# limeorange1102/multimodal-av-model

Measured on AMD Instinct MI355X. Metric: utterances/sec (4 s clip, 25 fps 96x96 lip) at batch 64, full training step, higher is better.
Workload: dtype bf16; 1 GPU; BASELINE metric configuration (= configs[3]'s per-GPU batch): batch 64/GPU x 4 s (T_audio 64000, T_enc 199, 100 lip frames 96x96 x 2 speakers), wav2vec2-large + ResNet-18 + fusion BiLSTM + CTC + contrastive, fwd+bwd+Adam, random-init weights; variant=as_executed, global_batch=64, parallelism=dp1, audio_passes=2, wav2vec2_regularizers=hf-defaults (dropout 0.1, LayerDrop 0.1, SpecAugment 0.05)

## Files before the change

include/av_hip.h:

```cpp
#ifndef AV_HIP_H
#define AV_HIP_H
#ifdef __cplusplus
extern "C" {
#endif

#define AV_OK 0
#define AV_ERR_ARG 1
#define AV_ERR_LAUNCH 2

#define AV_F32 0
#define AV_BF16 1

#define AV_A_ROWMAJOR 0
#define AV_A_TRANS 1
#define AV_A_CONV2D 2
#define AV_A_CONV3D1 3
#define AV_B_NK 0
#define AV_B_KN 1
#define AV_ACT_NONE 0
#define AV_ACT_GELU 1
#define AV_ACT_MUL_GELU_GRAD 2
#define AV_ACT_GELU_GF 3
#define AV_ACT_MUL_AUX 4

const char* av_last_error(void);
int av_version(void);

typedef struct av_gemm_args {
    const void* A;
    const void* B;
    void* C;
    void* C2;
    const float* bias;
    const float* R;
    const void* aux;
    float* stats;
    int M, N, K, batch;
    long long lda, ldb, ldc, ldr;
    long long sA, sB, sC, sR, sBias;
    int a_mode, b_mode, in_dtype, out_dtype, aux_dtype, act;
    float alpha;
    int cT, cH, cW, cCtot, cCin, cCoff;
    int cKt, cKh, cKw, cSh, cSw, cPt, cPh, cPw, cOh, cOw;
    int batch_inner;
    long long oA, oB, oC;
    float drop_p;
    unsigned int drop_stream;
    unsigned long long drop_seed;
    int k_total;
    int cNF, cPM;
} av_gemm_args;
int av_gemm(const av_gemm_args* args, void* stream);
int av_sum_slices(const float* parts, int n_slices, long long n, long long stride, float alpha, float* out, int accumulate,
                  void* stream);
int av_transpose(const void* in, int idt, void* out, int odt, int R, int C, long long ldi, int Rpad, void* stream);

int av_layernorm_fwd(const void* x, int xdt, const float* gamma, const float* beta, void* y, int ydt,
                     float* mean, float* rstd, long long rows, int cols, float eps, int act, void* stream);
int av_layernorm_bwd(const void* x, int xdt, const void* dy, int dydt, const float* gamma, const float* mean,
                     const float* rstd, const float* dres, float* dx, float* dgb_partial, int nblk,
                     long long rows, int cols, void* dx_bf16, void* stream);
int av_layernorm_bwd_drop(const void* x, int xdt, const void* dy, int dydt, const float* gamma, const float* mean,
                          const float* rstd, const float* dres, float* dx, float* dgb_partial, int nblk,
                          long long rows, int cols, void* dx_bf16, float drop_p, unsigned long long drop_seed,
                          unsigned int drop_stream, void* stream);
int av_log_softmax_fwd(const void* x, int xdt, float* y, long long rows, int cols, void* stream);
int av_log_softmax_bwd(const float* y, const float* dy, void* dx, int dxdt, long long rows, int cols, void* stream);
int av_log_softmax_bwd_ld(const float* y, const float* dy, void* dx, int dxdt, long long rows, int cols, int ldx, void* stream);
int av_colsum(const void* x, int xdt, float* out, long long rows, int cols, long long ld, int accumulate,
              void* stream);
int av_cast(const void* x, int xdt, void* y, int ydt, long long n, void* stream);
int av_cast_dropout(const void* x, int xdt, void* y, int ydt, long long n, float p, unsigned long long seed, unsigned int stream_id,
                    void* stream);
int av_dropout_uniform(float* u, long long n, unsigned long long seed, unsigned int stream_id, void* stream);
int av_fusion_xattn_fwd(const void* a, const void* v, const void* w_in, const float* b_in, void* q_out, void* kv_out, void* o,
                        float* lse, int B, int T, int E, int H, float scale, void* stream);
int av_fusion_xattn_bwd(const void* q, const void* kv, const void* o, const void* dout, const float* lse, void* dq, void* dkv, int B, int T,
                        int E, int H, float scale, void* stream);
int av_zero_feature_cols(void* x, int xdt, const unsigned char* mask, int B, int T, int H, void* stream);
int av_overwrite_rows(void* x, int xdt, const unsigned char* mask, const float* embed, long long rows, int cols, void* stream);
int av_axpby(float a, const void* x, int xdt, float b, float* y, long long n, void* stream);
int av_mask_rows(void* x, int xdt, const unsigned char* keep, long long rows, int cols, void* stream);
int av_mul_scalar_dev(const float* x, const float* scalar, float* y, long long n, void* stream);

int av_attention_fwd(const void* q, const void* k, const void* v, void* o, float* lse, int dtype, int B, int H, int Tq,
                     int Tk, int D, long long q_bs, long long q_rs, long long k_bs, long long k_rs, long long v_bs,
                     long long v_rs, long long o_bs, long long o_rs, const int* klen, float scale, float drop_p,
                     unsigned long long drop_seed, unsigned int drop_stream, void* stream);
int av_attention_bwd(const void* q, const void* k, const void* v, const void* o, const void* dout, const float* lse,
                     float* delta_ws, void* dq, void* dk, void* dv, int B, int H, int Tq, int Tk, int D,
                     const long long* strides, const int* klen, float scale, float drop_p, unsigned long long drop_seed,
                     unsigned int drop_stream, void* stream);
int av_attention_dropmask(void* mask, int B, int H, int Tq, int Tk, float drop_p, unsigned long long drop_seed, unsigned int drop_stream,
                          void* stream);
int av_attention_fwd_mask(const void* q, const void* k, const void* v, void* o, float* lse, int dtype, int B, int H, int Tq,
                          int Tk, int D, long long q_bs, long long q_rs, long long k_bs, long long k_rs, long long v_bs,
                          long long v_rs, long long o_bs, long long o_rs, const int* klen, float scale, float drop_p,
                          unsigned long long drop_seed, unsigned int drop_stream, const void* drop_mask, void* stream);
int av_attention_bwd_mask(const void* q, const void* k, const void* v, const void* o, const void* dout, const float* lse,
                          float* delta_ws, void* dq, void* dk, void* dv, int B, int H, int Tq, int Tk, int D,
                          const long long* strides, const int* klen, float scale, float drop_p, unsigned long long drop_seed,
                          unsigned int drop_stream, const void* drop_mask, void* stream);
int av_softmax_rows(const float* s, void* p, int pdt, long long rows, int cols, float scale, const int* klen,
                    int rows_per_batch, int ld, void* stream);
int av_softmax_bwd_rows(const void* p, int pdt, const float* dp, void* ds, int dsdt, long long rows, int cols,
                        float scale, int ld, void* stream);

int av_conv0_ln_gelu(const float* wav, const float* w, const float* bias, const float* gamma, const float* beta, void* out,
                     int out_dtype, int B, int T_in, int L_out, int C, int k, int stride, float eps, void* stream);

int av_lstm_fwd_step(const float* gx, const void* whh, void* hseq, float* cseq, void* gates, void* out_bt, int dtype,
                     int T, int B, int H, int s, void* stream);
int av_lstm_bwd_step(const void* dout, int dout_dtype, long long do_bs, long long do_ts, void* dgates, const void* whhT,
                     const void* gates, const float* cseq, float* dc, int dtype, int T, int B, int H, int s, void* stream);

#define AV_LSTM_COUNTER_INTS 1024
int av_lstm_fwd_layer(const float* gx, const void* whh, void* hseq, float* cseq, void* gates, void* out_bt, int* counters,
                      int T, int B, int H, void* stream);
int av_lstm_bwd_layer(const void* dout, int dout_dtype, long long do_bs, long long do_ts, void* dgates, const void* whhT,
                      const void* gates, const float* cseq, float* dc, int* counters, int T, int B, int H, void* stream);

int av_mask_downsample(const long long* mask, long long* out, int B, int Tin, int Tout, void* stream);
int av_fusion_gather_lerp_fwd(const float* feat, const long long* mask, int* ws_i32, float* out, long long* mask_out,
                              long long* lens, int B, int Ta, int Tv, int D, int groups, void* stream);
int av_fusion_gather_lerp_bwd(const float* dout, const int* ws_i32, float* dfeat, int B, int Ta, int Tv, int D, int groups,
                              void* stream);
int av_permute_bt(const void* in, int idt, void* out, int odt, int B, int T, int D, void* stream);
int av_gather_rows(const void* src, int sdt, const long long* idx, void* out, int odt, long long n, int D, void* stream);
int av_scatter_rows(const float* src, const long long* idx, float* out, long long n, int D, float alpha, int accumulate,
                    void* stream);
int av_class_order(const long long* mask, long long n, long long* order, void* stream);

int av_conv3d_front(const float* x, const void* w, void* y, float* stats, int B, int T, int H, int W, void* stream);
int av_conv3d_front_pool(const float* x, const void* w, void* ymax, void* ymin, float* stats, int B, int T, int H, int W, void* stream);
int av_bn_prelu_minmax(const void* ymax, const void* ymin, const float* scale, const float* shift, const float* slope, void* out, long long n,
                       void* stream);
int av_conv3x3_c64(const void* x, const void* w, void* y, float* stats, int n_img, int H, int W, const float* in_scale,
                   const float* in_shift, const float* in_slope, void* stream);
int av_bn_finalize(const float* partial, int nblk, long long count, const float* gamma, const float* beta,
                   float* running_mean, float* running_var, float momentum, float eps, int training, float* scale,
                   float* shift, int C, double* ws, int ws_zeroed, void* stream);
int av_bn_act(const void* x, const float* scale, const float* shift, const void* res, const float* rscale,
              const float* rshift, const float* slope, void* out, int dtype, long long n, int C, void* stream);
int av_bn_prelu_maxpool(const void* x, const float* scale, const float* shift, const float* slope, void* out, int dtype,
                        long long N, int H, int W, int C, void* stream);
int av_avgpool(const void* x, int dtype, float* out, long long N, int HW, int C, int pm_block, void* stream);

int av_l2norm_fwd(const float* x, float* y, float* nrm, long long rows, int cols, float eps, void* stream);
int av_l2norm_bwd(const float* y, const float* dy, const float* nrm, float* dx, long long rows, int cols, float eps,
                  void* stream);
int av_lse_rows(const float* s, float* lse, float* rowsum, long long rows, int cols, int ld, void* stream);
int av_contrastive_dsim(const float* s, const float* lse, void* out, int odt, long long rows, int cols, int ld, float coef,
                        void* stream);
int av_lse_rows_chunk(const float* s, float* lse, float* rowsum, long long rows, int cols, int ld, int accumulate, void* stream);
int av_contrastive_dsim_chunk(const float* s, const float* lse, void* out, int odt, long long rows, int cols, int ld, float coef,
                              int total_cols, void* stream);
int av_reduce_sum(const float* x, long long n, float* out, float scale, int accumulate, void* stream);
int av_loss_combine(const float* nll, const float* w, const float* c1, const float* c2, float half_lambda, int n, float* out3,
                    void* stream);
int av_ctc_greedy(const float* log_probs, const long long* lengths, int* out_ids, int* out_len, int B, int T, int V, int blank,
                  void* stream);
int av_ctc_beam_workspace_bytes(int B, int T, int V, int beam_width, long long* bytes);
int av_ctc_beam_frame_pass(const float* log_probs, long long stride_b, long long stride_t, const long long* lengths, void* workspace,
                           long long workspace_bytes, int B, int T, int V, int blank, int beam_width, void* stream);
int av_ctc_beam_search(const float* log_probs, long long stride_b, long long stride_t, const long long* lengths, int* out_ids,
                       int* out_len, float* out_score, void* workspace, long long workspace_bytes, int B, int T, int V, int blank,
                       int beam_width, int nbest, void* stream);
int av_ngram_score(const int* ids, const long long* lens, float* out, int B, int Lmax, const float* lm_unigrams, const void* lm_table,
                   long long lm_slots, int lm_order, int lm_vocab, int lm_bos, int lm_probe_bound, void* stream);
int av_ctc_beam_lm_workspace_bytes(int B, int T, int V, int beam_width, int tokens, long long* bytes);
int av_ctc_beam_search_lm(const float* log_probs, long long stride_b, long long stride_t, const long long* lengths, int* out_ids,
                          int* out_len, float* out_score, float* out_lm_score, void* workspace, long long workspace_bytes, int B, int T,
                          int V, int blank, int beam_width, int nbest, int tokens, const float* lm_unigrams, const void* lm_table,
                          long long lm_slots, int lm_order, int lm_vocab, int lm_bos, int lm_probe_bound, float lm_weight,
                          float token_bonus, void* stream);
int av_ctc_loss_fwd(const float* log_probs, long long stride_b, long long stride_t, const long long* targets, long long target_ld,
                    const long long* input_lengths, const long long* target_lengths, int B, int T, int V, int S_max, int blank,
                    int zero_infinity, float* nll, float* log_alpha, float* log_beta, void* stream);
int av_ctc_loss_bwd(const float* log_probs, long long stride_b, long long stride_t, const long long* targets, long long target_ld,
                    const long long* input_lengths, const long long* target_lengths, int B, int T, int V, int S_max, int blank,
                    const float* nll, const float* log_alpha, const float* log_beta, const float* grad_nll, float* grad, void* stream);
int av_ctc_align_workspace_bytes(int B, int T, int S_max, long long* bytes);
int av_ctc_align(const float* log_probs, long long stride_b, long long stride_t, const long long* targets, long long target_ld,
                 const long long* input_lengths, const long long* target_lengths, int B, int T, int V, int S_max, int blank,
                 int* out_state, int* out_span, float* out_token_score, float* out_score, void* workspace, long long workspace_bytes,
                 void* stream);
int av_lip_gray_resize(const void* src, int src_is_u8, float* dst, int T, int Hs, int Ws, int C, int Hd, int Wd, float divisor,
                       void* stream);
int av_mix_pair(const float* a1, long long len1, const float* a2, long long len2, float* mixed, long long* mask1, long long* mask2,
                unsigned* peak_ws, void* stream);
int av_adam_step(float* p, const float* g, float* m, float* v, long long n, float lr, float beta1, float beta2, float eps,
                 int step, float grad_scale, void* stream);
int av_adam_multi(const void* ptrs, const long long* sizes, const float* hyper, const int* chunk_tensor, const long long* chunk_start,
                  int n_chunks, int chunk_elems, int* steps, const int* step_slot, int n_tensors, float grad_scale,
                  float* scaler_state, float growth, float backoff, int growth_interval, void* stream);

int av_nchw_to_nhwc(const float* in, void* out, int out_dtype, long long N, int C, int H, int W, int Cp, void* stream);
int av_relu_maxpool2_fwd(const void* x, void* y, int dtype, long long N, int H, int W, int C, int nchw_out, void* stream);
int av_relu_maxpool2_bwd(const void* x, const void* dy, void* dx, int dtype, long long N, int H, int W, int C, int nchw_dy, void* stream);
int av_im2col3(const void* x, void* cols, int dtype, long long N, int H, int W, int C, void* stream);
int av_gru_fwd_step(const float* gx, const void* whh, const float* bhh, void* hseq, float* hf, float* gates, void* out_bt, int dtype,
                    int T, int B, int H, int s, void* stream);
int av_gru_bwd_step(const void* dout, int dout_dtype, long long do_bs, long long do_ts, void* dgi, void* dgh, const void* whhT,
// ... 45 lines not shown
```

multimodal-av-model_amd/_lib.py:

```python
from __future__ import annotations

import ctypes as C
import os

from . import precision as _precision

_HERE = os.path.dirname(os.path.abspath(__file__))
LIB_PATH = os.environ.get("AVAMD_LIB") or os.path.join(_HERE, "libavhip.so")

AV_F32, AV_BF16 = 0, 1
A_ROWMAJOR, A_TRANS, A_CONV2D, A_CONV3D1 = 0, 1, 2, 3
B_NK, B_KN = 0, 1
ACT_NONE, ACT_GELU, ACT_MUL_GELU_GRAD, ACT_GELU_GF, ACT_MUL_AUX = 0, 1, 2, 3, 4
LSTM_COUNTER_INTS = 1024

vp, ll, i32, f32 = C.c_void_p, C.c_longlong, C.c_int, C.c_float


class GemmArgs(C.Structure):
    _fields_ = [
        ("A", vp), ("B", vp), ("C", vp), ("C2", vp), ("bias", vp), ("R", vp), ("aux", vp), ("stats", vp),
        ("M", i32), ("N", i32), ("K", i32), ("batch", i32),
        ("lda", ll), ("ldb", ll), ("ldc", ll), ("ldr", ll),
        ("sA", ll), ("sB", ll), ("sC", ll), ("sR", ll), ("sBias", ll),
        ("a_mode", i32), ("b_mode", i32), ("in_dtype", i32), ("out_dtype", i32), ("aux_dtype", i32), ("act", i32),
        ("alpha", f32),
        ("cT", i32), ("cH", i32), ("cW", i32), ("cCtot", i32), ("cCin", i32), ("cCoff", i32),
        ("cKt", i32), ("cKh", i32), ("cKw", i32), ("cSh", i32), ("cSw", i32), ("cPt", i32), ("cPh", i32), ("cPw", i32),
        ("cOh", i32), ("cOw", i32),
        ("batch_inner", i32), ("oA", ll), ("oB", ll), ("oC", ll),
        ("drop_p", f32), ("drop_stream", C.c_uint), ("drop_seed", C.c_ulonglong),
        ("k_total", i32), ("cNF", i32), ("cPM", i32),
    ]


class W2v2LayerArgs(C.Structure):
    _fields_ = [
        ("B", i32), ("T", i32), ("hidden", i32), ("heads", i32), ("inter", i32), ("lp", i32), ("gf", i32), ("stream_base", i32),
        ("eps", f32), ("scale", f32), ("hd_p", f32), ("at_p", f32), ("ac_p", f32),
        ("seed", C.c_ulonglong),
        ("ln1_g", vp), ("ln1_b", vp), ("ln2_g", vp), ("ln2_b", vp), ("b_qkv", vp), ("b_o", vp), ("b_1", vp), ("b_2", vp),
        ("w_qkv", vp), ("w_o", vp), ("w_1", vp), ("w_2", vp),
        ("h", vp), ("klen", vp), ("amask", vp),
        ("x1", vp), ("qkv", vp), ("ao", vp), ("x2", vp), ("u", vp), ("g", vp),
        ("mu1", vp), ("rs1", vp), ("lse", vp), ("h2", vp), ("mu2", vp), ("rs2", vp), ("h3", vp),
    ]


class W2v2LayerBwdArgs(C.Structure):
    _fields_ = [
        ("B", i32), ("T", i32), ("hidden", i32), ("heads", i32), ("inter", i32), ("lp", i32), ("gf", i32), ("stream_base", i32), ("lower_stream", i32),
        ("scale", f32), ("hd_p", f32), ("at_p", f32), ("ac_p", f32),
        ("seed", C.c_ulonglong),
        ("ln1_g", vp), ("ln2_g", vp),
        ("w_2t", vp), ("w_1t", vp), ("w_ot", vp), ("w_qkvt", vp),
        ("dh", vp), ("h", vp), ("mu1", vp), ("rs1", vp), ("lse", vp), ("h2", vp), ("mu2", vp), ("rs2", vp),
        ("dh_lp", vp), ("qkv", vp), ("ao", vp), ("amask", vp), ("u", vp),
        ("klen", vp),
        ("dh3_t", vp), ("du", vp), ("dx2", vp), ("dh2_lp", vp), ("dao", vp), ("dqkv", vp), ("dx1", vp), ("dh_out_lp", vp),
        ("dh2", vp), ("delta", vp), ("dh_out", vp),
    ]


SIGNATURES = {
    "av_last_error": [],
    "av_version": [],
    "av_gemm": [C.POINTER(GemmArgs), vp],
    "av_w2v2_layer_fwd": [C.POINTER(W2v2LayerArgs), vp],
    "av_w2v2_layer_bwd_dx": [C.POINTER(W2v2LayerBwdArgs), vp],
    "av_transpose": [vp, i32, vp, i32, i32, i32, ll, i32, vp],
    "av_sum_slices": [vp, i32, ll, ll, f32, vp, i32, vp],
    "av_layernorm_fwd": [vp, i32, vp, vp, vp, i32, vp, vp, ll, i32, f32, i32, vp],
    "av_layernorm_bwd_drop": [vp, i32, vp, i32, vp, vp, vp, vp, vp, vp, i32, ll, i32, vp, f32, C.c_ulonglong, C.c_uint, vp],
    "av_layernorm_bwd": [vp, i32, vp, i32, vp, vp, vp, vp, vp, vp, i32, ll, i32, vp, vp],
    "av_log_softmax_fwd": [vp, i32, vp, ll, i32, vp],
    "av_log_softmax_bwd": [vp, vp, vp, i32, ll, i32, vp],
    "av_log_softmax_bwd_ld": [vp, vp, vp, i32, ll, i32, i32, vp],
    "av_colsum": [vp, i32, vp, ll, i32, ll, i32, vp],
    "av_cast": [vp, i32, vp, i32, ll, vp],
    "av_cast_dropout": [vp, i32, vp, i32, ll, f32, C.c_ulonglong, C.c_uint, vp],
    "av_dropout_uniform": [vp, ll, C.c_ulonglong, C.c_uint, vp],
    "av_fusion_xattn_fwd": [vp, vp, vp, vp, vp, vp, vp, vp, i32, i32, i32, i32, f32, vp],
    "av_fusion_xattn_bwd": [vp, vp, vp, vp, vp, vp, vp, i32, i32, i32, i32, f32, vp],
    "av_zero_feature_cols": [vp, i32, vp, i32, i32, i32, vp],
    "av_overwrite_rows": [vp, i32, vp, vp, ll, i32, vp],
    "av_axpby": [f32, vp, i32, f32, vp, ll, vp],
    "av_mask_rows": [vp, i32, vp, ll, i32, vp],
    "av_mul_scalar_dev": [vp, vp, vp, ll, vp],
    "av_attention_fwd": [vp, vp, vp, vp, vp, i32, i32, i32, i32, i32, i32, ll, ll, ll, ll, ll, ll, ll, ll, vp, f32, f32, C.c_ulonglong, C.c_uint, vp],
    "av_attention_dropmask": [vp, i32, i32, i32, i32, f32, C.c_ulonglong, C.c_uint, vp],
    "av_attention_fwd_mask": [vp, vp, vp, vp, vp, i32, i32, i32, i32, i32, i32, ll, ll, ll, ll, ll, ll, ll, ll, vp, f32, f32, C.c_ulonglong, C.c_uint, vp, vp],
    "av_attention_bwd_mask": [vp, vp, vp, vp, vp, vp, vp, vp, vp, vp, i32, i32, i32, i32, i32, vp, vp, f32, f32, C.c_ulonglong, C.c_uint, vp, vp],
    "av_attention_bwd": [vp, vp, vp, vp, vp, vp, vp, vp, vp, vp, i32, i32, i32, i32, i32, vp, vp, f32, f32, C.c_ulonglong, C.c_uint, vp],
    "av_softmax_rows": [vp, vp, i32, ll, i32, f32, vp, i32, i32, vp],
    "av_conv0_ln_gelu": [vp, vp, vp, vp, vp, vp, i32, i32, i32, i32, i32, i32, i32, f32, vp],
    "av_lstm_fwd_step": [vp, vp, vp, vp, vp, vp, i32, i32, i32, i32, i32, vp],
    "av_lstm_bwd_step": [vp, i32, ll, ll, vp, vp, vp, vp, vp, i32, i32, i32, i32, i32, vp],
    "av_lstm_fwd_layer": [vp, vp, vp, vp, vp, vp, vp, i32, i32, i32, vp],
    "av_lstm_bwd_layer": [vp, i32, ll, ll, vp, vp, vp, vp, vp, vp, i32, i32, i32, vp],
    "av_mask_downsample": [vp, vp, i32, i32, i32, vp],
    "av_fusion_gather_lerp_fwd": [vp, vp, vp, vp, vp, vp, i32, i32, i32, i32, i32, vp],
    "av_fusion_gather_lerp_bwd": [vp, vp, vp, i32, i32, i32, i32, i32, vp],
    "av_permute_bt": [vp, i32, vp, i32, i32, i32, i32, vp],
    "av_gather_rows": [vp, i32, vp, vp, i32, ll, i32, vp],
    "av_scatter_rows": [vp, vp, vp, ll, i32, f32, i32, vp],
    "av_class_order": [vp, ll, vp, vp],
    "av_conv3d_front": [vp, vp, vp, vp, i32, i32, i32, i32, vp],
    "av_conv3d_front_pool": [vp, vp, vp, vp, vp, i32, i32, i32, i32, vp],
    "av_bn_prelu_minmax": [vp, vp, vp, vp, vp, vp, ll, vp],
    "av_conv3x3_c64": [vp, vp, vp, vp, i32, i32, i32, vp, vp, vp, vp],
    "av_bn_finalize": [vp, i32, ll, vp, vp, vp, vp, f32, f32, i32, vp, vp, i32, vp, i32, vp],
    "av_bn_act": [vp, vp, vp, vp, vp, vp, vp, vp, i32, ll, i32, vp],
    "av_bn_prelu_maxpool": [vp, vp, vp, vp, vp, i32, ll, i32, i32, i32, vp],
    "av_avgpool": [vp, i32, vp, ll, i32, i32, i32, vp],
    "av_l2norm_fwd": [vp, vp, vp, ll, i32, f32, vp],
    "av_l2norm_bwd": [vp, vp, vp, vp, ll, i32, f32, vp],
    "av_lse_rows": [vp, vp, vp, ll, i32, i32, vp],
    "av_lse_rows_chunk": [vp, vp, vp, ll, i32, i32, i32, vp],
    "av_contrastive_dsim_chunk": [vp, vp, vp, i32, ll, i32, i32, f32, i32, vp],
    "av_contrastive_dsim": [vp, vp, vp, i32, ll, i32, i32, f32, vp],
    "av_reduce_sum": [vp, ll, vp, f32, i32, vp],
    "av_loss_combine": [vp, vp, vp, vp, f32, i32, vp, vp],
    "av_ctc_greedy": [vp, vp, vp, vp, i32, i32, i32, i32, vp],
    "av_ctc_beam_workspace_bytes": [i32, i32, i32, i32, C.POINTER(ll)],
    "av_ctc_beam_frame_pass": [vp, ll, ll, vp, vp, ll, i32, i32, i32, i32, i32, vp],
    "av_ctc_beam_search": [vp, ll, ll, vp, vp, vp, vp, vp, ll, i32, i32, i32, i32, i32, i32, vp],
    "av_ngram_score": [vp, vp, vp, i32, i32, vp, vp, ll, i32, i32, i32, i32, vp],
    "av_ctc_beam_lm_workspace_bytes": [i32, i32, i32, i32, i32, C.POINTER(ll)],
    "av_ctc_beam_search_lm": [vp, ll, ll, vp, vp, vp, vp, vp, vp, ll, i32, i32, i32, i32, i32, i32, i32, vp, vp, ll, i32, i32, i32, i32, f32, f32, vp],
    "av_ctc_loss_fwd": [vp, ll, ll, vp, ll, vp, vp, i32, i32, i32, i32, i32, i32, vp, vp, vp, vp],
    "av_ctc_loss_bwd": [vp, ll, ll, vp, ll, vp, vp, i32, i32, i32, i32, i32, vp, vp, vp, vp, vp, vp],
    "av_ctc_align_workspace_bytes": [i32, i32, i32, C.POINTER(ll)],
    "av_ctc_align": [vp, ll, ll, vp, ll, vp, vp, i32, i32, i32, i32, i32, vp, vp, vp, vp, vp, ll, vp],
    "av_lip_gray_resize": [vp, i32, vp, i32, i32, i32, i32, i32, i32, f32, vp],
    "av_mix_pair": [vp, ll, vp, ll, vp, vp, vp, vp, vp],
    "av_adam_multi": [vp, vp, vp, vp, vp, i32, i32, vp, vp, i32, f32, vp, f32, f32, i32, vp],
    "av_adam_step": [vp, vp, vp, vp, ll, f32, f32, f32, f32, i32, f32, vp],
    "av_softmax_bwd_rows": [vp, i32, vp, vp, i32, ll, i32, f32, i32, vp],
    "av_nchw_to_nhwc": [vp, vp, i32, ll, i32, i32, i32, i32, vp],
    "av_relu_maxpool2_fwd": [vp, vp, i32, ll, i32, i32, i32, i32, vp],
    "av_relu_maxpool2_bwd": [vp, vp, vp, i32, ll, i32, i32, i32, i32, vp],
    "av_im2col3": [vp, vp, i32, ll, i32, i32, i32, vp],
    "av_gru_fwd_step": [vp, vp, vp, vp, vp, vp, vp, i32, i32, i32, i32, i32, vp],
    "av_gru_bwd_step": [vp, i32, ll, ll, vp, vp, vp, vp, vp, vp, i32, i32, i32, i32, i32, vp],
    "av_wav_info": [C.c_char_p, C.POINTER(i32), C.POINTER(i32), C.POINTER(ll), C.POINTER(i32), C.POINTER(i32)],
    "av_wav_read_mono_f32": [C.c_char_p, ll, ll, vp],
    "av_resample_sinc": [vp, ll, vp, ll, vp, vp, i32, i32, i32, i32, vp],
}
_RESTYPES = {"av_last_error": C.c_char_p}

_libs = {}
_by_mode = {}


def _path() -> str:
    if _precision.get_precision() == "fp16":
        return os.environ.get("AVAMD_LIB_F16") or os.path.join(_HERE, "libavhip_f16.so")
    return LIB_PATH


def lib() -> C.CDLL:
    l = _by_mode.get(_precision._mode)
    if l is not None:
        return l
    path = _path()
    l = _libs.get(path)
    if l is None:
        if not os.path.exists(path):
            raise RuntimeError(
                f"{path} is missing: build it with `python {os.path.join(_HERE, 'build.py')}` "
                "(hipcc --offload-arch=gfx950). The MI355X path has no CPU/PyTorch fallback.")
        import torch
        l = C.CDLL(path)
        for name, argtypes in SIGNATURES.items():
            fn = getattr(l, name)
            fn.argtypes = argtypes
            fn.restype = _RESTYPES.get(name, C.c_int)
        _libs[path] = l
    _by_mode[_precision._mode] = l
    return l


def check(status: int, what: str = "") -> None:
    if status != 0:
        msg = lib().av_last_error().decode("utf-8", "replace")
# ... 2 lines not shown
```

multimodal-av-model_amd/csrc/gemm.hip:

```cpp
#include "av_common.h"

namespace {

constexpr int BM = 128;
constexpr int BK = 32;
constexpr int NT = 256;

template <typename T> struct Cfg;
template <> struct Cfg<float> { static constexpr int LD = 36, VEC = 4; };
template <> struct Cfg<bf16_t> { static constexpr int LD = 40, VEC = 8; };

template <typename T> struct Vec16 { uint4 v; };

template <typename T> __device__ __forceinline__ T elem_of(const uint4& v, int i);
template <> __device__ __forceinline__ float elem_of<float>(const uint4& v, int i) {
    const unsigned u = i == 0 ? v.x : i == 1 ? v.y : i == 2 ? v.z : v.w;
    return __uint_as_float(u);
}
template <> __device__ __forceinline__ bf16_t elem_of<bf16_t>(const uint4& v, int i) {
    const unsigned u = (i >> 1) == 0 ? v.x : (i >> 1) == 1 ? v.y : (i >> 1) == 2 ? v.z : v.w;
    const unsigned short s = (i & 1) ? (unsigned short)(u >> 16) : (unsigned short)(u & 0xffff);
    return __builtin_bit_cast(bf16_t, s);
}
template <typename T> __device__ __forceinline__ void set_elem(uint4& v, int i, T x);
// ... 215 lines not shown
    stage_load<T, BM, AMODE>(ra, A, p.lda, m0, p.M, 0, p.K, a_vec, p, ri, tid);
    stage_load<T, BN, BMODE == AV_B_NK ? AV_A_ROWMAJOR : AV_A_TRANS>(rb, B, p.ldb, n0, p.N, 0, p.K, b_vec, p, rib, tid);
    stage_store<T, BM, AMODE>(sA, ra, tid);
    stage_store<T, BN, BMODE == AV_B_NK ? AV_A_ROWMAJOR : AV_A_TRANS>(sB, rb, tid);
    __syncthreads();

    for (int kt = 0; kt < nk; ++kt) {
        const int cur = kt & 1;
        if (kt + 1 < nk) {
            stage_load<T, BM, AMODE>(ra, A, p.lda, m0, p.M, (kt + 1) * BK, p.K, a_vec, p, ri, tid);
            stage_load<T, BN, BMODE == AV_B_NK ? AV_A_ROWMAJOR : AV_A_TRANS>(rb, B, p.ldb, n0, p.N, (kt + 1) * BK, p.K, b_vec, p, rib, tid);
        }
        mma_step<T, WN_T>(sA + cur * BM * LD + wm * 64 * LD, sB + cur * BN * LD + wn * (BN / 2) * LD, acc, lane);
        if (kt + 1 < nk) {
            stage_store<T, BM, AMODE>(sA + (cur ^ 1) * BM * LD, ra, tid);
            stage_store<T, BN, BMODE == AV_B_NK ? AV_A_ROWMAJOR : AV_A_TRANS>(sB + (cur ^ 1) * BN * LD, rb, tid);
        }
        __syncthreads();
    }

    const int r = lane & 15, g = lane >> 4;
    const long long cbase = (long long)zo * p.oC + (long long)zi * p.sC;
    const float* R = p.R ? p.R + (long long)zi * p.sR : nullptr;
    float csum[WN_T], csq[WN_T];
#pragma unroll
    for (int j = 0; j < WN_T; ++j) { csum[j] = 0.f; csq[j] = 0.f; }
#pragma unroll
    for (int j = 0; j < WN_T; ++j) {
        const int n = n0 + wn * (BN / 2) + j * 16 + r;
        const bool nok = n < p.N;
        const float bias = (p.bias && nok) ? p.bias[(long long)zi * p.sBias + n] : 0.f;
#pragma unroll
        for (int i = 0; i < 4; ++i) {
#pragma unroll
            for (int e = 0; e < 4; ++e) {
                const int m = m0 + wm * 64 + i * 16 + 4 * g + e;
                if (nok && m < p.M) {
                    float v = acc[i][j][e] * p.alpha + bias;
                    const long long off = cbase + (long long)m * p.ldc + n;
                    if (p.act == AV_ACT_GELU_GF) {
                        const float mlt = p.drop_p > 0.f ? drop_mult_call(p.drop_seed, p.drop_stream, (unsigned long long)off, p.drop_p, drop_inv_keep(p.drop_p)) : 1.f;
                        if (p.C2) st_any(p.C2, off, p.out_dtype, gelu_grad_f(v) * mlt);
                        v = gelu_f(v) * mlt;
                    } else {
                        if (p.C2) st_any(p.C2, off, p.out_dtype, v);
                        if (p.act == AV_ACT_GELU) v = gelu_f(v);
                        else if (p.act == AV_ACT_MUL_GELU_GRAD) v *= gelu_grad_f(ld_any(p.aux, off, p.aux_dtype));
                        else if (p.act == AV_ACT_MUL_AUX) v *= ld_any(p.aux, off, p.aux_dtype);
                        if (p.drop_p > 0.f) v *= drop_mult_call(p.drop_seed, p.drop_stream, (unsigned long long)off, p.drop_p, drop_inv_keep(p.drop_p));
                    }
                    if (R) v += R[(long long)m * p.ldr + n];
                    st_any(p.C, off, p.out_dtype, v);
                    csum[j] += v; csq[j] += v * v;
                }
            }
        }
    }
    if (p.stats) {
        __syncthreads();
        float* red = (float*)smem;
#pragma unroll
        for (int j = 0; j < WN_T; ++j) {
            float s = csum[j], q = csq[j];
            s += __shfl_xor(s, 16, 64); s += __shfl_xor(s, 32, 64);
            q += __shfl_xor(q, 16, 64); q += __shfl_xor(q, 32, 64);
            if (g == 0) {
                const int col = wn * (BN / 2) + j * 16 + r;
                red[(wm * 2 + 0) * BN + col] = s;
                red[(wm * 2 + 1) * BN + col] = q;
            }
        }
        __syncthreads();
        if (tid < BN && n0 + tid < p.N) {
            float* out = p.stats + (long long)mb * 2 * p.N;
            out[n0 + tid] = red[0 * BN + tid] + red[2 * BN + tid];
            out[p.N + n0 + tid] = red[1 * BN + tid] + red[3 * BN + tid];
        }
    }
}

template <typename T, int BN, int AMODE, int BMODE>
int launch(const av_gemm_args& p, hipStream_t st, bool a_vec, bool b_vec) {
    const size_t lds = (size_t)(2 * BM + 2 * BN) * Cfg<T>::LD * sizeof(T);
    static bool attr_done = false;
    auto kern = gemm_kernel<T, BN, AMODE, BMODE>;
    if (!attr_done && lds > 48 * 1024) {
        if (hipFuncSetAttribute((const void*)kern, hipFuncAttributeMaxDynamicSharedMemorySize, (int)lds) != hipSuccess) {
            av_set_error("av_gemm: cannot raise dynamic LDS to %zu", lds);
            return AV_ERR_LAUNCH;
        }
        attr_done = true;
    }
    const int nbM = av_cdiv(p.M, BM), nbN = av_cdiv(p.N, BN);
    dim3 grid((unsigned)(nbM * (long long)nbN), 1, (unsigned)p.batch);
    hipLaunchKernelGGL(kern, grid, dim3(NT), lds, st, p, nbN, a_vec, b_vec);
    AV_LAUNCH_CHECK();
    return AV_OK;
}

template <typename T, int BN>
int dispatch_modes(const av_gemm_args& p, hipStream_t st, bool a_vec, bool b_vec) {
    if (p.a_mode == AV_A_ROWMAJOR && p.b_mode == AV_B_NK) return launch<T, BN, AV_A_ROWMAJOR, AV_B_NK>(p, st, a_vec, b_vec);
    if (p.a_mode == AV_A_ROWMAJOR && p.b_mode == AV_B_KN) return launch<T, BN, AV_A_ROWMAJOR, AV_B_KN>(p, st, a_vec, b_vec);
    if (p.a_mode == AV_A_TRANS && p.b_mode == AV_B_KN) return launch<T, BN, AV_A_TRANS, AV_B_KN>(p, st, a_vec, b_vec);
    if (p.a_mode == AV_A_CONV2D && p.b_mode == AV_B_NK) return launch<T, BN, AV_A_CONV2D, AV_B_NK>(p, st, a_vec, b_vec);
    if (p.a_mode == AV_A_CONV3D1 && p.b_mode == AV_B_NK) return launch<T, BN, AV_A_CONV3D1, AV_B_NK>(p, st, a_vec, b_vec);
    av_set_error("av_gemm: unsupported operand mode pair a_mode=%d b_mode=%d", p.a_mode, p.b_mode);
    return AV_ERR_ARG;
}

template <typename T>
bool vec_ok(const void* base, long long ld, long long stride) {
    const long long es = sizeof(T);
    return ((uintptr_t)base % 16 == 0) && ((ld * es) % 16 == 0) && ((stride * es) % 16 == 0);
}
template <typename T> bool vec_ok2(const void* base, long long ld, long long s1, long long s2) {
    return vec_ok<T>(base, ld, s1) && ((s2 * (long long)sizeof(T)) % 16 == 0);
}

}

int av_gemm_fast_try(const av_gemm_args& p, hipStream_t st);

extern "C" int av_gemm(const av_gemm_args* a, void* stream) {
    AV_CHECK(a != nullptr, "av_gemm: null args");
    const av_gemm_args& p = *a;
    AV_CHECK(p.A && p.B && p.C, "av_gemm: null operand pointer");
    AV_CHECK(p.M >= 0 && p.N >= 0 && p.K > 0 && p.batch >= 1, "av_gemm: bad shape M=%d N=%d K=%d batch=%d", p.M, p.N, p.K, p.batch);
    AV_CHECK(p.in_dtype == AV_F32 || p.in_dtype == AV_BF16, "av_gemm: bad in_dtype %d", p.in_dtype);
    AV_CHECK(p.out_dtype == AV_F32 || p.out_dtype == AV_BF16, "av_gemm: bad out_dtype %d", p.out_dtype);
    AV_CHECK(!(p.stats && p.batch != 1), "av_gemm: stats need batch == 1");
    AV_CHECK(!((p.act == AV_ACT_MUL_GELU_GRAD || p.act == AV_ACT_MUL_AUX) && !p.aux), "av_gemm: MUL_GELU_GRAD / MUL_AUX need aux");
    AV_CHECK(p.act >= AV_ACT_NONE && p.act <= AV_ACT_MUL_AUX, "av_gemm: unknown activation %d", p.act);
    AV_CHECK(p.drop_p >= 0.f && p.drop_p < 1.f, "av_gemm: drop_p=%f out of [0,1)", p.drop_p);
    if (p.M == 0 || p.N == 0) return AV_OK;
    const long long es = p.in_dtype == AV_F32 ? 4 : 2;
    const int vec = (int)(16 / es);
    if (p.a_mode == AV_A_CONV2D) {
        AV_CHECK(p.cCin % vec == 0 && p.cCoff % vec == 0 && p.cCtot % vec == 0 && (uintptr_t)p.A % 16 == 0 && (p.sA * es) % 16 == 0,
                 "av_gemm conv2d: channels (Cin=%d, Coff=%d, Ctot=%d) must be multiples of %d and the base 16-byte aligned", p.cCin, p.cCoff, p.cCtot, vec);
        AV_CHECK(p.K == p.cKh * p.cKw * p.cCin, "av_gemm conv2d: K=%d != Kh*Kw*Cin", p.K);
        AV_CHECK(p.cOh > 0 && p.cOw > 0 && p.M % (p.cOh * p.cOw) == 0, "av_gemm conv2d: M=%d not a multiple of Oh*Ow", p.M);
    }
    if (p.a_mode == AV_A_CONV3D1) {
        AV_CHECK(p.K == p.cKt * p.cKh * p.cKw, "av_gemm conv3d: K=%d != Kt*Kh*Kw", p.K);
        AV_CHECK(p.cOh > 0 && p.cOw > 0 && p.cT > 0 && p.M % (p.cOh * p.cOw * p.cT) == 0, "av_gemm conv3d: bad M=%d", p.M);
    }
    hipStream_t st = (hipStream_t)stream;
    {
        const int fr = av_gemm_fast_try(p, st);
        if (fr >= 0) return fr;
    }
    AV_CHECK(p.cPM == 0, "av_gemm: position-major pixel order (cPM) needs the bf16 fast path (2-D convolution, Cin a multiple of 64, one batch)");
    AV_CHECK(p.k_total == 0, "av_gemm: split-K (k_total) needs the bf16 fast path with both operands k-major (a_mode 1, b_mode 1, M, N multiples of 8 and > 64)");
    const bool wide = p.N > 64;
    if (p.in_dtype == AV_F32) {
        const bool av = vec_ok2<float>(p.A, p.lda, p.sA, p.oA), bv = vec_ok2<float>(p.B, p.ldb, p.sB, p.oB);
        return wide ? dispatch_modes<float, 128>(p, st, av, bv) : dispatch_modes<float, 64>(p, st, av, bv);
    } else {
        const bool av = vec_ok2<bf16_t>(p.A, p.lda, p.sA, p.oA), bv = vec_ok2<bf16_t>(p.B, p.ldb, p.sB, p.oB);
        return wide ? dispatch_modes<bf16_t, 128>(p, st, av, bv) : dispatch_modes<bf16_t, 64>(p, st, av, bv);
    }
}
```

multimodal-av-model_amd/csrc/gemm_fast.hip:

```cpp
#include <cstdlib>

#include "av_common.h"

namespace {

constexpr int BM = 128, BK = 64, NT = 256;
constexpr int TILE_A = BM * BK * 2;

typedef const __attribute__((address_space(1))) void* gptr_t;
typedef __attribute__((address_space(3))) void* lptr_t;

__device__ __attribute__((aligned(256))) unsigned char g_zero_line[256];

#ifdef AV_GEMM_STAMPS
__device__ unsigned long long g_gemm_stamps[8192 * 4];
#define AV_STAMP(SLOT) do { if (threadIdx.x == 0 && blockIdx.x < 8192) g_gemm_stamps[blockIdx.x * 4 + (SLOT)] = __builtin_amdgcn_s_memrealtime(); } while (0)
__device__ unsigned long long g_v7_stamps[256 * 16 * 4];
#define AV_STAMP7(SEQ, SLOT) do { if (threadIdx.x == 0 && blockIdx.x < 256 && (SEQ) < 16) g_v7_stamps[(blockIdx.x * 16 + (SEQ)) * 4 + (SLOT)] = __builtin_amdgcn_s_memrealtime(); } while (0)
#else
#define AV_STAMP(SLOT) do { } while (0)
#define AV_STAMP7(SEQ, SLOT) do { } while (0)
#endif

template <int NWI>
// ... 239 lines not shown
                bf16x8 o;
#pragma unroll
                for (int e = 0; e < 8; ++e) o[e] = (bf16_t)gf[e];
                {
#if AV_EPI_NT
                    __builtin_nontemporal_store(o, (bf16x8*)((bf16_t*)p.C2 + off));
#else
                    *(bf16x8*)((bf16_t*)p.C2 + off) = o;
#endif
                }
            } else {
#pragma unroll
                for (int e = 0; e < 8; ++e) if (gn + e < p.N) st_any(p.C2, off + e, p.out_dtype, gf[e]);
            }
        }
    } else
    if (p.C2) {
        if (full && fl.c_vec) {
            if (p.out_dtype == AV_BF16) {
                bf16x8 o;
#pragma unroll
                for (int e = 0; e < 8; ++e) o[e] = (bf16_t)v[e];
                *(bf16x8*)((bf16_t*)p.C2 + off) = o;
            } else {
                *(f32x4*)((float*)p.C2 + off) = f32x4{v[0], v[1], v[2], v[3]};
                *(f32x4*)((float*)p.C2 + off + 4) = f32x4{v[4], v[5], v[6], v[7]};
            }
        } else {
#pragma unroll
            for (int e = 0; e < 8; ++e) if (gn + e < p.N) st_any(p.C2, off + e, p.out_dtype, v[e]);
        }
    }
    if (p.act == AV_ACT_GELU) {
        av_f32x2 x4[4], g4[4];
#pragma unroll
        for (int k = 0; k < 4; ++k) x4[k] = av_f32x2{v[2 * k], v[2 * k + 1]};
        gelu_fast2x4(x4, g4);
#pragma unroll
        for (int k = 0; k < 4; ++k) { v[2 * k] = g4[k].x; v[2 * k + 1] = g4[k].y; }
    } else if (p.act == AV_ACT_MUL_AUX) {
        if (full && fl.aux_vec && p.aux_dtype == AV_BF16) {
            const bf16x8 u = *(const bf16x8*)((const bf16_t*)p.aux + off);
#pragma unroll
            for (int e = 0; e < 8; ++e) v[e] *= (float)u[e];
        } else {
#pragma unroll
            for (int e = 0; e < 8; ++e) if (gn + e < p.N) v[e] *= ld_any(p.aux, off + e, p.aux_dtype);
        }
    } else if (p.act == AV_ACT_MUL_GELU_GRAD) {
        if (full && fl.aux_vec && p.aux_dtype == AV_BF16) {
            const bf16x8 u = *(const bf16x8*)((const bf16_t*)p.aux + off);
#pragma unroll
            for (int e = 0; e < 8; e += 2) { const av_f32x2 g = gelu_grad_fast2(av_f32x2{(float)u[e], (float)u[e + 1]}); v[e] *= g.x; v[e + 1] *= g.y; }
        } else {
#pragma unroll
            for (int e = 0; e < 8; ++e) if (gn + e < p.N) v[e] *= gelu_grad_fast(ld_any(p.aux, off + e, p.aux_dtype));
        }
    }
    if (p.drop_p > 0.f && p.act != AV_ACT_GELU_GF) {
        const float ik = drop_inv_keep(p.drop_p);
        if (VO || (off & 3) == 0) {
            float m4[4];
            drop_mult4(p.drop_seed, p.drop_stream, (unsigned long long)off, p.drop_p, ik, m4);
#pragma unroll
            for (int e = 0; e < 4; e += 2) { const av_f32x2 t = av_f32x2{v[e], v[e + 1]} * av_f32x2{m4[e], m4[e + 1]}; v[e] = t.x; v[e + 1] = t.y; }
            drop_mult4(p.drop_seed, p.drop_stream, (unsigned long long)off + 4, p.drop_p, ik, m4);
#pragma unroll
            for (int e = 0; e < 4; e += 2) { const av_f32x2 t = av_f32x2{v[4 + e], v[5 + e]} * av_f32x2{m4[e], m4[e + 1]}; v[4 + e] = t.x; v[5 + e] = t.y; }
        } else {
#pragma unroll
            for (int e = 0; e < 8; ++e) v[e] *= drop_mult(p.drop_seed, p.drop_stream, (unsigned long long)(off + e), p.drop_p, ik);
        }
    }
    if (R) {
        const long long roff = (long long)gm * p.ldr + gn;
        if (full && fl.r_vec) {
            const f32x4 r0 = *(const f32x4*)(R + roff), r1 = *(const f32x4*)(R + roff + 4);
#pragma unroll
            for (int e = 0; e < 4; e += 2) {
                const av_f32x2 a = av_f32x2{v[e], v[e + 1]} + av_f32x2{r0[e], r0[e + 1]}, b = av_f32x2{v[4 + e], v[5 + e]} + av_f32x2{r1[e], r1[e + 1]};
                v[e] = a.x; v[e + 1] = a.y; v[4 + e] = b.x; v[5 + e] = b.y;
            }
        } else {
#pragma unroll
            for (int e = 0; e < 8; ++e) if (gn + e < p.N) v[e] += R[roff + e];
        }
    }
    if (full && fl.c_vec) {
        if (p.out_dtype == AV_BF16) {
            bf16x8 o;
#pragma unroll
            for (int e = 0; e < 8; ++e) o[e] = (bf16_t)v[e];
            *(bf16x8*)((bf16_t*)p.C + off) = o;
        } else {
            *(f32x4*)((float*)p.C + off) = f32x4{v[0], v[1], v[2], v[3]};
            *(f32x4*)((float*)p.C + off + 4) = f32x4{v[4], v[5], v[6], v[7]};
        }
    } else {
#pragma unroll
        for (int e = 0; e < 8; ++e) if (gn + e < p.N) st_any(p.C, off + e, p.out_dtype, v[e]);
    }
}

__device__ __forceinline__ void epilogue_store(const av_gemm_args& p, const FastFlags& fl, float (&v)[8], long long off, int gm, int gn, bool full,
                                               const float* R) {
    epilogue_store_t<false>(p, fl, v, off, gm, gn, full, R);
}


template <int BNT, bool CONV, bool AKM = false, bool BKM = false>
__global__ __launch_bounds__(NT, 2) void gemm_nt_bf16_kernel(const av_gemm_args p, const int nbM, const int nbN, const FastFlags fl) {
    constexpr int WM_T = BNT == 128 ? 4 : 2;
    constexpr int TILE_BB = BNT * BK * 2;
    constexpr int STAGE = TILE_A + TILE_BB;
    constexpr int CLD = BNT + 4;
    constexpr int EPI_BYTES = BM * CLD * 4;
    extern __shared__ __attribute__((aligned(16))) char smem[];
    const int tid = threadIdx.x, lane = tid & 63, w = tid >> 6;
    const int wrow = BNT == 128 ? (w >> 1) * 64 : w * 32;
    const int wcol = BNT == 128 ? (w & 1) * 64 : 0;
    const int r = lane & 15, g = lane >> 4;

    const int nwg = nbM * nbN;
    int bid = blockIdx.x;
    {
        const int q = nwg >> 3, rem = nwg & 7, xcd = bid & 7, slot = bid >> 3;
        bid = (xcd < rem ? xcd * (q + 1) : rem * (q + 1) + (xcd - rem) * q) + slot;
    }
    constexpr int GM = 8;
    const int per_group = GM * nbN;
    const int grp = bid / per_group, in_grp = bid - grp * per_group;
    const int first_m = grp * GM;
    const int gsz = nbM - first_m < GM ? nbM - first_m : GM;
    const int mb = first_m + in_grp % gsz, nb = in_grp / gsz;
    const int m0 = mb * BM, n0 = nb * BNT;
    const int z = blockIdx.z;
    const int zo = p.batch_inner > 0 ? z / p.batch_inner : 0;
    const int zi = p.batch_inner > 0 ? z % p.batch_inner : z;
    const bf16_t* A = (const bf16_t*)p.A + (long long)zo * p.oA + (long long)zi * p.sA;
    const bf16_t* B = (const bf16_t*)p.B + (long long)zo * p.oB + (long long)zi * p.sB;

    ConvRows cr;
    if constexpr (CONV) conv_rows_init(cr, A, p, m0, w, lane);
    int Kz = p.K;
    if constexpr (AKM && BKM) {
        if (p.k_total > 0 && p.k_total - z * p.K < Kz) Kz = p.k_total - z * p.K;
    }

    f32x4 acc[WM_T][4];
#pragma unroll
    for (int i = 0; i < WM_T; ++i)
#pragma unroll
        for (int j = 0; j < 4; ++j) acc[i][j] = f32x4{0.f, 0.f, 0.f, 0.f};

    TapSeq ts;
    ts.seq = 0ull; ts.ntap = -1; ts.sh = 0;
    if constexpr (CONV) { if (p.cPM) ts = tap_seq(p, m0, BM); }
    auto stage = [&](int kt, char* buf) {
        int k0 = kt * BK;
        if constexpr (CONV) { k0 = tap_k0(p, ts, kt); stage_conv(p, cr, k0, buf, w, lane); }
        else if constexpr (AKM) stage_kmajor(A, p.lda, m0, p.M, kt * BK, Kz, buf, w, lane);
        else stage_rows<4>(A, p.lda, m0, p.M, kt * BK, buf, w, lane);
        if constexpr (BKM) stage_kmajor(B, p.ldb, n0, p.N, kt * BK, Kz, buf + TILE_A, w, lane);
        else stage_rows<BNT / 32>(B, p.ldb, n0, p.N, k0, buf + TILE_A, w, lane);
    };

    int nk = (Kz + BK - 1) / BK;
    if constexpr (CONV) { if (ts.ntap >= 0) nk = ts.ntap << ts.sh; }
    KmOff ao[WM_T], bo[4];
    if constexpr (AKM) {
#pragma unroll
        for (int i = 0; i < WM_T; ++i) ao[i] = kmajor_off(wrow / 16 + i, lane);
    }
    if constexpr (BKM) {
#pragma unroll
        for (int j = 0; j < 4; ++j) bo[j] = kmajor_off(wcol / 16 + j, lane);
    }
    stage(0, smem);
    __syncthreads();

    const int sw = r & 7;
    const char* a_base = smem + (wrow + r) * 128;
    const char* b_base = smem + TILE_A + (wcol + r) * 128;
    for (int kt = 0; kt < nk; ++kt) {
        const int cur = kt & 1;
        if (kt + 1 < nk) stage(kt + 1, smem + (cur ^ 1) * STAGE);
        const char* ab = a_base + cur * STAGE;
        const char* bb = b_base + cur * STAGE;
#pragma unroll
        for (int ks = 0; ks < 2; ++ks) {
            const int choff = ((ks * 4 + g) ^ sw) << 4;
            bf16x8 a[WM_T], b[4];
            bf16x4 ah[4][2], bh[4][2];
#pragma unroll
            for (int i = 0; i < WM_T; ++i) {
                if constexpr (AKM) kmajor_read(smem + cur * STAGE, ao[i], ks, ah[i]);
                else a[i] = *(const bf16x8*)(ab + i * 16 * 128 + choff);
            }
#pragma unroll
            for (int j = 0; j < 4; ++j) {
                if constexpr (BKM) kmajor_read(smem + cur * STAGE + TILE_A, bo[j], ks, bh[j]);
                else b[j] = *(const bf16x8*)(bb + j * 16 * 128 + choff);
            }
            if constexpr (AKM || BKM) {
                asm volatile("s_waitcnt lgkmcnt(0)" ::: "memory");
                if constexpr (AKM) {
                    static_assert(WM_T == 4, "k-major A: 128-wide tiles");
                    kmajor_tie4(ah);
#pragma unroll
                    for (int i = 0; i < WM_T; ++i) a[i] = __builtin_shufflevector(ah[i][0], ah[i][1], 0, 1, 2, 3, 4, 5, 6, 7);
                }
                if constexpr (BKM) {
                    kmajor_tie4(bh);
#pragma unroll
                    for (int j = 0; j < 4; ++j) b[j] = __builtin_shufflevector(bh[j][0], bh[j][1], 0, 1, 2, 3, 4, 5, 6, 7);
                }
            }
#pragma unroll
            for (int i = 0; i < WM_T; ++i)
#pragma unroll
                for (int j = 0; j < 4; ++j)
                    acc[i][j] = AV_MFMA_F32_16X16X32_LP(a[i], b[j], acc[i][j], 0, 0, 0);
        }
        __syncthreads();
    }

    float* cs = (float*)smem;
#pragma unroll
    for (int i = 0; i < WM_T; ++i)
#pragma unroll
        for (int j = 0; j < 4; ++j)
#pragma unroll
            for (int e = 0; e < 4; ++e)
                cs[(wrow + i * 16 + 4 * g + e) * CLD + wcol + j * 16 + r] = acc[i][j][e] * p.alpha;
    if (p.stats) {
        float* red = (float*)(smem + EPI_BYTES);
        const int wslot = BNT == 128 ? (w >> 1) : w;
#pragma unroll
        for (int j = 0; j < 4; ++j) {
            float s1 = 0.f, s2 = 0.f;
#pragma unroll
            for (int i = 0; i < WM_T; ++i)
#pragma unroll
                for (int e = 0; e < 4; ++e) { const float v = acc[i][j][e] * p.alpha; s1 += v; s2 += v * v; }
            s1 += __shfl_xor(s1, 16, 64); s1 += __shfl_xor(s1, 32, 64);
            s2 += __shfl_xor(s2, 16, 64); s2 += __shfl_xor(s2, 32, 64);
            if (g == 0) {
                red[(wslot * 2) * BNT + wcol + j * 16 + r] = s1;
                red[(wslot * 2 + 1) * BNT + wcol + j * 16 + r] = s2;
            }
        }
    }
    __syncthreads();

    const long long cbase = (long long)zo * p.oC + (long long)zi * p.sC;
    const float* R = p.R ? p.R + (long long)zi * p.sR : nullptr;
    const float* bias = p.bias ? p.bias + (long long)zi * p.sBias : nullptr;
    constexpr int CPR = BNT / 8;
    float bv[8];
    {
        const int gnt = n0 + (tid % CPR) * 8;
#pragma unroll
        for (int e = 0; e < 8; ++e) bv[e] = (bias && gnt + e < p.N) ? bias[gnt + e] : 0.f;
    }
    const bool fast_tail = n0 + BNT <= p.N && fl.c_vec && !p.C2 && p.act == AV_ACT_NONE && p.drop_p <= 0.f && !R && p.out_dtype == AV_BF16;
    if (fast_tail) {
        constexpr int NIT = BM * CPR / NT;
        uint4 ov[NIT];
        const int cc = (tid % CPR) * 8;
#pragma unroll
        for (int it = 0; it < NIT; ++it) {
            const int row = (it * NT + tid) / CPR;
            const f32x4 v0 = *(const f32x4*)(cs + row * CLD + cc), v1 = *(const f32x4*)(cs + row * CLD + cc + 4);
            bf16x8 o;
#pragma unroll
            for (int e = 0; e < 4; ++e) { o[e] = (bf16_t)(v0[e] + bv[e]); o[4 + e] = (bf16_t)(v1[e] + bv[4 + e]); }
            ov[it] = __builtin_bit_cast(uint4, o);
        }
#pragma unroll
        for (int it = 0; it < NIT; ++it) asm volatile("" :: "v"(ov[it].x), "v"(ov[it].y), "v"(ov[it].z), "v"(ov[it].w));
#pragma unroll
        for (int it = 0; it < NIT; ++it) {
            const int row = (it * NT + tid) / CPR;
            if (m0 + row < p.M) *(uint4*)((bf16_t*)p.C + cbase + (long long)(m0 + row) * p.ldc + n0 + cc) = ov[it];
        }
    }
    if (!fast_tail)
#pragma unroll
    for (int it = 0; it < BM * CPR / NT; ++it) {
        const int id = it * NT + tid;
        const int row = id / CPR, cc = (id % CPR) * 8;
        const int gm = m0 + row, gn = n0 + cc;
        if (gm >= p.M || gn >= p.N) continue;
        float v[8];
        const f32x4 v0 = *(const f32x4*)(cs + row * CLD + cc), v1 = *(const f32x4*)(cs + row * CLD + cc + 4);
#pragma unroll
        for (int e = 0; e < 4; ++e) { v[e] = v0[e]; v[4 + e] = v1[e]; }
        const bool full = gn + 8 <= p.N;
        const long long off = cbase + (long long)gm * p.ldc + gn;
#pragma unroll
        for (int e = 0; e < 8; ++e) v[e] += bv[e];
        if (p.act == AV_ACT_GELU_GF) {
            float m[8], gf[8];
#pragma unroll
            for (int e = 0; e < 8; ++e) m[e] = 1.f;
            if (p.drop_p > 0.f) {
                const float ik = drop_inv_keep(p.drop_p);
                if ((off & 3) == 0) {
                    float m4[4];
                    drop_mult4(p.drop_seed, p.drop_stream, (unsigned long long)off, p.drop_p, ik, m4);
#pragma unroll
                    for (int e = 0; e < 4; ++e) m[e] = m4[e];
                    drop_mult4(p.drop_seed, p.drop_stream, (unsigned long long)off + 4, p.drop_p, ik, m4);
#pragma unroll
                    for (int e = 0; e < 4; ++e) m[4 + e] = m4[e];
                } else {
#pragma unroll
                    for (int e = 0; e < 8; ++e) m[e] = drop_mult(p.drop_seed, p.drop_stream, (unsigned long long)(off + e), p.drop_p, ik);
                }
            }
#pragma unroll
            for (int e = 0; e < 8; e += 2) {
                av_f32x2 gl, gp;
                const av_f32x2 mm = av_f32x2{m[e], m[e + 1]};
                gelu_both_fast2(av_f32x2{v[e], v[e + 1]}, gl, gp);
                gl = gl * mm; gp = gp * mm;
                v[e] = gl.x; v[e + 1] = gl.y; gf[e] = gp.x; gf[e + 1] = gp.y;
            }
            if (p.C2) {
                if (full && fl.c_vec && p.out_dtype == AV_BF16) {
                    bf16x8 o;
#pragma unroll
                    for (int e = 0; e < 8; ++e) o[e] = (bf16_t)gf[e];
                    *(bf16x8*)((bf16_t*)p.C2 + off) = o;
                } else {
#pragma unroll
                    for (int e = 0; e < 8; ++e) if (gn + e < p.N) st_any(p.C2, off + e, p.out_dtype, gf[e]);
                }
            }
        } else
        if (p.C2) {
            if (full && fl.c_vec) {
                if (p.out_dtype == AV_BF16) {
                    bf16x8 o;
#pragma unroll
                    for (int e = 0; e < 8; ++e) o[e] = (bf16_t)v[e];
                    *(bf16x8*)((bf16_t*)p.C2 + off) = o;
                } else {
                    *(f32x4*)((float*)p.C2 + off) = f32x4{v[0], v[1], v[2], v[3]};
                    *(f32x4*)((float*)p.C2 + off + 4) = f32x4{v[4], v[5], v[6], v[7]};
                }
            } else {
#pragma unroll
                for (int e = 0; e < 8; ++e) if (gn + e < p.N) st_any(p.C2, off + e, p.out_dtype, v[e]);
            }
        }
        if (p.act == AV_ACT_GELU) {
#pragma unroll
            for (int e = 0; e < 8; e += 2) { const av_f32x2 g = gelu_fast2(av_f32x2{v[e], v[e + 1]}); v[e] = g.x; v[e + 1] = g.y; }
        } else if (p.act == AV_ACT_MUL_AUX) {
            if (full && fl.aux_vec && p.aux_dtype == AV_BF16) {
                const bf16x8 u = *(const bf16x8*)((const bf16_t*)p.aux + off);
#pragma unroll
                for (int e = 0; e < 8; ++e) v[e] *= (float)u[e];
            } else {
#pragma unroll
                for (int e = 0; e < 8; ++e) if (gn + e < p.N) v[e] *= ld_any(p.aux, off + e, p.aux_dtype);
            }
        } else if (p.act == AV_ACT_MUL_GELU_GRAD) {
            if (full && fl.aux_vec && p.aux_dtype == AV_BF16) {
                const bf16x8 u = *(const bf16x8*)((const bf16_t*)p.aux + off);
#pragma unroll
                for (int e = 0; e < 8; e += 2) { const av_f32x2 g = gelu_grad_fast2(av_f32x2{(float)u[e], (float)u[e + 1]}); v[e] *= g.x; v[e + 1] *= g.y; }
            } else {
#pragma unroll
                for (int e = 0; e < 8; ++e) if (gn + e < p.N) v[e] *= gelu_grad_fast(ld_any(p.aux, off + e, p.aux_dtype));
            }
// ... 255 lines not shown
        if (t + 2 < nk) { issue(t + 2); asm volatile("s_waitcnt vmcnt(4)" ::: "memory"); }
        else asm volatile("s_waitcnt vmcnt(0)" ::: "memory");
        __builtin_amdgcn_s_barrier();
        __builtin_amdgcn_s_waitcnt(0xC07F);
        __builtin_amdgcn_sched_barrier(0);
        __builtin_amdgcn_s_setprio(1);
#pragma unroll
        for (int ks = 0; ks < 2; ++ks)
#pragma unroll
            for (int i = 0; i < 4; ++i)
#pragma unroll
                for (int j = 0; j < 2; ++j)
                    acc[i][j] = AV_MFMA_F32_16X16X32_LP(fa[i][ks], fb[j][ks], acc[i][j], 0, 0, 0);
        __builtin_amdgcn_s_setprio(0);
        __builtin_amdgcn_sched_barrier(0);
        __builtin_amdgcn_s_barrier();
        asm volatile("" ::: "memory");
    }
    if (wr == 0) __builtin_amdgcn_s_barrier();

    constexpr int QLD = 128 + 4;
    float* cs = (float*)smem;
    __syncthreads();
#pragma unroll
    for (int i = 0; i < 4; ++i)
#pragma unroll
        for (int j = 0; j < 2; ++j)
#pragma unroll
            for (int e = 0; e < 4; ++e)
                cs[(wr * 64 + i * 16 + 4 * g + e) * QLD + wc * 32 + j * 16 + r] = acc[i][j][e] * p.alpha;
    __syncthreads();
    constexpr int CPR = 128 / 8;
    float bv[8];
    {
        const int gnt = n0 + (tid % CPR) * 8;
#pragma unroll
        for (int e = 0; e < 8; ++e) bv[e] = (bias && gnt + e < p.N) ? bias[gnt + e] : 0.f;
    }
    for (int it = 0; it < 128 * CPR / V4_NT; ++it) {
        const int id = it * V4_NT + tid;
        const int row = id / CPR, cc = (id % CPR) * 8;
        const int gm = m0 + row, gn = n0 + cc;
        if (gm >= m_end || gn >= p.N) continue;
        float v[8];
        const f32x4 v0 = *(const f32x4*)(cs + row * QLD + cc), v1 = *(const f32x4*)(cs + row * QLD + cc + 4);
#pragma unroll
        for (int e = 0; e < 4; ++e) { v[e] = v0[e] + bv[e]; v[4 + e] = v1[e] + bv[4 + e]; }
        const bool full = gn + 8 <= p.N;
        const long long off = cbase + (long long)gm * p.ldc + gn;
        epilogue_store(p, fl, v, off, gm, gn, full, R);
    }
}

struct ConvRows2 { const bf16_t* rowp[2]; unsigned valid[2]; };
__device__ __forceinline__ void conv_rows2_init(ConvRows2& cr, const bf16_t* __restrict__ base, const av_gemm_args& p, int mbase, int w, int lane) {
    const int sub = lane >> 3, choff = ((lane & 7) ^ sub) << 3;
#pragma unroll
    for (int i = 0; i < 2; ++i) {
        const int m = mbase + (w * 2 + i) * 8 + sub;
        cr.rowp[i] = base;
        cr.valid[i] = 0u;
        if (m < p.M) {
            int q, oy, ox;
            conv_decode(p, m, q, oy, ox);
            const int iy0 = oy * p.cSh - p.cPh, ix0 = ox * p.cSw - p.cPw;
            cr.rowp[i] = base + conv_pixel(p, q, iy0, ix0) * p.cCtot + p.cCoff + choff;
            unsigned v = 0u;
            for (int ky = 0; ky < p.cKh; ++ky)
                for (int kx = 0; kx < p.cKw; ++kx)
                    if (iy0 + ky >= 0 && iy0 + ky < p.cH && ix0 + kx >= 0 && ix0 + kx < p.cW) v |= 1u << (ky * p.cKw + kx);
            cr.valid[i] = v;
        }
    }
}
__device__ __forceinline__ void stage_conv2(const av_gemm_args& p, const ConvRows2& cr, int k0, char* tile, int w, int lane, bool all_in) {
    const int sub = lane >> 3, pch = lane & 7;
    const int tap = k0 / p.cCin, c0 = k0 - tap * p.cCin;
    const int ky = tap / p.cKw, kx = tap - ky * p.cKw;
    const long long toff = ((long long)ky * p.cW + kx) * ((p.cPM & 1) ? p.cNF : 1) * p.cCtot + c0;
    if (all_in) {
#pragma unroll
        for (int i = 0; i < 2; ++i) {
            const unsigned off = __builtin_amdgcn_readfirstlane((unsigned)((w * 2 + i) * 1024));
            __builtin_amdgcn_global_load_lds((gptr_t)(cr.rowp[i] + toff), (lptr_t)(tile + off), 16, 0, 0);
        }
        return;
    }
    const bf16_t* zl = (const bf16_t*)g_zero_line + ((pch ^ sub) << 3);
#pragma unroll
    for (int i = 0; i < 2; ++i) {
        const bf16_t* src = ((cr.valid[i] >> tap) & 1u) ? cr.rowp[i] + toff : zl;
        const unsigned off = __builtin_amdgcn_readfirstlane((unsigned)((w * 2 + i) * 1024));
        __builtin_amdgcn_global_load_lds((gptr_t)src, (lptr_t)(tile + off), 16, 0, 0);
    }
}

template <bool CONV, bool KM = false>
__global__ __launch_bounds__(V4_NT, 2) void gemm_nt_bf16_v4_kernel(const av_gemm_args p, const int nbM, const int nbN, const FastFlags fl, const int nfull, const int bm_eff) {
    static_assert(!(CONV && KM), "k-major operands: plain products only");
    extern __shared__ __attribute__((aligned(16))) char smem[];
    AV_STAMP(0);
    const int tid = threadIdx.x, lane = tid & 63, w = tid >> 6;
    const int wr = __builtin_amdgcn_readfirstlane(w >> 2), wc = w & 3;
    const int r = lane & 15, g = lane >> 4;
    const int ntile = nbM * nbN;
    int bid = blockIdx.x, quad = -1;
    if (bid < nfull) {
        const int q = nfull >> 3, rem = nfull & 7, xcd = bid & 7, slot = bid >> 3;
        bid = (xcd < rem ? xcd * (q + 1) : rem * (q + 1) + (xcd - rem) * q) + slot;
    } else {
        const int nq = 4 * (ntile - nfull);
        int j = bid - nfull;
        const int q = nq >> 3, rem = nq & 7, xcd = j & 7, slot = j >> 3;
        j = (xcd < rem ? xcd * (q + 1) : rem * (q + 1) + (xcd - rem) * q) + slot;
        bid = nfull + (j >> 2);
        quad = j & 3;
    }
    int z = blockIdx.z;
    if constexpr (KM) {
        z = bid / ntile;
        bid -= z * ntile;
    }
    constexpr int GM = 4;
    const int per_group = GM * nbN;
    const int grp = bid / per_group, in_grp = bid - grp * per_group;
    const int first_m = grp * GM;
    const int gsz = nbM - first_m < GM ? nbM - first_m : GM;
    const int mb = first_m + in_grp % gsz, nb = in_grp / gsz;
    const int m0 = mb * bm_eff, n0 = nb * V4_BN;
    const int rows_here = p.M - m0 < bm_eff ? p.M - m0 : bm_eff;
    const int zo = p.batch_inner > 0 ? z / p.batch_inner : 0;
    const int zi = p.batch_inner > 0 ? z % p.batch_inner : z;
    const bf16_t* A = (const bf16_t*)p.A + (long long)zo * p.oA + (long long)zi * p.sA;
    const bf16_t* B = (const bf16_t*)p.B + (long long)zo * p.oB + (long long)zi * p.sB;
    if (quad >= 0) {
        const int qm = m0 + (quad >> 1) * 128, qn = n0 + (quad & 1) * 128;
        if (qm < m0 + rows_here && qn < p.N)
            v4_quadrant_job(p, fl, smem, A, B, qm, qn, m0 + rows_here, (long long)zo * p.oC + (long long)zi * p.sC,
                            p.R ? p.R + (long long)zi * p.sR : nullptr, p.bias ? p.bias + (long long)zi * p.sBias : nullptr);
        return;
    }
    auto ntiles = [&](int start) { int n = (rows_here - start + 15) >> 4; return n < 0 ? 0 : (n > 4 ? 4 : n); };
    const int nmt0 = __builtin_amdgcn_readfirstlane(ntiles(wr * 64)), nmt1 = __builtin_amdgcn_readfirstlane(ntiles(128 + wr * 64));

    f32x4 acc[2][2][4][2];
#pragma unroll
    for (int a = 0; a < 2; ++a)
#pragma unroll
        for (int b = 0; b < 2; ++b)
#pragma unroll
            for (int i = 0; i < 4; ++i)
#pragma unroll
                for (int j = 0; j < 2; ++j) acc[a][b][i][j] = f32x4{0.f, 0.f, 0.f, 0.f};

    int nk = p.K / BK;
    int Kz = p.K;
    if constexpr (KM) {
        if (p.k_total > 0 && p.k_total - z * p.K < Kz) Kz = p.k_total - z * p.K;
        nk = (Kz + BK - 1) / BK;
    }
    ConvRows2 cr0, cr1;
    TapSeq ts;
    ts.seq = 0ull; ts.ntap = -1; ts.sh = 0;
    if constexpr (CONV) {
        conv_rows2_init(cr0, A, p, m0, w, lane); conv_rows2_init(cr1, A, p, m0 + 128, w, lane);
        if (p.cPM) { ts = tap_seq(p, m0, V4_BM); if (ts.ntap >= 0) nk = ts.ntap << ts.sh; }
    }
    const bool conv_all_in = CONV && (p.cPM & 2) && ts.ntap >= 0 && m0 + V4_BM <= p.M && m0 / p.cNF == (m0 + V4_BM - 1) / p.cNF;
    KmLane kl[4];
    if constexpr (KM) {
        km_lane_init(kl[0], p.lda, m0, p.M, w, lane); km_lane_init(kl[2], p.lda, m0 + 128, p.M, w, lane);
        km_lane_init(kl[3], p.ldb, n0, p.N, w, lane); km_lane_init(kl[1], p.ldb, n0 + 128, p.N, w, lane);
    }
    const int nh = 4 * nk;
    auto issue = [&](int t, int j, int sidx) {
#ifdef AV_ABL_NODMA
        return;
#endif
        char* slot = smem + sidx * V4_HALF;
        int k0 = t * BK;
#ifdef AV_ABL_KSCRAMBLE
        k0 = (int)(((long long)t * 37) % nk) * BK;
#endif
        if constexpr (CONV) k0 = tap_k0(p, ts, t);
        if constexpr (KM) {
            if (j == 0) stage_kmajor8(A, p.lda, kl[0], k0, Kz, slot, w, lane);
            else if (j == 2) stage_kmajor8(A, p.lda, kl[2], k0, Kz, slot, w, lane);
            else if (j == 3) stage_kmajor8(B, p.ldb, kl[3], k0, Kz, slot, w, lane);
            else stage_kmajor8(B, p.ldb, kl[1], k0, Kz, slot, w, lane);
            return;
        }
        if (j == 0) { if constexpr (CONV) stage_conv2(p, cr0, k0, slot, w, lane, conv_all_in); else stage_rows<2>(A, p.lda, m0, p.M, k0, slot, w, lane); }
        else if (j == 2) { if constexpr (CONV) stage_conv2(p, cr1, k0, slot, w, lane, conv_all_in); else stage_rows<2>(A, p.lda, m0 + 128, p.M, k0, slot, w, lane); }
        else if (j == 3) stage_rows<2>(B, p.ldb, n0, p.N, k0, slot, w, lane);
        else stage_rows<2>(B, p.ldb, n0 + 128, p.N, k0, slot, w, lane);
    };
    issue(0, 0, 0); issue(0, 1, 1); issue(0, 2, 2); issue(0, 3, 3);
    if (nk > 1) {
        issue(1, 0, 4); issue(1, 1, 5);
        if constexpr (V4_LEAD == 8) { issue(1, 2, 6); issue(1, 3, 7); asm volatile("s_waitcnt vmcnt(8)" ::: "memory"); }
        else asm volatile("s_waitcnt vmcnt(4)" ::: "memory");
    } else asm volatile("s_waitcnt vmcnt(0)" ::: "memory");
    __builtin_amdgcn_s_barrier();
    asm volatile("" ::: "memory");
    if (wr == 1) __builtin_amdgcn_s_barrier();
    AV_STAMP(1);

    const int sw = r & 7;
    const int ch0 = (g ^ sw) << 4, ch1 = ((4 + g) ^ sw) << 4;
    const int a_row = (wr * 64 + r) * 128, b_row = (wc * 32 + r) * 128;
    bf16x8 fa[4][2], fb[2][2];
#ifdef AV_ABL_NOREAD
#pragma unroll
    for (int i = 0; i < 4; ++i)
#pragma unroll
        for (int ks = 0; ks < 2; ++ks) { fa[i][ks] = bf16x8{0, 0, 0, 0, 0, 0, 0, 0}; fb[i >> 1][ks] = bf16x8{0, 0, 0, 0, 0, 0, 0, 0}; asm volatile("" : "+v"(fa[i][ks]), "+v"(fb[i >> 1][ks])); }
#endif
    bf16x8 fb0[2][2];
    bf16x4 kfa[2][2][2][2], kfb[2][2][2];
    Km8Base kab, kbb;
    const unsigned lds0 = (unsigned)(unsigned long long)(lds_b4_t)smem;
    if constexpr (KM) { km8_base_init(kab, 1024 * wr, lane); km8_base_init(kbb, 512 * wc, lane); }

#ifdef AV_ABL_NOMFMA
#define V4_MFMA_OP(ACC, A, B) asm volatile("" :: "v"(A), "v"(B))
#else
#define V4_MFMA_OP(ACC, A, B) ACC = AV_MFMA_F32_16X16X32_LP(A, B, ACC, 0, 0, 0)
#endif
#ifdef AV_ABL_NOREAD
#define V4_ABL_NR 0
#else
#define V4_ABL_NR 4
#endif
#define V4_READ_A(SLOT, NMT)                                                                                       \
    if constexpr (KM) {                                                                                            \
        if (V4_ABL_NR) {                                                                                           \
            const unsigned sb_ = lds0 + sl[SLOT] * V4_HALF;                                                        \
            const unsigned a00_ = sb_ + kab.b[0][0], a01_ = sb_ + kab.b[0][1], a10_ = sb_ + kab.b[1][0], a11_ = sb_ + kab.b[1][1];    \
            km8_read<0>(a00_, a01_, kfa[0][0][0]);       km8_read<8192>(a00_, a01_, kfa[0][0][1]);                 \
            km8_read<0>(a10_, a11_, kfa[0][1][0]);       km8_read<8192>(a10_, a11_, kfa[0][1][1]);                 \
            km8_read<512>(a00_, a01_, kfa[1][0][0]);     km8_read<8192 + 512>(a00_, a01_, kfa[1][0][1]);           \
            km8_read<512>(a10_, a11_, kfa[1][1][0]);     km8_read<8192 + 512>(a10_, a11_, kfa[1][1][1]);           \
        }                                                                                                          \
    } else {                                                                                                       \
    _Pragma("unroll") for (int i = 0; i < V4_ABL_NR; ++i) {                                                        \
            fa[i][0] = *(const bf16x8*)(smem + sl[SLOT] * V4_HALF + a_row + i * 2048 + ch0);                       \
            fa[i][1] = *(const bf16x8*)(smem + sl[SLOT] * V4_HALF + a_row + i * 2048 + ch1); } }
#define V4_READ_B(SLOT, FB, KFB)                                                                                   \
    if constexpr (KM) {                                                                                            \
        if (V4_ABL_NR) {                                                                                           \
            const unsigned sb_ = lds0 + sl[SLOT] * V4_HALF;                                                        \
            const unsigned b00_ = sb_ + kbb.b[0][0], b01_ = sb_ + kbb.b[0][1], b10_ = sb_ + kbb.b[1][0], b11_ = sb_ + kbb.b[1][1];    \
            km8_read<0>(b00_, b01_, KFB[0][0]);          km8_read<8192>(b00_, b01_, KFB[0][1]);                    \
            km8_read<0>(b10_, b11_, KFB[1][0]);          km8_read<8192>(b10_, b11_, KFB[1][1]);                    \
        }                                                                                                          \
    } else {                                                                                                       \
    _Pragma("unroll") for (int j = 0; j < V4_ABL_NR / 2; ++j) {                                                    \
            FB[j][0] = *(const bf16x8*)(smem + sl[SLOT] * V4_HALF + b_row + j * 2048 + ch0);                       \
            FB[j][1] = *(const bf16x8*)(smem + sl[SLOT] * V4_HALF + b_row + j * 2048 + ch1); } }
#define V4_JOIN_A                                                                                                  \
    if constexpr (KM) { if (V4_ABL_NR) {                                                                           \
        km8_tie8(kfa[0]); km8_tie8(kfa[1]);                                                                        \
        _Pragma("unroll") for (int i = 0; i < 4; ++i) { fa[i][0] = km8_join(kfa[i >> 1][i & 1][0]); fa[i][1] = km8_join(kfa[i >> 1][i & 1][1]); } } }
#define V4_JOIN_B(FB, KFB)                                                                                         \
    if constexpr (KM) { if (V4_ABL_NR) {                                                                           \
        km8_tie8(KFB);                                                                                             \
        _Pragma("unroll") for (int j = 0; j < 2; ++j) { FB[j][0] = km8_join(KFB[j][0]); FB[j][1] = km8_join(KFB[j][1]); } } }
#define V4_JOIN_NONE
#define V4_MMA(QA, QB, FB, JOIN)                                                                                   \
    __builtin_amdgcn_s_barrier();                                                                                  \
    __builtin_amdgcn_s_waitcnt(0xC07F);                                                                            \
    JOIN                                                                                                           \
    __builtin_amdgcn_sched_barrier(0);                                                                             \
    __builtin_amdgcn_s_setprio(1);                                                                                 \
    _Pragma("unroll") for (int ks = 0; ks < 2; ++ks)                                                               \
        _Pragma("unroll") for (int i = 0; i < 4; ++i)                                                              \
            _Pragma("unroll") for (int j = 0; j < 2; ++j)                                                          \
                V4_MFMA_OP(acc[QA][QB][i][j], fa[i][ks], FB[j][ks]);                                               \
    __builtin_amdgcn_s_setprio(0);                                                                                 \
    __builtin_amdgcn_sched_barrier(0);                                                                             \
    __builtin_amdgcn_s_barrier();                                                                                  \
    asm volatile("" ::: "memory");

    int b4 = 0;
    for (int t = 0; t < nk; ++t) {
        int sl[4], si[4];
#pragma unroll
        for (int j = 0; j < 4; ++j) {
            int x = b4 + j; x = x >= V4_NS ? x - V4_NS : x; sl[j] = x;
            int y = b4 + j - 2; y = y < 0 ? y + V4_NS : y; si[j] = y;
        }
        b4 += 4; b4 = b4 >= V4_NS ? b4 - V4_NS : b4;
        if constexpr (KM) { V4_READ_B(3, fb0, kfb) } else { V4_READ_B(3, fb, kfb) }
        __builtin_amdgcn_sched_barrier(0);
        V4_READ_A(0, nmt0)
        if (4 * t + V4_LEAD + 0 < nh) issue(t + (V4_LEAD + 0) / 4, (V4_LEAD + 0) % 4, si[0]);
        if constexpr (KM) { V4_MMA(0, 0, fb0, V4_JOIN_A V4_JOIN_B(fb0, kfb)) } else { V4_MMA(0, 0, fb, V4_JOIN_NONE) }
        V4_READ_B(1, fb, kfb)
        if (4 * t + V4_LEAD + 1 < nh) issue(t + (V4_LEAD + 1) / 4, (V4_LEAD + 1) % 4, si[1]);
        V4_MMA(0, 1, fb, V4_JOIN_B(fb, kfb))
        V4_READ_A(2, nmt1)
        if (4 * t + V4_LEAD + 2 < nh) issue(t + (V4_LEAD + 2) / 4, (V4_LEAD + 2) % 4, si[2]);
        V4_MMA(1, 1, fb, V4_JOIN_A)
        if constexpr (!KM) { V4_READ_B(3, fb, kfb) }
        if (4 * t + V4_LEAD + 3 < nh) {
            issue(t + (V4_LEAD + 3) / 4, (V4_LEAD + 3) % 4, si[3]);
            if constexpr (V4_LEAD == 8) asm volatile("s_waitcnt vmcnt(8)" ::: "memory"); else asm volatile("s_waitcnt vmcnt(4)" ::: "memory");
        } else asm volatile("s_waitcnt vmcnt(0)" ::: "memory");
        if constexpr (KM) { V4_MMA(1, 0, fb0, V4_JOIN_NONE) } else { V4_MMA(1, 0, fb, V4_JOIN_B(fb, kfb)) }
    }
#undef V4_READ_A
#undef V4_READ_B
#undef V4_MMA
#undef V4_JOIN_A
#undef V4_JOIN_B
#undef V4_JOIN_NONE
#undef V4_MFMA_OP
    if (wr == 0) __builtin_amdgcn_s_barrier();
    AV_STAMP(2);

    float* cs = (float*)smem;
    const long long cbase = (long long)zo * p.oC + (long long)zi * p.sC;
    const float* R = p.R ? p.R + (long long)zi * p.sR : nullptr;
    const float* bias = p.bias ? p.bias + (long long)zi * p.sBias : nullptr;
    constexpr int CPR = V4_BN / 8;
    float bv[8];
    {
        const int gnt = n0 + (tid % CPR) * 8;
#pragma unroll
        for (int e = 0; e < 8; ++e) bv[e] = (bias && gnt + e < p.N) ? bias[gnt + e] : 0.f;
    }
#pragma unroll
    for (int half = 0; half < 2; ++half) {
        __syncthreads();
#pragma unroll
        for (int b = 0; b < 2; ++b)
#pragma unroll
            for (int i = 0; i < 4; ++i)
#pragma unroll
                for (int j = 0; j < 2; ++j)
#pragma unroll
                    for (int e = 0; e < 4; ++e)
                        cs[(wr * 64 + i * 16 + 4 * g + e) * V4_CLD + b * 128 + wc * 32 + j * 16 + r] = acc[half][b][i][j][e] * p.alpha;
        if (CONV && p.stats) {
            float* red = (float*)(smem + V4_EPI);
#pragma unroll
            for (int b = 0; b < 2; ++b)
#pragma unroll
                for (int j = 0; j < 2; ++j) {
                    float s1 = 0.f, s2 = 0.f;
#pragma unroll
                    for (int i = 0; i < 4; ++i)
#pragma unroll
                        for (int e = 0; e < 4; ++e) { const float v = acc[half][b][i][j][e] * p.alpha; s1 += v; s2 += v * v; }
                    s1 += __shfl_xor(s1, 16, 64); s1 += __shfl_xor(s1, 32, 64);
                    s2 += __shfl_xor(s2, 16, 64); s2 += __shfl_xor(s2, 32, 64);
                    if (g == 0) {
                        const int col = b * 128 + wc * 32 + j * 16 + r;
                        red[(wr * 2) * 256 + col] = s1;
                        red[(wr * 2 + 1) * 256 + col] = s2;
                    }
                }
        }
        __syncthreads();
        for (int it = 0; it < 128 * CPR / V4_NT; ++it) {
            const int id = it * V4_NT + tid;
            const int row = id / CPR, cc = (id % CPR) * 8;
            const int gm = m0 + half * 128 + row, gn = n0 + cc;
            if (half * 128 + row >= rows_here || gn >= p.N) continue;
            float v[8];
            const f32x4 v0 = *(const f32x4*)(cs + row * V4_CLD + cc), v1 = *(const f32x4*)(cs + row * V4_CLD + cc + 4);
#pragma unroll
            for (int e = 0; e < 4; ++e) { v[e] = v0[e] + bv[e]; v[4 + e] = v1[e] + bv[4 + e]; }
            const bool full = gn + 8 <= p.N;
            const long long off = cbase + (long long)gm * p.ldc + gn;
            epilogue_store(p, fl, v, off, gm, gn, full, R);
        }
        if (CONV && p.stats && tid < 256 && n0 + tid < p.N && m0 + half * 128 < p.M) {
            const float* red = (const float*)(smem + V4_EPI);
            float* o = p.stats + (long long)(2 * mb + half) * 2 * p.N;
            o[n0 + tid] = red[tid] + red[512 + tid];
            o[p.N + n0 + tid] = red[256 + tid] + red[768 + tid];
        }
    }
#ifdef AV_GEMM_STAMPS
    asm volatile("s_waitcnt vmcnt(0)" ::: "memory");
#endif
    AV_STAMP(3);
}


__device__ __forceinline__ int v7_bcol(int rho, int b) {
    return ((rho >> 5) << 6) | (b << 5) | (((rho >> 2) & 3) << 3) | (((rho >> 4) & 1) << 2) | (rho & 3);
}
__device__ __forceinline__ void v7_stage_b(const bf16_t* __restrict__ base, long long ld, int n0, int nrows, int k0, char* tile, int w, int lane, int b) {
    const int sub = lane >> 3, pch = lane & 7;
#pragma unroll
    for (int i = 0; i < 2; ++i) {
        const int rho = (w * 2 + i) * 8 + sub;
        int gr = n0 + v7_bcol(rho, b);
        if (gr > nrows - 1) gr = nrows - 1;
        const bf16_t* src = base + (long long)gr * ld + k0 + ((pch ^ sub) << 3);
        const unsigned off = __builtin_amdgcn_readfirstlane((unsigned)((w * 2 + i) * 1024));
        __builtin_amdgcn_global_load_lds((gptr_t)src, (lptr_t)(tile + off), 16, 0, 0);
    }
}

__device__ __forceinline__ void v7_wait_dma8_plus(int S) {
#define V7_WCASE(H) case H: asm volatile("s_waitcnt vmcnt(%0)" :: "n"(8 + 2 * (H)) : "memory"); break;
    switch (S >> 1) {
        V7_WCASE(16) V7_WCASE(15) V7_WCASE(14) V7_WCASE(13) V7_WCASE(12) V7_WCASE(11) V7_WCASE(10) V7_WCASE(9) V7_WCASE(8) V7_WCASE(7) V7_WCASE(6)
        V7_WCASE(5) V7_WCASE(4) V7_WCASE(3) V7_WCASE(2) V7_WCASE(1)
        default: asm volatile("s_waitcnt vmcnt(8)" ::: "memory"); break;
    }
#undef V7_WCASE
}

template <bool VO>
__device__ __forceinline__ void v7_chunk(const av_gemm_args& p, const FastFlags& fl, const f32x4& c0, const f32x4& c1, const float (&bv)[8],
                                         int gm, int gn, int m_end, long long cbase, const float* R) {
    if (gm >= m_end || gn >= p.N) return;
    float v[8];
#pragma unroll
    for (int e = 0; e < 4; ++e) { v[e] = c0[e] * p.alpha + bv[e]; v[4 + e] = c1[e] * p.alpha + bv[4 + e]; }
    epilogue_store_t<VO>(p, fl, v, cbase + (long long)gm * p.ldc + gn, gm, gn, gn + 8 <= p.N, R);
}

template <int ACT, int ODT, bool VO, int NM1>
__global__ __launch_bounds__(V4_NT, 2) void gemm_nt_bf16_v7_kernel(const av_gemm_args pa, const int nbM, const int nbN, const FastFlags fl, const int nfull, const int bm_eff) {
    extern __shared__ __attribute__((aligned(16))) char smem[];
    static_assert(V4_LEAD == 8, "v7 assumes the 10-slot ring");
    av_gemm_args p = pa;
    if constexpr (ACT >= 0) p.act = ACT;
    if constexpr (ODT >= 0) p.out_dtype = ODT;
    const int tid = threadIdx.x, lane = tid & 63, w = tid >> 6;
    const int wr = __builtin_amdgcn_readfirstlane(w >> 2), wc = w & 3;
    const int r = lane & 15, g = lane >> 4;
    const int ntile = nbM * nbN;
    const int G = (int)gridDim.x;
    const int xcd = blockIdx.x & 7, slot = blockIdx.x >> 3;
    const int S = (G - xcd + 7) >> 3;
    int cs, cn;
    { const int q = nfull >> 3, rem = nfull & 7; cn = q + (xcd < rem ? 1 : 0); cs = xcd < rem ? xcd * (q + 1) : rem * (q + 1) + (xcd - rem) * q; }
    auto coords = [&](int id, int& m0, int& n0, int& mb) {
        constexpr int GM = 4;
        const int per_group = GM * nbN;
        const int grp = id / per_group, in_grp = id - grp * per_group;
        const int first_m = grp * GM;
        const int gsz = nbM - first_m < GM ? nbM - first_m : GM;
        mb = first_m + in_grp % gsz;
        m0 = mb * bm_eff; n0 = (in_grp / gsz) * V4_BN;
    };
    const int z = blockIdx.z;
    const int zo = p.batch_inner > 0 ? z / p.batch_inner : 0;
    const int zi = p.batch_inner > 0 ? z % p.batch_inner : z;
    const bf16_t* A = (const bf16_t*)p.A + (long long)zo * p.oA + (long long)zi * p.sA;
    const bf16_t* B = (const bf16_t*)p.B + (long long)zo * p.oB + (long long)zi * p.sB;
    const long long cbase = (long long)zo * p.oC + (long long)zi * p.sC;
    const float* R = p.R ? p.R + (long long)zi * p.sR : nullptr;
    const float* bias = p.bias ? p.bias + (long long)zi * p.sBias : nullptr;
    const int nk = p.K / BK, nh = 4 * nk;

    auto issue = [&](int tm0, int tn0, int t, int j, int sidx) {
        char* sl_ = smem + sidx * V4_HALF;
        const int k0 = t * BK;
        const int a_end = p.M - tm0 < bm_eff ? p.M : tm0 + bm_eff;
        if (j == 0) stage_rows<2>(A, p.lda, tm0, a_end, k0, sl_, w, lane);
        else if (j == 2) stage_rows<2>(A, p.lda, tm0 + 128, a_end, k0, sl_, w, lane);
        else if (j == 3) v7_stage_b(B, p.ldb, tn0, p.N, k0, sl_, w, lane, 0);
        else v7_stage_b(B, p.ldb, tn0, p.N, k0, sl_, w, lane, 1);
    };
    auto prefetch = [&](int tm0, int tn0) {
// ... 251 lines not shown
        asm volatile("s_waitcnt vmcnt(8)" ::: "memory");
    } else {
        asm volatile("s_waitcnt vmcnt(0)" ::: "memory");
    }
    __builtin_amdgcn_s_barrier();
    asm volatile("" ::: "memory");
    AV_STAMP(1);

    const int sw = r & 7;
    const int ch0 = (g ^ sw) << 4, ch1 = ((4 + g) ^ sw) << 4;
    const int a_off = (wr * 128 + r) * 128, b_off = 32768 + (wc * 128 + r) * 128;
#define V6_A(ST, I, CH) (*(const bf16x8*)((ST) + a_off + (I) * 2048 + (CH)))
#define V6_B(ST, J, CH) (*(const bf16x8*)((ST) + b_off + (J) * 2048 + (CH)))
#define V6_MMA8(I, FA, FB)                                                                                         \
    _Pragma("unroll") for (int j = 0; j < 8; ++j) acc[I][j] = AV_MFMA_F32_16X16X32_LP(FA, FB[j], acc[I][j], 0, 0, 0);

    bf16x8 fb[8], fbn[8], fa0, fa1, fa2;
    {
        const char* st = smem;
#pragma unroll
        for (int j = 0; j < 8; ++j) fb[j] = V6_B(st, j, ch0);
        fa0 = V6_A(st, 0, ch0);
    }
    for (int t = 0; t < nk; ++t) {
        const char* st = smem + (t & 1) * V6_STAGE;
        const char* stn = smem + ((t + 1) & 1) * V6_STAGE;
        const bool more1 = t + 1 < nk, more2 = t + 2 < nk;
#pragma unroll
        for (int i = 0; i < 8; ++i) {
            __builtin_amdgcn_sched_barrier(0);
            fa1 = i < 7 ? V6_A(st, i + 1, ch0) : V6_A(st, 0, ch1);
            fbn[i] = V6_B(st, i, ch1);
            if (more1) V6_DMA(t + 1, 8 + i);
            __builtin_amdgcn_sched_barrier(0);
            V6_MMA8(i, fa0, fb)
            fa0 = fa1;
        }
#pragma unroll
        for (int i = 0; i < 6; ++i) {
            __builtin_amdgcn_sched_barrier(0);
            fa1 = V6_A(st, i + 1, ch1);
            if (i == 5) fa2 = V6_A(st, 7, ch1);
            __builtin_amdgcn_sched_barrier(0);
            V6_MMA8(i, fa0, fbn)
            fa0 = fa1;
        }
        __builtin_amdgcn_sched_barrier(0);
        asm volatile("s_waitcnt vmcnt(0) lgkmcnt(0)" ::: "memory");
        __builtin_amdgcn_s_barrier();
        asm volatile("" ::: "memory");
        __builtin_amdgcn_sched_barrier(0);
        if (more1) {
#pragma unroll
            for (int j = 0; j < 4; ++j) fb[j] = V6_B(stn, j, ch0);
        }
        if (more2) {
#pragma unroll
            for (int q = 0; q < 4; ++q) V6_DMA(t + 2, q);
        }
        __builtin_amdgcn_sched_barrier(0);
        V6_MMA8(6, fa0, fbn)
        __builtin_amdgcn_sched_barrier(0);
        if (more1) {
#pragma unroll
            for (int j = 4; j < 8; ++j) fb[j] = V6_B(stn, j, ch0);
            fa0 = V6_A(stn, 0, ch0);
        }
        if (more2) {
#pragma unroll
            for (int q = 4; q < 8; ++q) V6_DMA(t + 2, q);
        }
        __builtin_amdgcn_sched_barrier(0);
        V6_MMA8(7, fa2, fbn)
    }
#undef V6_A
#undef V6_B
#undef V6_MMA8
#undef V6_DMA
    AV_STAMP(2);

    float* cs = (float*)smem;
    const long long cbase = (long long)zo * p.oC + (long long)zi * p.sC;
    const float* R = p.R ? p.R + (long long)zi * p.sR : nullptr;
    const float* bias = p.bias ? p.bias + (long long)zi * p.sBias : nullptr;
    constexpr int CPR = 32;
    float bv[8];
    {
        const int gnt = n0 + (tid % CPR) * 8;
#pragma unroll
        for (int e = 0; e < 8; ++e) bv[e] = (bias && gnt + e < p.N) ? bias[gnt + e] : 0.f;
    }
#pragma unroll
    for (int h = 0; h < 2; ++h) {
        __syncthreads();
#pragma unroll
        for (int i = 0; i < 4; ++i)
#pragma unroll
            for (int j = 0; j < 8; ++j)
#pragma unroll
                for (int e = 0; e < 4; ++e)
                    cs[(wr * 64 + i * 16 + 4 * g + e) * V6_CLD + wc * 128 + j * 16 + r] = acc[4 * h + i][j][e] * p.alpha;
        __syncthreads();
        const int cc = (tid % CPR) * 8, gn = n0 + cc, row0 = tid / CPR;
        const bool full = gn + 8 <= p.N;
        f32x4 n0v = *(const f32x4*)(cs + row0 * V6_CLD + cc), n1v = *(const f32x4*)(cs + row0 * V6_CLD + cc + 4);
        for (int it = 0; it < 128 * CPR / V6_NT; ++it) {
            const int row = row0 + it * (V6_NT / CPR);
            const f32x4 v0 = n0v, v1 = n1v;
            if (it + 1 < 128 * CPR / V6_NT) {
                n0v = *(const f32x4*)(cs + (row + V6_NT / CPR) * V6_CLD + cc);
                n1v = *(const f32x4*)(cs + (row + V6_NT / CPR) * V6_CLD + cc + 4);
            }
            const int gm = m0 + (row >> 6) * 128 + h * 64 + (row & 63);
            if (gm >= p.M || gn >= p.N) continue;
            float v[8];
#pragma unroll
            for (int e = 0; e < 4; ++e) { v[e] = v0[e] + bv[e]; v[4 + e] = v1[e] + bv[4 + e]; }
            const long long off = cbase + (long long)gm * p.ldc + gn;
            epilogue_store(p, fl, v, off, gm, gn, full, R);
        }
    }
#ifdef AV_GEMM_STAMPS
    asm volatile("s_waitcnt vmcnt(0)" ::: "memory");
#endif
    AV_STAMP(3);
}

template <int BNT, bool CONV, bool AKM = false, bool BKM = false>
int launch_fast(const av_gemm_args& p, hipStream_t st, const FastFlags& fl) {
    constexpr int STAGE = TILE_A + BNT * BK * 2;
    constexpr int EPI = BM * (BNT + 4) * 4 + 2048;
    constexpr int LDS = 2 * STAGE > EPI ? 2 * STAGE : EPI;
    auto kern = gemm_nt_bf16_kernel<BNT, CONV, AKM, BKM>;
    static bool attr_done = false;
    if (!attr_done) {
        if (hipFuncSetAttribute((const void*)kern, hipFuncAttributeMaxDynamicSharedMemorySize, LDS) != hipSuccess) {
            av_set_error("av_gemm(fast): cannot raise dynamic LDS to %d", LDS);
            return AV_ERR_LAUNCH;
        }
        attr_done = true;
    }
    const int nbM = av_cdiv(p.M, BM), nbN = av_cdiv(p.N, BNT);
    dim3 grid((unsigned)(nbM * (long long)nbN), 1, (unsigned)p.batch);
    hipLaunchKernelGGL(kern, grid, dim3(NT), LDS, st, p, nbM, nbN, fl);
    AV_LAUNCH_CHECK();
    return AV_OK;
}

int av_gemm_fast_try(const av_gemm_args& p, hipStream_t st) {
    if (p.in_dtype != AV_BF16) return -1;
    if (p.k_total > 0 && !(p.a_mode == AV_A_TRANS && p.b_mode == AV_B_KN && p.batch_inner == 0 && (long long)(p.batch - 1) * p.K < p.k_total)) return -1;
    const bool conv = p.a_mode == AV_A_CONV2D;
    const bool akm = p.a_mode == AV_A_TRANS, bkm = p.b_mode == AV_B_KN;
    if (!conv && !akm && p.a_mode != AV_A_ROWMAJOR) return -1;
    if (!bkm && p.b_mode != AV_B_NK) return -1;
    if (p.K < BK || p.ldb % 8 || p.sA % 8 || p.sB % 8 || p.oA % 8 || p.oB % 8) return -1;
    if (p.K % BK && !(akm && bkm)) return -1;
    if (conv && bkm) return -1;
    if ((akm && (p.M % 8 || p.M <= 64)) || (bkm && (p.N % 8 || p.N <= 64))) return -1;
    if (!al16(p.A) || !al16(p.B) || p.M < 1 || p.N < 1) return -1;
    if (conv) {
        if (p.cCin % 64 || p.cCtot % 8 || p.cCoff % 8 || (p.cKh * p.cKw > 32 && (p.cKw != 1 || p.cKh > 65535))) return -1;
        if (p.cPM && (p.cNF < 1 || p.cT != 1 || p.cKt != 1 || p.batch != 1 || p.cKh * p.cKw > 32 || p.M % (p.cOh * p.cOw * p.cNF))) return -1;
    } else {
        if (p.lda % 8 || p.stats) return -1;
    }
    const long long oes = p.out_dtype == AV_F32 ? 4 : 2;
    FastFlags fl;
    fl.c_vec = al16(p.C) && (!p.C2 || al16(p.C2)) && (p.ldc * oes) % 16 == 0 && (p.sC * oes) % 16 == 0 && (p.oC * oes) % 16 == 0;
    fl.r_vec = p.R && al16(p.R) && (p.ldr % 4 == 0) && (p.sR % 4 == 0);
    const long long aes = p.aux_dtype == AV_F32 ? 4 : 2;
    fl.aux_vec = p.aux && al16(p.aux) && (p.ldc * aes) % 16 == 0 && (p.sC * aes) % 16 == 0 && (p.oC * aes) % 16 == 0;
    const bool narrow = p.N <= 64;
    if (akm || bkm) {
        if (p.stats || p.lda % 8) return -1;
        static const int km8 = [] { const char* e = getenv("AVAMD_GEMM_KM8"); return e ? atoi(e) : 1; }();
        if (akm && bkm && km8 && p.M >= 256 && p.N >= 256 && (km8 >= 2 || av_cdiv(p.M, V4_BM) * av_cdiv(p.N, V4_BN) >= 32) && p.batch_inner == 0 && p.lda < (1 << 24) && p.ldb < (1 << 24)) {
            static bool km_attr = false;
            if (!km_attr) {
                if (hipFuncSetAttribute((const void*)gemm_nt_bf16_v4_kernel<false, true>, hipFuncAttributeMaxDynamicSharedMemorySize, V4_LDS) != hipSuccess) {
                    av_set_error("av_gemm(fast v4 k-major): cannot raise dynamic LDS to %d", V4_LDS);
                    return AV_ERR_LAUNCH;
                }
                km_attr = true;
            }
            const int nbM = av_cdiv(p.M, V4_BM), nbN = av_cdiv(p.N, V4_BN);
            hipLaunchKernelGGL((gemm_nt_bf16_v4_kernel<false, true>), dim3((unsigned)(nbM * nbN * p.batch), 1, 1), dim3(V4_NT), V4_LDS, st, p, nbM, nbN, fl,
                               nbM * nbN * p.batch, V4_BM);
            AV_LAUNCH_CHECK();
            return AV_OK;
        }
        if (akm && bkm) return launch_fast<128, false, true, true>(p, st, fl);
        if (akm) return launch_fast<128, false, true, false>(p, st, fl);
        return launch_fast<128, false, false, true>(p, st, fl);
    }
    static const int v4_mode = [] { const char* e = getenv("AVAMD_GEMM_V4"); return e ? atoi(e) : 1; }();
    static const int v2_mode = [] { const char* e = getenv("AVAMD_GEMM_V2"); return e ? atoi(e) : 2; }();
    const bool v2_ok = !conv && !narrow && p.M >= 512 && (v2_mode == 1 || (v2_mode == 2 && p.K >= 2048));
    static const int v4_conv = [] { const char* e = getenv("AVAMD_GEMM_V4_CONV"); return e ? atoi(e) : 1; }();
    if (conv && v4_conv && v4_mode > 0 && p.N >= 256 && p.M >= 4096 && p.K >= 512 && p.batch == 1 && p.cKh * p.cKw <= 32 && p.alpha == 1.0f) {
        static bool v4c_attr = false;
        if (!v4c_attr) {
            if (hipFuncSetAttribute((const void*)gemm_nt_bf16_v4_kernel<true>, hipFuncAttributeMaxDynamicSharedMemorySize, V4_LDS) != hipSuccess) {
                av_set_error("av_gemm(fast v4 conv): cannot raise dynamic LDS to %d", V4_LDS);
                return AV_ERR_LAUNCH;
            }
            v4c_attr = true;
        }
        const int nbM = av_cdiv(p.M, V4_BM), nbN = av_cdiv(p.N, V4_BN);
        hipLaunchKernelGGL(gemm_nt_bf16_v4_kernel<true>, dim3((unsigned)(nbM * nbN), 1, 1), dim3(V4_NT), V4_LDS, st, p, nbM, nbN, fl, nbM * nbN, V4_BM);
        AV_LAUNCH_CHECK();
        return AV_OK;
    }
    static const int v6_mode = [] { const char* e = getenv("AVAMD_GEMM_V6"); return e ? atoi(e) : 0; }();
    if (v6_mode > 0 && !conv && !narrow && p.M >= 256 && p.N >= 256 && !p.stats) {
        static bool v6_attr = false;
        if (!v6_attr) {
            if (hipFuncSetAttribute((const void*)gemm_nt_bf16_v6_kernel, hipFuncAttributeMaxDynamicSharedMemorySize, V6_LDS) != hipSuccess) {
                av_set_error("av_gemm(fast v6): cannot raise dynamic LDS to %d", V6_LDS);
                return AV_ERR_LAUNCH;
            }
            v6_attr = true;
        }
        const int nbM = av_cdiv(p.M, 256), nbN = av_cdiv(p.N, 256);
        hipLaunchKernelGGL(gemm_nt_bf16_v6_kernel, dim3((unsigned)(nbM * nbN), 1, (unsigned)p.batch), dim3(V6_NT), V6_LDS, st, p, nbM, nbN, fl);
        AV_LAUNCH_CHECK();
        return AV_OK;
    }
    if (!conv && !narrow && v4_mode > 0 && p.M >= 256 && p.N >= 256) {
        const double nk = p.K / 64.0;
        const int nbN4 = av_cdiv(p.N, V4_BN);
        static const int v4_tail = [] { const char* e = getenv("AVAMD_GEMM_V4_TAIL"); return e ? atoi(e) : 1; }();
        static const int v4_bm = [] { const char* e = getenv("AVAMD_GEMM_V4_BM"); return e ? atoi(e) : 0; }();
        static const int v7_mode = [] { const char* e = getenv("AVAMD_GEMM_V7"); return e ? atoi(e) : 1; }();
        const bool v7_vo = p.N % 8 == 0 && fl.c_vec && (!p.R || fl.r_vec) && (!p.aux || fl.aux_vec);
        const bool v7_cls = (p.out_dtype == AV_BF16 && (p.act == AV_ACT_NONE || p.act == AV_ACT_GELU || p.act == AV_ACT_GELU_GF || p.act == AV_ACT_MUL_AUX)) ||
                            (p.out_dtype == AV_F32 && p.act == AV_ACT_NONE);
        const bool v7_ok = v7_mode > 0 && v7_vo && v7_cls;
        int best_bm = V4_BM; double e4 = 1e30; int best_full = 0;
        for (int bm = V4_BM; bm >= 160; bm -= 16) {
            if (v4_bm && bm != v4_bm) continue;
            const long long t4 = (long long)av_cdiv(p.M, bm) * nbN4 * p.batch;
            const double per_tile = nk * 1.55 * ((v7_ok && bm <= 224) ? 0.9 : 1.0) + 4.0;
            const long long r4 = t4 % 256;
            const bool tail = p.batch == 1 && v4_tail && t4 > 256 && r4 > 0 && r4 <= 128;
            const double e = tail ? (double)(t4 / 256) * per_tile + (double)((4 * r4 + 255) / 256) * (nk * 0.8 + 4.0) : (double)((t4 + 255) / 256) * per_tile;
            if (e < e4 * 0.98) { e4 = e; best_bm = bm; best_full = tail ? (int)(t4 - r4) : (int)t4; }
        }
        const long long t2 = (long long)av_cdiv(p.M, V2_BM) * av_cdiv(p.N, V2_BN) * p.batch;
        const long long t1 = (long long)av_cdiv(p.M, BM) * av_cdiv(p.N, 128) * p.batch;
        const double e2 = (double)((t2 + 255) / 256) * (nk * 0.85 + 2.0);
        const double e1 = (double)((t1 + 511) / 512) * (nk * 1.0 + 2.5);
        if (v7_ok && (v7_mode >= 2 || v4_mode >= 2 || e4 < (v2_ok ? (e2 < e1 ? e2 : e1) : e1))) {
            static int ncu = 0;
            if (!ncu) {
                int dev = 0;
                if (hipGetDevice(&dev) != hipSuccess || hipDeviceGetAttribute(&ncu, hipDeviceAttributeMultiprocessorCount, dev) != hipSuccess || ncu <= 0) ncu = 256;
            }
            static const int v7_g = [] { const char* e = getenv("AVAMD_GEMM_V7_G"); return e ? atoi(e) : 0; }();
            const int ng = v7_g > 0 && v7_g < ncu ? v7_g : ncu;
            const int nbM = av_cdiv(p.M, best_bm);
            const int ntile = nbM * nbN4;
            int nfull = ntile;
            if (p.batch == 1 && v4_tail && ntile > ng) { const int r = ntile % ng; if (r > 0 && r <= ng / 2) nfull = ntile - r; }
            const int G = ntile < ng ? ntile : ng;
            int rc = AV_OK;
            auto go = [&](auto kern) {
                static bool attr = false;
                if (!attr) {
                    if (hipFuncSetAttribute((const void*)kern, hipFuncAttributeMaxDynamicSharedMemorySize, V4_LDS) != hipSuccess) {
                        av_set_error("av_gemm(fast v7): cannot raise dynamic LDS to %d", V4_LDS);
                        rc = AV_ERR_LAUNCH;
                        return;
                    }
                    attr = true;
                }
                hipLaunchKernelGGL(kern, dim3((unsigned)G, 1, (unsigned)p.batch), dim3(V4_NT), V4_LDS, st, p, nbM, nbN4, fl, nfull, best_bm);
            };
            const bool nm3 = best_bm <= 224;
            if (p.out_dtype == AV_F32) { if (nm3) go(gemm_nt_bf16_v7_kernel<AV_ACT_NONE, AV_F32, true, 3>); else go(gemm_nt_bf16_v7_kernel<AV_ACT_NONE, AV_F32, true, 4>); }
            else if (p.act == AV_ACT_NONE) { if (nm3) go(gemm_nt_bf16_v7_kernel<AV_ACT_NONE, AV_BF16, true, 3>); else go(gemm_nt_bf16_v7_kernel<AV_ACT_NONE, AV_BF16, true, 4>); }
            else if (p.act == AV_ACT_GELU) { if (nm3) go(gemm_nt_bf16_v7_kernel<AV_ACT_GELU, AV_BF16, true, 3>); else go(gemm_nt_bf16_v7_kernel<AV_ACT_GELU, AV_BF16, true, 4>); }
            else if (p.act == AV_ACT_GELU_GF) { if (nm3) go(gemm_nt_bf16_v7_kernel<AV_ACT_GELU_GF, AV_BF16, true, 3>); else go(gemm_nt_bf16_v7_kernel<AV_ACT_GELU_GF, AV_BF16, true, 4>); }
            else { if (nm3) go(gemm_nt_bf16_v7_kernel<AV_ACT_MUL_AUX, AV_BF16, true, 3>); else go(gemm_nt_bf16_v7_kernel<AV_ACT_MUL_AUX, AV_BF16, true, 4>); }
            if (rc != AV_OK) return rc;
            AV_LAUNCH_CHECK();
            return AV_OK;
        }
        if (v4_mode >= 2 || e4 < (v2_ok ? (e2 < e1 ? e2 : e1) : e1)) {
            static bool v4_attr = false;
            if (!v4_attr) {
                if (hipFuncSetAttribute((const void*)gemm_nt_bf16_v4_kernel<false>, hipFuncAttributeMaxDynamicSharedMemorySize, V4_LDS) != hipSuccess) {
                    av_set_error("av_gemm(fast v4): cannot raise dynamic LDS to %d", V4_LDS);
                    return AV_ERR_LAUNCH;
                }
                v4_attr = true;
            }
            const int nbM = av_cdiv(p.M, best_bm);
            const int ntile = nbM * nbN4;
            const int nfull = p.batch == 1 ? best_full : ntile;
            const unsigned nblocks = (unsigned)(nfull + 4 * (ntile - nfull));
            hipLaunchKernelGGL(gemm_nt_bf16_v4_kernel<false>, dim3(nblocks, 1, (unsigned)p.batch), dim3(V4_NT), V4_LDS, st, p, nbM, nbN4, fl, nfull, best_bm);
            AV_LAUNCH_CHECK();
            return AV_OK;
        }
    }
// ... 42 lines not shown
```

multimodal-av-model_amd/model/decoder.py:

```python
from __future__ import annotations

import torch
import torch.nn as nn
import torch.nn.functional as F

from .. import ops
from ..precision import compute_dtype
from ..utils.shadow import ParamCache


class _HeadFn(torch.autograd.Function):
    @staticmethod
    def forward(fctx, x, w, b, wt, arena, wpad):
        dtype = compute_dtype()
        xt = ops.cast(x.contiguous().float(), dtype)
        logits = ops.linear(xt, wt, b.data, out_dtype=torch.float32)
        lp = ops.log_softmax_fwd(logits)
        fctx.save_for_backward(xt, wt, lp)
        fctx.dtype = dtype
        fctx.arena = arena
        fctx.wpad = wpad
        return lp

    @staticmethod
    def backward(fctx, dlp):
        xt, wt, lp = fctx.saved_tensors
        V, D = wt.shape
        wpad = fctx.wpad
        if wpad is not None:
            Vp = wpad.shape[0]
            dpad = ops.log_softmax_bwd(lp, dlp.contiguous().float(), fctx.dtype, pad_to=64).view(-1, Vp)
            d2 = dpad[:, :V]
            dx = ops.matmul_nn(dpad, wpad, out_dtype=torch.float32).view(xt.shape) if fctx.needs_input_grad[0] else None
        else:
            dlogits = ops.log_softmax_bwd(lp, dlp.contiguous().float(), fctx.dtype)
            d2 = dlogits.view(-1, V)
            dx = ops.matmul_nn(d2, wt, out_dtype=torch.float32).view(xt.shape) if fctx.needs_input_grad[0] else None
        ar, dev = fctx.arena, d2.device
        A = (lambda n, shp, vec=False: ar.out("decoder." + n, shp, dev, vec)) if ar is not None else (lambda n, shp, vec=False: None)
        dw = ops.matmul_tn(d2, xt.view(-1, D), out=A("weight", (V, D))) if fctx.needs_input_grad[1] else None
        db = ops.colsum_into(d2, A("bias", (V,), True)) if fctx.needs_input_grad[2] else None
        return dx, dw, db, None, None, None


class CTCDecoder(nn.Module):
    def __init__(self, input_dim, vocab_size, blank_id=0, native_ctc=None):
        super().__init__()
        self.net = nn.Sequential(nn.Linear(input_dim, vocab_size))
        self.ctc_loss = nn.CTCLoss(blank=blank_id, zero_infinity=True)
        self.blank_id = blank_id
        self.native_ctc = ops.native_ctc_default() if native_ctc is None else bool(native_ctc)
        self._cache = ParamCache()
        self.grad_arena = None
        self._wpad = None

    def forward(self, x, target=None, input_lengths=None, target_lengths=None):
        if not x.is_cuda:
            raise RuntimeError("CTCDecoder (HIP): input must be on the GPU; there is no CPU fallback")
        lin = self.net[0]
        dtype = compute_dtype()
        wpad = None
        if dtype == torch.float32:
            wt = lin.weight.data
        else:
            V, D = lin.weight.shape
            Vp = (V + 63) // 64 * 64
            if Vp != V and D % 8 == 0:
                def build():
                    self._wpad = torch.zeros((Vp, D), dtype=dtype, device=lin.weight.device)
                    self._wpad[:V].copy_(ops.cast(lin.weight.data.contiguous(), dtype))
                    return self._wpad[:V]
                wt = self._cache.get("w", [lin.weight], dtype, build, flat=True)
                wpad = self._wpad
            else:
                wt = self._cache.get("w", [lin.weight], dtype, lambda: ops.cast(lin.weight.data.contiguous(), dtype), flat=True)
        log_probs = _HeadFn.apply(x, lin.weight, lin.bias, wt, self.grad_arena, wpad)
        if target is not None:
            if self.native_ctc:
                return ops.ctc_loss(log_probs, target, input_lengths, target_lengths, blank=self.blank_id, reduction="mean",
                                    zero_infinity=True, batch_first=True)
            return self.ctc_loss(log_probs.transpose(0, 1), target, input_lengths, target_lengths)
        return log_probs
```

multimodal-av-model_amd/model/fusion_module.py:

```python
from __future__ import annotations

from typing import Dict, Optional

import torch
import torch.nn as nn

from .. import _lib as L
from .. import ops
from ..precision import compute_dtype, is_lp
from ..utils.shadow import ParamCache

Tensor = torch.Tensor
import os as _os
PERSISTENT_LSTM = _os.environ.get("AVAMD_LSTM_PERSISTENT", "1") != "0"
FUSED_XATTN = _os.environ.get("AVAMD_FUSED_XATTN", "1") != "0"


def lstm_forward(mod: "CrossAttentionFusion", x_tm: Tensor, save: bool):
    lstm = mod.temporal_model
    dtype = x_tm.dtype
    T, B, _ = x_tm.shape
    H = lstm.hidden_size
    dev = x_tm.device
    layers = []
    inp = x_tm
    out_bt = None
    for layer in range(lstm.num_layers):
        names = [f"weight_ih_l{layer}", f"weight_ih_l{layer}_reverse", f"weight_hh_l{layer}", f"weight_hh_l{layer}_reverse",
                 f"bias_ih_l{layer}", f"bias_ih_l{layer}_reverse", f"bias_hh_l{layer}", f"bias_hh_l{layer}_reverse"]
        P = [getattr(lstm, n) for n in names]
        wih = mod._cache.get(("wih", layer), P[0:2], dtype, lambda: ops.cast(torch.cat([P[0].data, P[1].data], 0).contiguous(), dtype), flat=True)
        whh = mod._cache.get(("whh", layer), P[2:4], dtype, lambda: ops.cast(torch.stack([P[2].data, P[3].data], 0).contiguous(), dtype), flat=True)
        bias = mod._cache.get(("b", layer), P[4:8], torch.float32,
                              lambda: torch.cat([P[4].data + P[6].data, P[5].data + P[7].data], 0).contiguous())
        gx = ops.linear(inp, wih, bias, out_dtype=torch.float32)
        hseq = torch.empty((T, B, 2 * H), dtype=dtype, device=dev)
        cseq = torch.empty((T, B, 2, H), dtype=torch.float32, device=dev)
        gates = torch.empty((T, B, 2, 4 * H), dtype=dtype, device=dev) if save else None
        last = layer == lstm.num_layers - 1
        if last:
            out_bt = torch.empty((B, T, 2 * H), dtype=dtype, device=dev)
        st = ops.stream()
        if PERSISTENT_LSTM and is_lp(dtype) and H == 512:
            cnt = torch.empty(L.LSTM_COUNTER_INTS, dtype=torch.int32, device=dev)
            L.check(L.lib().av_lstm_fwd_layer(ops.ptr(gx), ops.ptr(whh), ops.ptr(hseq), ops.ptr(cseq), ops.ptr(gates),
                                              ops.ptr(out_bt) if last else None, ops.ptr(cnt), T, B, H, st), "av_lstm_fwd_layer")
            mod._lstm_flags.append(cnt)
        else:
            fn = L.lib().av_lstm_fwd_step
            for s in range(T):
                L.check(fn(ops.ptr(gx), ops.ptr(whh), ops.ptr(hseq), ops.ptr(cseq), ops.ptr(gates), ops.ptr(out_bt) if last else None,
                           ops.dt(hseq), T, B, H, s, st), "av_lstm_fwd_step")
        if save:
            layers.append(dict(inp=inp, hseq=hseq, cseq=cseq, gates=gates, wih=wih, whh=whh, names=names))
        inp = hseq
    return out_bt, (layers if save else None)


def lstm_backward(mod: "CrossAttentionFusion", layers, dout_bt: Tensor, grads: Dict[str, Tensor]) -> Tensor:
    lstm = mod.temporal_model
    A = mod._grad_out
    H = lstm.hidden_size
    dout, do_bs, do_ts = dout_bt, dout_bt.shape[1] * 2 * H, 2 * H
    dx = None
    for layer in range(lstm.num_layers - 1, -1, -1):
        c = layers[layer]
        hseq, gates, cseq, inp = c["hseq"], c["gates"], c["cseq"], c["inp"]
        T, B, _ = hseq.shape
        dtype = hseq.dtype
        dev = hseq.device
        whhT = ops.cast(c["whh"].transpose(1, 2).contiguous(), dtype)
        dgates = torch.empty((T, B, 2, 4 * H), dtype=dtype, device=dev)
        dc = torch.empty((2, B, H), dtype=torch.float32, device=dev)
        st = ops.stream()
        if PERSISTENT_LSTM and is_lp(dtype) and H == 512:
            cnt = torch.empty(L.LSTM_COUNTER_INTS, dtype=torch.int32, device=dev)
            L.check(L.lib().av_lstm_bwd_layer(ops.ptr(dout), ops.dt(dout), do_bs, do_ts, ops.ptr(dgates), ops.ptr(whhT), ops.ptr(gates),
                                              ops.ptr(cseq), ops.ptr(dc), ops.ptr(cnt), T, B, H, st), "av_lstm_bwd_layer")
            mod._lstm_flags.append(cnt)
        else:
            fn = L.lib().av_lstm_bwd_step
            for s in range(T):
                L.check(fn(ops.ptr(dout), ops.dt(dout), do_bs, do_ts, ops.ptr(dgates), ops.ptr(whhT), ops.ptr(gates), ops.ptr(cseq),
                           ops.ptr(dc), ops.dt(dgates), T, B, H, s, st), "av_lstm_bwd_step")
        M = T * B
        dg2 = dgates.view(M, 8 * H)
        in_f = inp.shape[-1]
        dwih = ops.matmul_tn(dg2, inp.view(M, in_f), out=A(f"lstm.dwih{layer}", (8 * H, in_f), dev))
        db = ops.colsum_into(dg2, A(f"lstm.db{layer}", (8 * H,), dev, True))
        n = c["names"]
        grads["temporal_model." + n[0]] = dwih[:4 * H]
        grads["temporal_model." + n[1]] = dwih[4 * H:]
        grads["temporal_model." + n[4]] = db[:4 * H]; grads["temporal_model." + n[6]] = db[:4 * H]
        grads["temporal_model." + n[5]] = db[4 * H:]; grads["temporal_model." + n[7]] = db[4 * H:]
        dwhh = A(f"lstm.dwhh{layer}", (2, 4 * H, H), dev)
        if dwhh is None:
            dwhh = torch.zeros((2, 4 * H, H), dtype=torch.float32, device=dev)
        elif T <= 1:
            dwhh.zero_()
        if T > 1:
            h2 = hseq.view(M, 2 * H)
            ops.matmul_tn(dg2[B:, :4 * H], h2[:M - B, :H], out=dwhh[0])
            ops.matmul_tn(dg2[:M - B, 4 * H:], h2[B:, H:], out=dwhh[1])
        grads["temporal_model." + n[2]] = dwhh[0]
        grads["temporal_model." + n[3]] = dwhh[1]
        dx = ops.matmul_nn(dg2, c["wih"], out_dtype=dtype).view(T, B, in_f)
        dout, do_bs, do_ts = dx, in_f, B * in_f
    return dx


class _FusionFn(torch.autograd.Function):
    @staticmethod
    def forward(fctx, mod: "CrossAttentionFusion", save: bool, names, groups: int, visual_feat, audio_feat, mask, *params):
        dtype = compute_dtype()
        dev = audio_feat.device
        E, nh = mod.fused_dim, mod.num_heads
        hd = E // nh
        B, Tv, Dv = visual_feat.shape
        _, Ta, Da = audio_feat.shape
        af = audio_feat.contiguous().float()
        mask = mask.contiguous().long()
        ws = torch.empty(B * Ta + B + groups, dtype=torch.int32, device=dev)
        a_in = torch.empty((B, Tv, Da), dtype=torch.float32, device=dev)
        m_out = torch.empty((B, Tv), dtype=torch.long, device=dev)
        lens = torch.empty((B,), dtype=torch.long, device=dev)
        L.check(L.lib().av_fusion_gather_lerp_fwd(ops.ptr(af), ops.ptr(mask), ops.ptr(ws), ops.ptr(a_in), ops.ptr(m_out), ops.ptr(lens),
                                                  B, Ta, Tv, Da, groups, ops.stream()), "av_fusion_gather_lerp_fwd")
        c = lambda p: mod.cparam(p, dtype)
        vis_t = ops.cast(visual_feat.contiguous().float(), dtype)
        a_in_t = ops.cast(a_in, dtype)
        v = ops.linear(vis_t, c(mod.visual_proj.weight), mod.visual_proj.bias.data)
        a = ops.linear(a_in_t, c(mod.audio_proj.weight), mod.audio_proj.bias.data)
        mha = mod.cross_attn_audio
        Win = c(mha.in_proj_weight)
        bin_ = mha.in_proj_bias.data
        scale = hd ** -0.5
        if FUSED_XATTN and is_lp(dtype) and E == 512 and nh == 4 and Tv <= 112:
            o, q, kv, lse = ops.fusion_xattn_fwd(a, v, Win, bin_, nh, scale, save)
        else:
            q = ops.linear(a, Win[:E], bin_[:E].contiguous()).view(B, Tv, nh, hd)
            kv = ops.linear(v, Win[E:], bin_[E:].contiguous()).view(B, Tv, 2, nh, hd)
            o, lse = ops.attention_fwd(q, kv[:, :, 0], kv[:, :, 1], None, scale, need_lse=save)
        a2v = ops.linear(o.view(B, Tv, E), c(mha.out_proj.weight), mha.out_proj.bias.data)
        fused = ops.linear(a2v, c(mod.fusion_proj.weight), mod.fusion_proj.bias.data)
        x_tm = torch.empty((Tv, B, E), dtype=dtype, device=dev)
        L.check(L.lib().av_permute_bt(ops.ptr(fused), ops.dt(fused), ops.ptr(x_tm), ops.dt(x_tm), B, Tv, E, ops.stream()), "av_permute_bt")
        out_bt, lctx = lstm_forward(mod, x_tm, save)
        out = ops.cast(out_bt, torch.float32)
        if save:
            fctx.saved = dict(ws=ws, vis_t=vis_t, a_in_t=a_in_t, v=v, a=a, q=q, kv=kv, o=o, lse=lse, a2v=a2v, fused=fused, lstm=lctx,
                              shape=(B, Tv, Ta, Da, Dv), dtype=dtype, groups=groups)
        else:
            fctx.saved = None
        fctx.mod, fctx.names = mod, names
        fctx.need_audio = audio_feat.requires_grad
        fctx.need_visual = visual_feat.requires_grad
        fctx.mark_non_differentiable(lens, m_out)
        return out, lens, m_out

    @staticmethod
    def backward(fctx, dout, _dl, _dm):
        mod, s = fctx.mod, fctx.saved
        n_extra = 7
        if s is None:
            return (None,) * (n_extra + len(fctx.names))
        B, Tv, Ta, Da, Dv = s["shape"]
        dtype = s["dtype"]
        E, nh = mod.fused_dim, mod.num_heads
        hd = E // nh
        M = B * Tv
        c = lambda p: mod.cparam(p, dtype)
        g: Dict[str, Tensor] = {}
        dx_tm = lstm_backward(mod, s["lstm"], dout.contiguous().float(), g)
        dfused = torch.empty((B, Tv, E), dtype=dtype, device=dout.device)
        L.check(L.lib().av_permute_bt(ops.ptr(dx_tm), ops.dt(dx_tm), ops.ptr(dfused), ops.dt(dfused), Tv, B, E, ops.stream()), "av_permute_bt")
        df2 = dfused.view(M, E)
        dev = dout.device
        A = mod._grad_out
        g["fusion_proj.weight"] = ops.matmul_tn(df2, s["a2v"].view(M, E), out=A("fusion_proj.weight", (E, E), dev))
        g["fusion_proj.bias"] = ops.colsum_into(df2, A("fusion_proj.bias", (E,), dev, True))
        da2v = ops.matmul_nn(df2, c(mod.fusion_proj.weight))
        mha = mod.cross_attn_audio
        g["cross_attn_audio.out_proj.weight"] = ops.matmul_tn(da2v, s["o"].view(M, E), out=A("xa.out_proj.weight", (E, E), dev))
        g["cross_attn_audio.out_proj.bias"] = ops.colsum_into(da2v, A("xa.out_proj.bias", (E,), dev, True))
        do = ops.matmul_nn(da2v, c(mha.out_proj.weight)).view(B, Tv, nh, hd)
        q, kv = s["q"], s["kv"]
        if FUSED_XATTN and is_lp(dtype) and E == 512 and nh == 4 and Tv <= 112:
            dq, dkv = ops.fusion_xattn_bwd(q, kv, s["o"], do.contiguous(), s["lse"], hd ** -0.5)
        else:
            dq = torch.empty_like(q); dkv = torch.empty_like(kv)
            ops.attention_bwd(q, kv[:, :, 0], kv[:, :, 1], do, dq, dkv[:, :, 0], dkv[:, :, 1], None, hd ** -0.5, o=s["o"], lse=s["lse"])
        Win = c(mha.in_proj_weight)
        dq2, dkv2 = dq.view(M, E), dkv.view(M, 2 * E)
        dWin = A("xa.in_proj_weight", (3 * E, E), dev)
        if dWin is None:
            dWin = torch.empty((3 * E, E), dtype=torch.float32, device=dev)
        ops.matmul_tn(dq2, s["a"].view(M, E), out=dWin[:E])
        ops.matmul_tn(dkv2, s["v"].view(M, E), out=dWin[E:])
        g["cross_attn_audio.in_proj_weight"] = dWin
        dbin = A("xa.in_proj_bias", (3 * E,), dev, True)
        zeroed = dbin is not None
        if dbin is None:
            dbin = torch.empty(3 * E, dtype=torch.float32, device=dev)
        ops.colsum(dq2, out=dbin[:E], accumulate=zeroed); ops.colsum(dkv2, out=dbin[E:], accumulate=zeroed)
        g["cross_attn_audio.in_proj_bias"] = dbin
        da = ops.matmul_nn(dq2, Win[:E])
        dv = ops.matmul_nn(dkv2, Win[E:])
        g["audio_proj.weight"] = ops.matmul_tn(da, s["a_in_t"].view(M, Da), out=A("audio_proj.weight", (E, Da), dev))
        g["audio_proj.bias"] = ops.colsum_into(da, A("audio_proj.bias", (E,), dev, True))
        g["visual_proj.weight"] = ops.matmul_tn(dv, s["vis_t"].view(M, Dv), out=A("visual_proj.weight", (E, Dv), dev))
        g["visual_proj.bias"] = ops.colsum_into(dv, A("visual_proj.bias", (E,), dev, True))
        d_audio = d_visual = None
        if fctx.need_audio:
            da_in = ops.matmul_nn(da, c(mod.audio_proj.weight), out_dtype=torch.float32)
            d_audio = torch.empty((B, Ta, Da), dtype=torch.float32, device=dout.device)
            L.check(L.lib().av_fusion_gather_lerp_bwd(ops.ptr(da_in), ops.ptr(s["ws"]), ops.ptr(d_audio), B, Ta, Tv, Da, s["groups"], ops.stream()),
                    "av_fusion_gather_lerp_bwd")
        if fctx.need_visual:
            d_visual = ops.matmul_nn(dv, c(mod.visual_proj.weight), out_dtype=torch.float32).view(B, Tv, Dv)
        fctx.saved = None
        return (None, None, None, None, d_visual, d_audio, None) + tuple(g.get(n) for n in fctx.names)


class CrossAttentionFusion(nn.Module):
    def __init__(self, visual_dim, audio_dim, fused_dim, num_heads=4):
        super().__init__()
        self.visual_proj = nn.Linear(visual_dim, fused_dim)
        self.audio_proj = nn.Linear(audio_dim, fused_dim)
        self.cross_attn_visual = nn.MultiheadAttention(embed_dim=fused_dim, num_heads=num_heads, batch_first=True)
        self.cross_attn_audio = nn.MultiheadAttention(embed_dim=fused_dim, num_heads=num_heads, batch_first=True)
        self.fusion_proj = nn.Linear(fused_dim, fused_dim)
        self.temporal_model = nn.LSTM(input_size=fused_dim, hidden_size=fused_dim, num_layers=2, batch_first=True, bidirectional=True)
        self.fused_dim, self.num_heads = fused_dim, num_heads
        self._cache = ParamCache()
        self.grad_arena = None
        self._lstm_flags = []
        self._flag_host, self._flag_evt, self._flag_n = None, None, 0
        if fused_dim % 32 or (fused_dim // num_heads) not in (16, 32, 64, 128):
            raise ValueError("fused_dim must be a multiple of 32 with head_dim in {16,32,64,128} for the HIP kernels")

    def stage_flag_check(self):
        if not self._lstm_flags or self._flag_evt is not None:
            return
        n = min(len(self._lstm_flags), 16)
        if self._flag_host is None:
            self._flag_host = torch.zeros(16, dtype=torch.int32).pin_memory()
        words = torch.stack([c[2] for c in self._lstm_flags[:n]])
        self._flag_host[:n].copy_(words, non_blocking=True)
        self._flag_evt = torch.cuda.Event(); self._flag_evt.record()
        self._flag_n = n
        del self._lstm_flags[:n]

    def finish_flag_check(self, wait: bool = False):
        if self._flag_evt is None:
            return
        if not self._flag_evt.query():
            if not wait:
                return
            self._flag_evt.synchronize()
        bad = int(self._flag_host[: self._flag_n].max()) != 0
        self._flag_evt = None
        if bad:
            raise RuntimeError("persistent LSTM kernel: inter-workgroup wait timed out (the step that launched it is invalid); "
                               "AVAMD_LSTM_PERSISTENT=0 selects the per-step kernels (e.g. on a GPU shared with other processes)")

    def drain_flag_check(self):
        while self._flag_evt is not None or self._lstm_flags:
            self.stage_flag_check()
            self.finish_flag_check(wait=True)

    def _grad_out(self, name: str, shape, device, vec: bool = False):
        return self.grad_arena.out("fusion." + name, shape, device, vec) if self.grad_arena is not None else None

    def cparam(self, p: Tensor, dtype) -> Tensor:
        if dtype == torch.float32:
            return p.data
        return self._cache.get(("c", id(p)), [p], dtype, lambda: ops.cast(p.data.contiguous(), dtype), flat=True)

    def forward(self, visual_feat, audio_feat, mask=None, groups: int = 1):
        if mask is None:
            raise ValueError("CrossAttentionFusion: mask is required (the reference dereferences it unconditionally, :66)")
        if not audio_feat.is_cuda:
            raise RuntimeError("CrossAttentionFusion (HIP): inputs must be on the GPU; there is no CPU fallback")
        if getattr(self, "_np", None) is None:
            self._np = [(n, p) for n, p in self.named_parameters() if not n.startswith("cross_attn_visual.")]
        names = [n for n, p in self._np if p.requires_grad]
        params = [p for n, p in self._np if p.requires_grad]
        save = torch.is_grad_enabled() and (bool(names) or audio_feat.requires_grad or visual_feat.requires_grad)
        self.finish_flag_check()
        if len(self._lstm_flags) > 64:
            old, self._lstm_flags = self._lstm_flags[:32], self._lstm_flags[32:]
            if int(torch.stack(old)[:, 2].max()) != 0:
                raise RuntimeError("persistent LSTM kernel: inter-workgroup wait timed out (results of that step are invalid)")
        out, lens, m_out = _FusionFn.apply(self, save, names, groups, visual_feat, audio_feat, mask, *params)
        self.last_mask = m_out
        return out, lens
```

multimodal-av-model_amd/model/w2v2.py:

```python
from __future__ import annotations

import ctypes
import json
import os
from types import SimpleNamespace
from typing import Dict, List, Optional

import torch
import torch.nn as nn

from .. import _lib as L
from .. import ops
from ..precision import compute_dtype, is_lp
from ..utils import init as _init
from ..utils.shadow import ParamCache

Tensor = torch.Tensor
DROP_BITS = os.environ.get("AVAMD_ATTN_DROPBITS", "1") != "0"
FFN_GF = os.environ.get("AVAMD_FFN_GF", "1") != "0"
NATIVE_LAYER = int(os.environ.get("AVAMD_W2V2_NATIVE", "1"))
NATIVE_MAX_ROWS = 4096
PASS_STREAMS = os.environ.get("AVAMD_PASS_STREAMS", "1") != "0"


# ... 429 lines not shown
        ctx = None
        if save and first < nl:
            ctx = dict(saved=saved, hL=h, muf=muf, rsf=rsf, klen=klen, first=first, train=train, B=B, T=T, dtype=dtype,
                       seed=r.seed, hd_p=r.hd_p, at_p=r.at_p, ac_p=r.ac_p)
        return last, mid, ctx

    def backward(self, ctx: dict, dlast: Optional[Tensor], dmid: Optional[Tensor]) -> Dict[str, Tensor]:
        return self.backward_multi([ctx], [dlast], [dmid])

    def backward_multi(self, ctxs: List[dict], dlasts: List[Optional[Tensor]], dmids: List[Optional[Tensor]]) -> Dict[str, Tensor]:
        cfg = self.cfg
        nl = cfg["num_hidden_layers"]
        Hd = cfg["hidden_size"]
        grads: Dict[str, Tensor] = {}
        states = []
        for ctx, dlast, dmid in zip(ctxs, dlasts, dmids):
            B, T = ctx["B"], ctx["T"]
            dev = ctx["hL"].device
            if dlast is not None:
                dh = ops.layernorm_bwd(ctx["hL"], dlast.contiguous().float(), self.P("encoder.layer_norm.weight").data, ctx["muf"], ctx["rsf"])
            else:
                dh = torch.zeros((B, T, Hd), dtype=torch.float32, device=dev)
            states.append(dict(dh=dh, dh_lp=None, dmid=dmid.contiguous().float() if dmid is not None else None))
        first = min(c["first"] for c in ctxs)
        dev = ctxs[0]["hL"].device
        two_streams = PASS_STREAMS and len(ctxs) == 2 and dev.type == "cuda"
        if two_streams:
            main = torch.cuda.current_stream(dev)
            side = self._side_stream(dev)
            side.wait_stream(main)
            for t in _tensors_of(states[1]):
                t.record_stream(side)
        for li in range(nl - 1, first - 1, -1):
            p = f"encoder.layers.{li}."
            for i, (ctx, st) in enumerate(zip(ctxs, states)):
                if li < ctx["first"]:
                    continue
                if two_streams and i == 1:
                    done0 = torch.cuda.Event(); done0.record(main)
                    side.wait_event(done0)
                    with torch.cuda.stream(side):
                        before = set(grads)
                        self._layer_backward(ctx, st, li, grads)
                    for k in grads:
                        if k.startswith(p):
                            grads[k].record_stream(side if k in before else main)
                else:
                    self._layer_backward(ctx, st, li, grads)
            if self.grad_ready is not None:
                keys = [k for k in grads if k.startswith(p)]
                ar = self._arenas.get(li)
                if keys and ar is not None and self.grad_flat_ready is not None and all(ar.owns(grads[k]) for k in keys):
                    self.grad_flat_ready(ar, (side,) if two_streams else ())
                elif keys:
                    if two_streams:
                        main.wait_stream(side)
                    for k, v in zip(keys, self.grad_ready([grads[k] for k in keys])):
                        grads[k] = v
        if two_streams:
            main.wait_stream(side)
            for t in _tensors_of(states[1]):
                t.record_stream(main)
        for ar in self._arenas.values():
            ar.finalize()
        if self.grad_wait is not None:
            self.grad_wait()
        return grads

    def _side_stream(self, dev) -> "torch.cuda.Stream":
        if getattr(self, "_pass_stream", None) is None:
            self._pass_stream = torch.cuda.Stream(device=dev)
        return self._pass_stream

    def begin_grad_step(self) -> None:
        for ar in self._arenas.values():
            ar.begin_step()

    @staticmethod
    def _lower_copy_ok(ctx: dict, li: int, dmid_c: Optional[Tensor]) -> bool:
        lower = li - 1
        return ctx["hd_p"] == 0 or (lower >= ctx["first"] and not isinstance(ctx["saved"][lower], str)
                                    and not (dmid_c is not None and 6 <= lower + 1 <= 9))

    def _layer_backward_native(self, ctx: dict, st: dict, li: int, dh: Tensor, dh_lp: Optional[Tensor]) -> bool:
        cfg = self.cfg
        dtype, B, T, s = ctx["dtype"], ctx["B"], ctx["T"], ctx["saved"][li]
        Hd, nh, I = cfg["hidden_size"], cfg["num_attention_heads"], cfg["intermediate_size"]
        hd, M, dev, w = Hd // nh, B * T, ctx["hL"].device, s["w"]
        wt = [ops.transpose_cached(x) for x in (w.w_2, w.w_1, w.w_o, w.w_qkv)]
        if any(x is None for x in wt):
            return False
        lp_ok = self._lower_copy_ok(ctx, li, st["dmid"])
        e16 = lambda *shape: torch.empty(shape, dtype=dtype, device=dev)
        dh3_t = None if dh_lp is not None else e16(M, Hd)
        du, dx2, dh2_lp, dao, dqkv, dx1 = e16(M, I), e16(M, Hd), e16(M, Hd), e16(M, Hd), e16(B, T, 3, nh, hd), e16(M, Hd)
        dh2 = torch.empty((B, T, Hd), dtype=torch.float32, device=dev); dh_new = torch.empty((B, T, Hd), dtype=torch.float32, device=dev)
        delta = torch.empty((B, nh, T), dtype=torch.float32, device=dev)
        dh_new_lp = e16(B, T, Hd) if lp_ok else None
        a = getattr(self, "_lbargs", None)
        if a is None:
            a = self._lbargs = L.W2v2LayerBwdArgs()
        a.B, a.T, a.hidden, a.heads, a.inter, a.lp, a.gf, a.stream_base, a.lower_stream = B, T, Hd, nh, I, L.AV_BF16, int(bool(s.get("gf"))), li * 8, (li - 1) * 8 + 2
        a.scale, a.hd_p, a.at_p, a.ac_p, a.seed = hd ** -0.5, ctx["hd_p"], ctx["at_p"], ctx["ac_p"], ctx["seed"]
        a.ln1_g, a.ln2_g = w.ln1_g.data_ptr(), w.ln2_g.data_ptr()
        a.w_2t, a.w_1t, a.w_ot, a.w_qkvt = (x.data_ptr() for x in wt)
        a.dh, a.h, a.mu1, a.rs1, a.lse = dh.data_ptr(), s["h"].data_ptr(), s["mu1"].data_ptr(), s["rs1"].data_ptr(), s["lse"].data_ptr()
        a.h2, a.mu2, a.rs2 = s["h2"].data_ptr(), s["mu2"].data_ptr(), s["rs2"].data_ptr()
        a.dh_lp, a.qkv, a.ao, a.amask, a.u = ops.ptr(dh_lp), s["qkv"].data_ptr(), s["ao"].data_ptr(), ops.ptr(s["amask"]), s["u"].data_ptr()
        a.klen = ops.ptr(ctx["klen"])
        a.dh3_t, a.du, a.dx2, a.dh2_lp, a.dao, a.dqkv, a.dx1, a.dh_out_lp = (ops.ptr(dh3_t), du.data_ptr(), dx2.data_ptr(), dh2_lp.data_ptr(), dao.data_ptr(),
                                                                           dqkv.data_ptr(), dx1.data_ptr(), ops.ptr(dh_new_lp))
        a.dh2, a.delta, a.dh_out = dh2.data_ptr(), delta.data_ptr(), dh_new.data_ptr()
        L.check(L.lib().av_w2v2_layer_bwd_dx(ctypes.byref(a), ops.stream()), "av_w2v2_layer_bwd_dx")
        ctx["saved"][li] = None
        st["dh"], st["dh_lp"] = dh_new, dh_new_lp
        return True

    def _layer_backward(self, ctx: dict, st: dict, li: int, grads: Dict[str, Tensor]) -> None:
        dh, dh_lp, dmid_c = st["dh"], st["dh_lp"], st["dmid"]
        if dmid_c is not None and 6 <= li + 1 <= 9 and li + 1 < self.cfg["num_hidden_layers"]:
            ops.axpby(0.25, dmid_c, 1.0, dh)
            dh_lp = None
        if isinstance(ctx["saved"][li], str):
            st["dh_lp"] = dh_lp
            return
        tr = ctx["train"][li]
        ar = self._arenas.get(li)
        if ar is None and tr:
            from ..parallel.dp import GradArena
            ar = self._arenas[li] = GradArena()
        if not tr and _native_ok(ctx["B"] * ctx["T"], ctx["dtype"], ctx["hL"].device) and self._layer_backward_native(ctx, st, li, dh, dh_lp):
            return
        self._layer_backward_kernels(ctx, st, li, grads, ar, dh, dh_lp)

    def _layer_backward_kernels(self, ctx: dict, st: dict, li: int, grads: Dict[str, Tensor], ar, dh: Tensor, dh_lp: Optional[Tensor]) -> None:
        cfg = self.cfg
        dtype, B, T, s, dmid_c = ctx["dtype"], ctx["B"], ctx["T"], ctx["saved"][li], st["dmid"]
        Hd, nh, I = cfg["hidden_size"], cfg["num_attention_heads"], cfg["intermediate_size"]
        hd, M, w = Hd // nh, B * T, s["w"]
        scale = hd ** -0.5
        fuse_lp = is_lp(dtype)
        tr = ctx["train"][li]
        p = f"encoder.layers.{li}."
        seed, hd_p, at_p, ac_p = ctx["seed"], ctx["hd_p"], ctx["at_p"], ctx["ac_p"]
        wgrad, bgrad, gb_target = _grad_writers(grads, ar, ctx["hL"].device, Hd)
        dh3 = dh
        dh3_t = dh_lp if (fuse_lp and dh_lp is not None) else ops.cast_dropout(dh3, dtype, (hd_p, seed, li * 8 + 2))
        if s.get("gf"):
            du = ops.matmul_nn(dh3_t.view(M, Hd), w.w_2, out_dtype=dtype, act=L.ACT_MUL_AUX, aux=s["u"].view(M, I), b_is_weight=True)
        else:
            du = ops.matmul_nn(dh3_t.view(M, Hd), w.w_2, out_dtype=dtype, act=L.ACT_MUL_GELU_GRAD, aux=s["u"].view(M, I), b_is_weight=True,
                               drop=(ac_p, seed, li * 8 + 1))
        if tr:
            wgrad(p + "feed_forward.output_dense.weight", dh3_t.view(M, Hd), s["g"].view(M, I))
            bgrad(p + "feed_forward.output_dense.bias", (dh3_t if hd_p > 0 else dh3).view(M, Hd))
        dx2 = ops.matmul_nn(du, w.w_1, out_dtype=dtype, b_is_weight=True)
        if tr:
            wgrad(p + "feed_forward.intermediate_dense.weight", du, s["x2"].view(M, Hd))
            bgrad(p + "feed_forward.intermediate_dense.bias", du)
        ln2 = p + "final_layer_norm."
        r = ops.layernorm_bwd(s["h2"], dx2.view(B, T, Hd), w.ln2_g, s["mu2"], s["rs2"], dres=dh3,
                              want_param_grads=tr, lp_copy=fuse_lp, lp_drop=(hd_p, seed, li * 8 + 0),
                              gb_acc=gb_target(ln2 + "_gb") if tr else None, packed_gb=True)
        dh2_lp = None
        if fuse_lp:
            r, dh2_lp = r[:-1], r[-1]
            r = r if tr else r[0]
        if tr:
            dh2, gb = r
            grads[ln2 + "_gb"] = gb
        else:
            dh2 = r
        dh2_t = dh2_lp if dh2_lp is not None else ops.cast_dropout(dh2, dtype, (hd_p, seed, li * 8 + 0))
        dao = ops.matmul_nn(dh2_t.view(M, Hd), w.w_o, out_dtype=dtype, b_is_weight=True).view(B, T, nh, hd)
        if tr:
            wgrad(p + "attention.out_proj.weight", dh2_t.view(M, Hd), s["ao"].view(M, Hd))
            bgrad(p + "attention.out_proj.bias", (dh2_t if hd_p > 0 else dh2).view(M, Hd))
        qkv = s["qkv"]
        dqkv = torch.empty_like(qkv)
        ops.attention_bwd(qkv[:, :, 0], qkv[:, :, 1], qkv[:, :, 2], dao, dqkv[:, :, 0], dqkv[:, :, 1], dqkv[:, :, 2], ctx["klen"], scale,
                          o=s["ao"], lse=s["lse"], drop=(at_p, seed, li * 8 + 3), drop_mask=s["amask"])
        dx1 = ops.matmul_nn(dqkv.view(M, 3 * Hd), w.w_qkv, out_dtype=dtype, b_is_weight=True)
        if tr:
            wgrad(p + "attention._qkv_w", dqkv.view(M, 3 * Hd), s["x1"].view(M, Hd))
            bgrad(p + "attention._qkv_b", dqkv.view(M, 3 * Hd))
        lp_ok = fuse_lp and self._lower_copy_ok(ctx, li, dmid_c)
        ln1 = p + "layer_norm."
        r = ops.layernorm_bwd(s["h"], dx1.view(B, T, Hd), w.ln1_g, s["mu1"], s["rs1"], dres=dh2,
                              want_param_grads=tr, lp_copy=lp_ok, lp_drop=(hd_p, seed, (li - 1) * 8 + 2),
                              gb_acc=gb_target(ln1 + "_gb") if tr else None, packed_gb=True)
        dh_lp = None
        if lp_ok:
            r, dh_lp = r[:-1], r[-1]
            r = r if tr else r[0]
        if tr:
            dh, gb = r
            grads[ln1 + "_gb"] = gb
        else:
            dh = r
        ctx["saved"][li] = None
        st["dh"], st["dh_lp"] = dh, dh_lp

    @staticmethod
    def unpack_grads(grads: Dict[str, Tensor], Hd: int) -> Dict[str, Tensor]:
        out: Dict[str, Tensor] = {}
        for k, v in grads.items():
            if k.endswith("._qkv_w") or k.endswith("._qkv_b"):
                base, kind = k[: -len("_qkv_w")], ("weight" if k.endswith("w") else "bias")
                for j, n in enumerate(("q", "k", "v")):
                    out[f"{base}{n}_proj.{kind}"] = v[j * Hd:(j + 1) * Hd]
            elif k.endswith("._gb"):
                base = k[: -len("_gb")]
                out[base + "weight"], out[base + "bias"] = v[:Hd], v[Hd:]
            else:
                out[k] = v
        return out


def _grad_writers(grads: Dict[str, Tensor], ar, dev, Hd: int):
    def wgrad(key, dy, x):
        if key in grads:
            ops.matmul_tn(dy, x, out=grads[key], accumulate=True)
        else:
            grads[key] = ops.matmul_tn(dy, x, out=ar.out(key, (dy.shape[1], x.shape[1]), dev))

    def bgrad(key, dy):
        if key in grads:
            ops.colsum(dy, out=grads[key], accumulate=True)
        else:
            grads[key] = ops.colsum_into(dy, ar.out(key, (dy.shape[-1],), dev, vec=True))

    def gb_target(key):
        hit = grads.get(key)
        return hit if hit is not None else ar.out(key, (2 * Hd,), dev, vec=True)
    return wgrad, bgrad, gb_target


def _tensors_of(obj):
    if torch.is_tensor(obj):
        if obj.is_cuda:
            yield obj
    elif isinstance(obj, dict):
        for v in obj.values():
            yield from _tensors_of(v)
    elif isinstance(obj, (list, tuple)):
        for v in obj:
            yield from _tensors_of(v)


class _EncodeFn(torch.autograd.Function):

    @staticmethod
    def forward(fctx, model: Wav2Vec2ModelHIP, wav, masks, valid, names, *params):
        outs, ctxs = [], []
        fc = getattr(model, "_feat_cache", None)
        own_cache = len(masks) == 2 and fc is None
        if own_cache:
            model._feat_cache = fc = {}
        two_streams = PASS_STREAMS and len(masks) == 2 and wav.is_cuda
        if two_streams:
            dev = wav.device
            main = torch.cuda.current_stream(dev)
            side = model._side_stream(dev)
            model.warm_caches(compute_dtype())
            start = torch.cuda.Event(); start.record(main)
        for i, (am, vl) in enumerate(zip(masks, valid)):
            if two_streams and i == 1:
                side.wait_event(start)
                if fc.get("evt") is not None:
                    side.wait_event(fc["evt"])
                with torch.cuda.stream(side):
                    last, mid, ctx = model.encode(wav, am, save=True, valid_lengths=vl)
                main.wait_stream(side)
                for t in _tensors_of((last, mid, ctx)):
                    t.record_stream(main)
                for t in _tensors_of((wav, am, fc.get("feats"))):
                    t.record_stream(side)
            else:
                last, mid, ctx = model.encode(wav, am, save=True, valid_lengths=vl)
            outs += [last, mid]
            ctxs.append(ctx)
        if own_cache:
            model._feat_cache = None
        fctx.model, fctx.ctxs, fctx.names = model, ctxs, names
        return tuple(outs)

    @staticmethod
    def backward(fctx, *douts):
        live = [(c, douts[2 * i], douts[2 * i + 1]) for i, c in enumerate(fctx.ctxs) if c is not None]
        if not live:
            return (None, None, None, None, None) + tuple(None for _ in fctx.names)
        if fctx.model.grad_pre is not None:
            fctx.model.grad_pre()
        g = fctx.model.backward_multi([c for c, _, _ in live], [a for _, a, _ in live], [b for _, _, b in live])
        g = fctx.model.unpack_grads(g, fctx.model.cfg["hidden_size"])
        fctx.ctxs = None
        return (None, None, None, None, None) + tuple(g.get(n) for n in fctx.names)


def w2v2_apply(model: Wav2Vec2ModelHIP, wav: Tensor, attention_mask, second_mask=None, two_passes: bool = False, valid_lengths=None):
    masks = (attention_mask, second_mask) if two_passes else (attention_mask,)
    valid = tuple(valid_lengths) if valid_lengths is not None else (None,) * len(masks)
    if getattr(model, "_np", None) is None:
        model._np = list(model.named_parameters())
    flags = tuple(p.requires_grad for _, p in model._np)
    if torch.is_grad_enabled() and any(flags):
        if getattr(model, "_np_flags", None) != flags:
            model.check_freeze_policy()
            model._np_flags = flags
            model._np_train = ([n for (n, p), f in zip(model._np, flags) if f], [p for (n, p), f in zip(model._np, flags) if f])
        names, params = model._np_train
        return _EncodeFn.apply(model, wav, masks, valid, names, *params)
    outs = []
    with torch.no_grad():
        for am, vl in zip(masks, valid):
            last, mid, _ = model.encode(wav, am, save=False, valid_lengths=vl)
            outs += [last, mid]
    return tuple(outs)


def load_local_config(path: str) -> dict:
    with open(os.path.join(path, "config.json"), "r", encoding="utf-8") as f:
        c = json.load(f)
    if c.get("feat_extract_norm", "layer") != "layer" or not c.get("do_stable_layer_norm", True):
        raise NotImplementedError("only the stable-layer-norm / feat_extract_norm='layer' (XLSR) architecture is built")
    keys = ("hidden_size", "num_hidden_layers", "num_attention_heads", "intermediate_size", "conv_dim", "conv_kernel", "conv_stride",
            "num_conv_pos_embeddings", "num_conv_pos_embedding_groups", "layer_norm_eps")
    out = {k: (tuple(c[k]) if isinstance(c[k], list) else c[k]) for k in keys}
    hf_defaults = dict(hidden_dropout=0.1, attention_dropout=0.1, activation_dropout=0.1, feat_proj_dropout=0.0, layerdrop=0.1,
                       mask_time_prob=0.05, mask_time_length=10, mask_time_min_masks=2, mask_feature_prob=0.0, mask_feature_length=10,
                       mask_feature_min_masks=0, apply_spec_augment=True)
    for k, v in hf_defaults.items():
        out[k] = c.get(k, v)
    out["conv_bias"] = bool(c.get("conv_bias", False))
    return out


_DROP_PREFIXES = ("lm_head.", "quantizer.", "project_hid.", "project_q.", "dropout_features.")


def remap_hf_keys(sd: Dict[str, Tensor]) -> Dict[str, Tensor]:
    out: Dict[str, Tensor] = {}
    for k, v in sd.items():
        if k.startswith("wav2vec2."):
            k = k[len("wav2vec2."):]
        if k.startswith(_DROP_PREFIXES):
            continue
        if k.endswith("pos_conv_embed.conv.weight_g"):
            k = k[:-len("weight_g")] + "parametrizations.weight.original0"
        elif k.endswith("pos_conv_embed.conv.weight_v"):
            k = k[:-len("weight_v")] + "parametrizations.weight.original1"
        out[k] = v
    return out


def load_local_weights(path: str) -> Optional[Dict[str, Tensor]]:
    st = os.path.join(path, "model.safetensors")
    if os.path.exists(st):
        from safetensors.torch import load_file
        return remap_hf_keys(load_file(st))
    pt = os.path.join(path, "pytorch_model.bin")
    if os.path.exists(pt):
        return remap_hf_keys(torch.load(pt, map_location="cpu", weights_only=True))
    return None
```

multimodal-av-model_amd/ops.py:

```python
from __future__ import annotations

import ctypes as C
import os
from typing import Optional

import torch

from . import _lib as L
from . import precision
from ._lib import AV_BF16, AV_F32

Tensor = torch.Tensor


def _lp() -> torch.dtype:
    return torch.float16 if precision.get_precision() == "fp16" else torch.bfloat16


def dt(t: Tensor) -> int:
    if t.dtype == torch.float32:
        return AV_F32
    if t.dtype == _lp():
        return AV_BF16
    raise TypeError(f"unsupported dtype {t.dtype} (the library of precision mode {precision.get_precision()!r} handles float32 / {_lp()})")


def tdt(code: int) -> torch.dtype:
    return torch.float32 if code == AV_F32 else _lp()


def ptr(t: Optional[Tensor]):
    return None if t is None else t.data_ptr()


_raw_stream = getattr(torch._C, "_cuda_getCurrentRawStream", None)
_cur_dev = getattr(torch._C, "_cuda_getDevice", None) or torch.cuda.current_device


def stream():
    if _raw_stream is not None:
        return _raw_stream(_cur_dev())
    return torch.cuda.current_stream().cuda_stream


def h2d_async(arr, device) -> Tensor:
    return torch.from_numpy(arr).pin_memory().to(device, non_blocking=True)


def _req(t: Tensor, name: str):
    if not t.is_cuda:
        raise RuntimeError(f"{name}: tensor must live on the GPU (no CPU fallback in libavhip)")


class GemmProbe:
    active = None

    @classmethod
    def start(cls, in_dtype: int, a_mode: int, b_mode: int, wide: bool):
        cls.active = dict(key=(in_dtype, a_mode, b_mode, wide), records=[])

    @classmethod
    def stop(cls):
        a, cls.active = cls.active, None
        return a


class AttnProbe:
    active = None

    @classmethod
    def start(cls):
        cls.active = []

    @classmethod
    def stop(cls):
        a, cls.active = cls.active, None
        return a


def _probed(tag, flops, nbytes, fn):
    pr = AttnProbe.active
    if pr is None:
        return fn()
    e0 = torch.cuda.Event(enable_timing=True); e1 = torch.cuda.Event(enable_timing=True)
    e0.record()
    r = fn()
    e1.record()
    pr.append((e0, e1, tag, float(flops), float(nbytes)))
    return r


def gemm(A: Tensor, B: Tensor, C_: Tensor, *, M: int, N: int, K: int, lda: int, ldb: int, ldc: int,
         a_mode: int = L.A_ROWMAJOR, b_mode: int = L.B_NK, bias: Optional[Tensor] = None, act: int = L.ACT_NONE,
         R: Optional[Tensor] = None, ldr: int = 0, aux: Optional[Tensor] = None, C2: Optional[Tensor] = None,
         stats: Optional[Tensor] = None, alpha: float = 1.0, batch: int = 1, sA: int = 0, sB: int = 0, sC: int = 0,
         sR: int = 0, sBias: int = 0, conv: Optional[dict] = None, a_off: int = 0, b_off: int = 0, c_off: int = 0,
         batch_inner: int = 0, oA: int = 0, oB: int = 0, oC: int = 0, drop: Optional[tuple] = None, k_total: int = 0) -> Tensor:
    _req(A, "gemm A"); _req(B, "gemm B"); _req(C_, "gemm C")
    if A.dtype != B.dtype:
        raise TypeError(f"gemm: A {A.dtype} and B {B.dtype} must match")
    a = L.GemmArgs()
    a.A = A.data_ptr() + a_off * A.element_size()
    a.B = B.data_ptr() + b_off * B.element_size()
    a.C = C_.data_ptr() + c_off * C_.element_size()
    a.C2 = ptr(C2) if C2 is None else C2.data_ptr() + c_off * C2.element_size()
    a.bias = ptr(bias); a.R = ptr(R) if R is None else R.data_ptr() + c_off * 4
    a.aux = ptr(aux); a.stats = ptr(stats)
    a.M, a.N, a.K, a.batch = M, N, K, batch
    a.lda, a.ldb, a.ldc, a.ldr = lda, ldb, ldc, (ldr or ldc)
    a.sA, a.sB, a.sC, a.sR, a.sBias = sA, sB, sC, sR, sBias
    a.batch_inner, a.oA, a.oB, a.oC = batch_inner, oA, oB, oC
    a.k_total = k_total
    if drop is not None and drop[0] > 0:
        a.drop_p, a.drop_seed, a.drop_stream = float(drop[0]), int(drop[1]), int(drop[2])
    a.a_mode, a.b_mode = a_mode, b_mode
    a.in_dtype, a.out_dtype = dt(A), dt(C_)
    a.aux_dtype = dt(aux) if aux is not None else 0
    a.act, a.alpha = act, alpha
    if bias is not None and bias.dtype != torch.float32:
        raise TypeError("gemm: bias must be float32")
    if R is not None and R.dtype != torch.float32:
        raise TypeError("gemm: residual must be float32")
    if conv:
        for k, v in conv.items():
            setattr(a, k, v)
    pr = GemmProbe.active
    if pr is not None and pr["key"] == (a.in_dtype, a_mode, b_mode, N > 64):
        e0 = torch.cuda.Event(enable_timing=True); e1 = torch.cuda.Event(enable_timing=True)
        e0.record()
        L.check(L.lib().av_gemm(C.byref(a), stream()), "av_gemm")
        e1.record()
        es, oes = A.element_size(), C_.element_size()
        nbytes = batch * ((M * K + N * K) * es + M * N * (oes + (4 if R is not None else 0) + (aux.element_size() if aux is not None else 0)
                                                          + (oes if C2 is not None else 0)))
        pr["records"].append((e0, e1, 2.0 * M * N * K * batch, float(nbytes),
                              (M, N, K, batch, act, bias is not None, R is not None, aux is not None, C2 is not None,
                               drop is not None and drop[0] > 0, bool(conv), stats is not None)))
        return C_
    L.check(L.lib().av_gemm(C.byref(a), stream()), "av_gemm")
    return C_


def linear(x: Tensor, w: Tensor, bias: Optional[Tensor] = None, *, out_dtype: Optional[torch.dtype] = None,
           act: int = L.ACT_NONE, R: Optional[Tensor] = None, out: Optional[Tensor] = None, C2: Optional[Tensor] = None,
           aux: Optional[Tensor] = None, alpha: float = 1.0, drop: Optional[tuple] = None) -> Tensor:
    K = x.shape[-1]
    M = x.numel() // K
    N = w.shape[0]
    assert w.shape[1] == K and x.is_contiguous() and w.is_contiguous()
    if out is None:
        out = torch.empty(x.shape[:-1] + (N,), dtype=out_dtype or x.dtype, device=x.device)
    gemm(x, w, out, M=M, N=N, K=K, lda=K, ldb=K, ldc=N, bias=bias, act=act, R=R, aux=aux, C2=C2, alpha=alpha, drop=drop)
    return out


def transpose(x: Tensor, out_dtype: Optional[torch.dtype] = None, pad_to: int = 1) -> Tensor:
    R, Cc = x.shape
    assert x.stride(1) == 1
    Rp = (R + pad_to - 1) // pad_to * pad_to
    out = torch.empty((Cc, Rp), dtype=out_dtype or x.dtype, device=x.device)
    L.check(L.lib().av_transpose(ptr(x), dt(x), ptr(out), dt(out), R, Cc, x.stride(0), Rp, stream()), "av_transpose")
    return out


_WT_CACHE = {}


def transpose_cached(b: Tensor, hot_ok: bool = False) -> Optional[Tensor]:
    key = (b.data_ptr(), tuple(b.shape), b.dtype)
    ver = b._version
    hit = _WT_CACHE.get(key)
    if hit is None or hit[2]() is not b:
        import weakref
        hit = [ver, transpose(b), weakref.ref(b), 0]
        if len(_WT_CACHE) > 512:
            _WT_CACHE.clear()
        _WT_CACHE[key] = hit
    elif hit[0] != ver:
        hit[3] += 1
        if hot_ok and hit[3] >= 2:
            hit[0], hit[1] = None, None
            return None
        hit[0], hit[1] = ver, transpose(b)
    elif hit[1] is None:
        if hot_ok:
            return None
        hit[0], hit[1] = ver, transpose(b)
    return hit[1]


def _fast_ok(t: Tensor, K: int, N: int) -> bool:
    return precision.is_lp(t.dtype) and K >= 64 and N > 64


KMAJOR = os.environ.get("AVAMD_GEMM_KMAJOR", "1") != "0"
KM8 = int(os.environ.get("AVAMD_GEMM_KM8", "1"))
KMAJOR_DX_HOT = os.environ.get("AVAMD_GEMM_KMAJOR_DX", "0") != "0"


def matmul_nn(a: Tensor, b: Tensor, *, out_dtype: Optional[torch.dtype] = None, act: int = L.ACT_NONE,
              aux: Optional[Tensor] = None, R: Optional[Tensor] = None, out: Optional[Tensor] = None, alpha: float = 1.0,
              b_is_weight: bool = False, drop: Optional[tuple] = None) -> Tensor:
    K = a.shape[-1]
    M = a.numel() // K
    N = b.shape[1]
    assert b.shape[0] == K and a.is_contiguous() and b.is_contiguous()
    if out is None:
        out = torch.empty(a.shape[:-1] + (N,), dtype=out_dtype or a.dtype, device=a.device)
    kmajor_ok = KMAJOR and N % 8 == 0
    if _fast_ok(a, K, N) and K % 64 == 0 and (b_is_weight or not kmajor_ok):
        bt = transpose_cached(b, hot_ok=kmajor_ok and KMAJOR_DX_HOT) if b_is_weight else transpose(b)
        if bt is not None:
            gemm(a, bt, out, M=M, N=N, K=K, lda=K, ldb=K, ldc=N, act=act, aux=aux, R=R, alpha=alpha, drop=drop)
            return out
    gemm(a, b, out, M=M, N=N, K=K, lda=K, ldb=N, ldc=N, b_mode=L.B_KN, act=act, aux=aux, R=R, alpha=alpha, drop=drop)
    return out


def _split_k(tiles: int, Kk: int, mn: int, slots: int = 512) -> int:
    best, best_cost = 1, None
    for S in range(1, 9):
        if S > 1 and Kk // S < 512:
            break
        rounds = (tiles * S + slots - 1) // slots
        cost = rounds * (Kk / S) * 22e-9 + (S * mn * 8 / 5e12 if S > 1 else 0.0)
        if best_cost is None or cost < best_cost * 0.97:
            best, best_cost = S, cost
    return best


def _split_k8(tiles: int, Kk: int, mn: int, slots: int = 256):
    best = (1, Kk, None)
    for S in range(1, 33):
        chunk = ((Kk + S - 1) // S + 63) // 64 * 64
        if S > 1 and chunk < 512:
            break
        Se = (Kk + chunk - 1) // chunk
        rounds = (tiles * Se + slots - 1) // slots
        cost = rounds * (chunk / 64 * 1.55e-6 + 7e-6) + (Se * mn * 8 / 5e12 if Se > 1 else 0.0)
        if best[2] is None or cost < best[2] * 0.97:
            best = (Se, chunk, cost)
    return best[0], best[1]


def matmul_tn(a: Tensor, b: Tensor, *, out: Optional[Tensor] = None, alpha: float = 1.0, accumulate: bool = False) -> Tensor:
    Kk, M = a.shape
    N = b.shape[1]
    assert b.shape[0] == Kk and a.stride(1) == 1 and b.stride(1) == 1
    if out is None:
        out = torch.empty((M, N), dtype=torch.float32, device=a.device)
    if _fast_ok(a, Kk, N) and M > 64 and not (KMAJOR and M % 8 == 0 and N % 8 == 0 and N > 64 and a.stride(0) % 8 == 0 and b.stride(0) % 8 == 0):
        at = transpose(a, pad_to=64)
        bt = transpose(b, pad_to=64)
        Kp = at.shape[1]
        gemm(at, bt, out, M=M, N=N, K=Kp, lda=Kp, ldb=Kp, ldc=N, alpha=alpha, R=out if accumulate else None)
        return out
    km = KMAJOR and _fast_ok(a, Kk, N) and M > 64 and M % 8 == 0 and N % 8 == 0 and a.stride(0) % 8 == 0 and b.stride(0) % 8 == 0
    t8 = ((M + 255) // 256) * ((N + 255) // 256)
    if km and KM8 and M >= 256 and N >= 256 and (KM8 >= 2 or t8 >= 32):
        S, chunk = _split_k8(t8, Kk, M * N)
    else:
        tiles = ((M + 127) // 128) * ((N + 127) // 128)
        S = _split_k(tiles, Kk, M * N) if km else 1
        if S > 1:
            chunk = ((Kk + S - 1) // S + 63) // 64 * 64
            S = (Kk + chunk - 1) // chunk
    if S > 1:
        parts = torch.empty((S, M, N), dtype=torch.float32, device=a.device)
        gemm(a, b, parts, M=M, N=N, K=chunk, lda=a.stride(0), ldb=b.stride(0), ldc=N, a_mode=L.A_TRANS, b_mode=L.B_KN, batch=S,
             sA=chunk * a.stride(0), sB=chunk * b.stride(0), sC=M * N, k_total=Kk)
        L.check(L.lib().av_sum_slices(ptr(parts), S, M * N, M * N, float(alpha), ptr(out), int(accumulate), stream()), "av_sum_slices")
        return out
    gemm(a, b, out, M=M, N=N, K=Kk, lda=a.stride(0), ldb=b.stride(0), ldc=N, a_mode=L.A_TRANS, b_mode=L.B_KN, alpha=alpha,
         R=out if accumulate else None)
    return out


def layernorm_fwd(x: Tensor, gamma: Tensor, beta: Tensor, *, out_dtype: torch.dtype, eps: float = 1e-5, act: int = L.ACT_NONE,
                  save_stats: bool = False):
    cols = x.shape[-1]
    rows = x.numel() // cols
    assert x.is_contiguous()
    y = torch.empty(x.shape, dtype=out_dtype, device=x.device)
    mean = rstd = None
    if save_stats:
        mean = torch.empty(rows, dtype=torch.float32, device=x.device)
        rstd = torch.empty(rows, dtype=torch.float32, device=x.device)
    L.check(L.lib().av_layernorm_fwd(ptr(x), dt(x), ptr(gamma), ptr(beta), ptr(y), dt(y), ptr(mean), ptr(rstd), rows, cols,
                                     eps, act, stream()), "av_layernorm_fwd")
    return (y, mean, rstd) if save_stats else y


def layernorm_bwd(x: Tensor, dy: Tensor, gamma: Tensor, mean: Tensor, rstd: Tensor, dres: Optional[Tensor] = None,
                  want_param_grads: bool = False, lp_copy: bool = False, lp_drop: Optional[tuple] = None, gb_acc: Optional[Tensor] = None,
                  packed_gb: bool = False):
    cols = x.shape[-1]
    rows = x.numel() // cols
    assert x.is_contiguous() and dy.is_contiguous()
    dx = torch.empty(x.shape, dtype=torch.float32, device=x.device)
    dxl = torch.empty(x.shape, dtype=_lp(), device=x.device) if lp_copy else None
    nblk = max(1, min(512, (rows + 15) // 16))
    part = torch.empty((nblk, 2 * cols), dtype=torch.float32, device=x.device) if want_param_grads else None
    if lp_copy and lp_drop is not None and lp_drop[0] > 0:
        L.check(L.lib().av_layernorm_bwd_drop(ptr(x), dt(x), ptr(dy), dt(dy), ptr(gamma), ptr(mean), ptr(rstd), ptr(dres), ptr(dx),
                                              ptr(part), nblk, rows, cols, ptr(dxl), float(lp_drop[0]), int(lp_drop[1]), int(lp_drop[2]), stream()),
                "av_layernorm_bwd_drop")
    else:
        L.check(L.lib().av_layernorm_bwd(ptr(x), dt(x), ptr(dy), dt(dy), ptr(gamma), ptr(mean), ptr(rstd), ptr(dres), ptr(dx),
                                         ptr(part), nblk, rows, cols, ptr(dxl), stream()), "av_layernorm_bwd")
    res = (dx,)
    if want_param_grads:
        if gb_acc is not None:
            gb = colsum(part, out=gb_acc, accumulate=True)
            res = (dx, gb)
        elif packed_gb:
            res = (dx, colsum(part))
        else:
            gb = colsum(part)
            res = (dx, gb[:cols], gb[cols:])
    if lp_copy:
        return res + (dxl,)
    return res if want_param_grads else dx


def log_softmax_fwd(x: Tensor) -> Tensor:
    cols = x.shape[-1]
    y = torch.empty(x.shape, dtype=torch.float32, device=x.device)
    L.check(L.lib().av_log_softmax_fwd(ptr(x), dt(x), ptr(y), x.numel() // cols, cols, stream()), "av_log_softmax_fwd")
    return y


def log_softmax_bwd(y: Tensor, dy: Tensor, out_dtype: torch.dtype, pad_to: int = 0) -> Tensor:
    cols = y.shape[-1]
    ldx = (cols + pad_to - 1) // pad_to * pad_to if pad_to > 0 else cols
    dx = torch.empty(y.shape[:-1] + (ldx,), dtype=out_dtype, device=y.device)
    L.check(L.lib().av_log_softmax_bwd_ld(ptr(y), ptr(dy), ptr(dx), dt(dx), y.numel() // cols, cols, ldx, stream()), "av_log_softmax_bwd")
    return dx


def colsum(x: Tensor, out: Optional[Tensor] = None, accumulate: bool = False) -> Tensor:
    cols = x.shape[-1]
    if x.is_contiguous():
        rows, ld = x.numel() // cols, cols
    else:
        assert x.dim() == 2 and x.stride(1) == 1
        rows, ld = x.shape[0], x.stride(0)
    if out is None:
        out = torch.empty(cols, dtype=torch.float32, device=x.device)
        accumulate = False
    L.check(L.lib().av_colsum(ptr(x), dt(x), ptr(out), rows, cols, ld, int(accumulate), stream()), "av_colsum")
    return out


def colsum_into(x: Tensor, zeroed_view: Optional[Tensor]) -> Tensor:
    return colsum(x, out=zeroed_view, accumulate=True) if zeroed_view is not None else colsum(x)


def cast(x: Tensor, dtype: torch.dtype) -> Tensor:
    if x.dtype == dtype:
        return x
    assert x.is_contiguous()
    y = torch.empty(x.shape, dtype=dtype, device=x.device)
    L.check(L.lib().av_cast(ptr(x), dt(x), ptr(y), dt(y), x.numel(), stream()), "av_cast")
    return y


def cast_dropout(x: Tensor, dtype: torch.dtype, drop: Optional[tuple]) -> Tensor:
    if drop is None or drop[0] <= 0:
        return cast(x, dtype)
    assert x.is_contiguous()
    y = torch.empty(x.shape, dtype=dtype, device=x.device)
    L.check(L.lib().av_cast_dropout(ptr(x), dt(x), ptr(y), dt(y), x.numel(), float(drop[0]), int(drop[1]), int(drop[2]), stream()), "av_cast_dropout")
    return y


def axpby(a: float, x: Tensor, b: float, y: Tensor) -> Tensor:
    assert x.is_contiguous() and y.is_contiguous() and y.dtype == torch.float32 and x.numel() == y.numel()
    L.check(L.lib().av_axpby(a, ptr(x), dt(x), b, ptr(y), x.numel(), stream()), "av_axpby")
    return y


def mask_rows_(x: Tensor, keep_u8: Tensor) -> Tensor:
    cols = x.shape[-1]
    L.check(L.lib().av_mask_rows(ptr(x), dt(x), ptr(keep_u8), x.numel() // cols, cols, stream()), "av_mask_rows")
    return x


def _chk_view(t: Tensor, name: str):
    if t.dim() != 4 or t.stride(3) != 1 or t.stride(2) != t.shape[3]:
        raise ValueError(f"{name}: expected a [B,T,H,D] view with contiguous D and head stride D, got {tuple(t.shape)} / {t.stride()}")


_ATTN_SHORT = os.environ.get("AVAMD_ATTN_SHORT", "1") != "0"


def attention_mask_shape_ok(dtype, B: int, Tq: int, Tk: int, D: int) -> bool:
    return _ATTN_SHORT and precision.is_lp(dtype) and D == 64 and Tq <= 256 and Tk <= 256 and B <= 65535


def attention_dropmask(B: int, H: int, Tq: int, Tk: int, drop: tuple, device) -> Tensor:
    mask = torch.empty((B, H, (Tq + 15) // 16, 64), dtype=torch.int64, device=device)
    L.check(L.lib().av_attention_dropmask(ptr(mask), B, H, Tq, Tk, float(drop[0]), int(drop[1]), int(drop[2]), stream()), "av_attention_dropmask")
    return mask


def attention_fwd(q: Tensor, k: Tensor, v: Tensor, klen: Optional[Tensor], scale: float, need_lse: bool = True,
                  drop: Optional[tuple] = None, drop_mask: Optional[Tensor] = None):
    for t, n in ((q, "q"), (k, "k"), (v, "v")):
        _chk_view(t, n)
    B, Tq, H, D = q.shape
    Tk = k.shape[1]
    o = torch.empty((B, Tq, H, D), dtype=q.dtype, device=q.device)
    lse = torch.empty((B, H, Tq), dtype=torch.float32, device=q.device) if need_lse else None
    dp, dseed, dstream = (float(drop[0]), int(drop[1]), int(drop[2])) if (drop is not None and drop[0] > 0) else (0.0, 0, 0)
    es = q.element_size()
    _probed(f"fwd{D}", 4.0 * B * H * Tq * Tk * D, B * H * D * es * (2 * Tq + 2 * Tk),
            lambda: L.check(L.lib().av_attention_fwd_mask(ptr(q), ptr(k), ptr(v), ptr(o), ptr(lse), dt(q), B, H, Tq, Tk, D,
                                                          q.stride(0), q.stride(1), k.stride(0), k.stride(1), v.stride(0), v.stride(1),
                                                          o.stride(0), o.stride(1), ptr(klen), scale, dp, dseed, dstream,
                                                          ptr(drop_mask) if dp > 0 else None, stream()), "av_attention_fwd"))
    return o, lse


def fusion_xattn_fwd(a: Tensor, v: Tensor, w_in: Tensor, b_in: Tensor, nh: int, scale: float, save: bool):
    B, T, E = a.shape
    hd = E // nh
    assert a.is_contiguous() and v.is_contiguous() and w_in.is_contiguous() and w_in.shape == (3 * E, E) and b_in.dtype == torch.float32
    o = torch.empty((B, T, nh, hd), dtype=a.dtype, device=a.device)
# ... 187 lines not shown
```

Measured before the change: 992.4 utterances/s.

## Fuse bias-gradient column sums into weight-gradient GEMM via MFMA with ones

Adds an optional a_colsum output to the bf16 k-major GEMM fast paths. The kernel computes column sums of the dY operand with extra MFMAs against a ones vector, done by one wave group per tile row, and adds them into the bias gradient with atomics. The wav2vec2, fusion, LSTM and decoder backward passes now use this instead of separate colsum kernels, so each bias gradient no longer needs its own read of dY. In exchange it adds MFMA work and float atomics (summation order becomes nondeterministic), and the fast path needs a zero-init when not accumulating.

Result: no change. 998.5 utterances/s (median of 6 runs) (+0.6%).

```diff
diff --git a/include/av_hip.h b/include/av_hip.h
--- a/include/av_hip.h
+++ b/include/av_hip.h
@@ -49,6 +49,7 @@
     unsigned long long drop_seed;
     int k_total;
     int cNF, cPM;
+    float* a_colsum;
 } av_gemm_args;
 int av_gemm(const av_gemm_args* args, void* stream);
 int av_sum_slices(const float* parts, int n_slices, long long n, long long stride, float alpha, float* out, int accumulate,
diff --git a/multimodal-av-model_amd/_lib.py b/multimodal-av-model_amd/_lib.py
--- a/multimodal-av-model_amd/_lib.py
+++ b/multimodal-av-model_amd/_lib.py
@@ -31,6 +31,7 @@
         ("batch_inner", i32), ("oA", ll), ("oB", ll), ("oC", ll),
         ("drop_p", f32), ("drop_stream", C.c_uint), ("drop_seed", C.c_ulonglong),
         ("k_total", i32), ("cNF", i32), ("cPM", i32),
+        ("a_colsum", vp),
     ]
 
 
diff --git a/multimodal-av-model_amd/csrc/gemm.hip b/multimodal-av-model_amd/csrc/gemm.hip
--- a/multimodal-av-model_amd/csrc/gemm.hip
+++ b/multimodal-av-model_amd/csrc/gemm.hip
@@ -391,6 +391,7 @@
         if (fr >= 0) return fr;
     }
     AV_CHECK(p.cPM == 0, "av_gemm: position-major pixel order (cPM) needs the bf16 fast path (2-D convolution, Cin a multiple of 64, one batch)");
+    AV_CHECK(p.a_colsum == nullptr, "av_gemm: a_colsum needs the bf16 fast path with both operands k-major (a_mode 1, b_mode 1, M, N multiples of 8 and > 64)");
     AV_CHECK(p.k_total == 0, "av_gemm: split-K (k_total) needs the bf16 fast path with both operands k-major (a_mode 1, b_mode 1, M, N multiples of 8 and > 64)");
     const bool wide = p.N > 64;
     if (p.in_dtype == AV_F32) {
diff --git a/multimodal-av-model_amd/csrc/gemm_fast.hip b/multimodal-av-model_amd/csrc/gemm_fast.hip
--- a/multimodal-av-model_amd/csrc/gemm_fast.hip
+++ b/multimodal-av-model_amd/csrc/gemm_fast.hip
@@ -415,6 +415,16 @@
     for (int i = 0; i < WM_T; ++i)
 #pragma unroll
         for (int j = 0; j < 4; ++j) acc[i][j] = f32x4{0.f, 0.f, 0.f, 0.f};
+    bool cs_on = false;
+    int cs_n = 0;
+    f32x4 csacc[2] = {f32x4{0.f, 0.f, 0.f, 0.f}, f32x4{0.f, 0.f, 0.f, 0.f}};
+    bf16x8 cs_ones;
+    if constexpr (AKM && BKM) {
+        cs_on = p.a_colsum != nullptr && nb == 0;
+        cs_n = __builtin_amdgcn_readfirstlane(w & 1);
+#pragma unroll
+        for (int e = 0; e < 8; ++e) cs_ones[e] = (bf16_t)1.0f;
+    }
 
     TapSeq ts;
     ts.seq = 0ull; ts.ntap = -1; ts.sh = 0;
@@ -484,8 +494,26 @@
 #pragma unroll
                 for (int j = 0; j < 4; ++j)
                     acc[i][j] = AV_MFMA_F32_16X16X32_LP(a[i], b[j], acc[i][j], 0, 0, 0);
+            if constexpr (AKM && BKM) {
+                if (cs_on) {
+#pragma unroll
+                    for (int i = 0; i < WM_T; ++i)
+                        if ((i >> 1) == cs_n) csacc[i & 1] = AV_MFMA_F32_16X16X32_LP(a[i], cs_ones, csacc[i & 1], 0, 0, 0);
+                }
+            }
         }
         __syncthreads();
+    }
+    if constexpr (AKM && BKM) {
+        if (cs_on && r == 0) {
+#pragma unroll
+            for (int q = 0; q < 2; ++q)
+#pragma unroll
+                for (int e = 0; e < 4; ++e) {
+                    const int gm = m0 + wrow + (2 * cs_n + q) * 16 + 4 * g + e;
+                    if (gm < p.M) atomicAdd(p.a_colsum + gm, csacc[q][e]);
+                }
+        }
     }
 
     float* cs = (float*)smem;
@@ -1047,6 +1075,17 @@
             for (int i = 0; i < 4; ++i)
 #pragma unroll
                 for (int j = 0; j < 2; ++j) acc[a][b][i][j] = f32x4{0.f, 0.f, 0.f, 0.f};
+
+    bool cs_on = false;
+    int cs_i = 0, cs_next = nb;
+    f32x4 csacc[2] = {f32x4{0.f, 0.f, 0.f, 0.f}, f32x4{0.f, 0.f, 0.f, 0.f}};
+    bf16x8 cs_ones;
+    if constexpr (KM) {
+        cs_on = p.a_colsum != nullptr;
+        cs_i = __builtin_amdgcn_readfirstlane(wc);
+#pragma unroll
+        for (int e = 0; e < 8; ++e) cs_ones[e] = (bf16_t)1.0f;
+    }
 
     int nk = p.K / BK;
     int Kz = p.K;
@@ -1162,7 +1201,12 @@
         km8_tie8(KFB);                                                                                             \
         _Pragma("unroll") for (int j = 0; j < 2; ++j) { FB[j][0] = km8_join(KFB[j][0]); FB[j][1] = km8_join(KFB[j][1]); } } }
 #define V4_JOIN_NONE
-#define V4_MMA(QA, QB, FB, JOIN)                                                                                   \
+#define V4_CS_NONE(QA)
+#define V4_CS_ROWS(QA)                                                                                             \
+    if constexpr (KM) { if (cs_now) {                                                                              \
+        _Pragma("unroll") for (int i = 0; i < 4; ++i)                                                              \
+            if (cs_i == i) { V4_MFMA_OP(csacc[QA], fa[i][0], cs_ones); V4_MFMA_OP(csacc[QA], fa[i][1], cs_ones); } } }
+#define V4_MMA(QA, QB, FB, JOIN, CS)                                                                               \
     __builtin_amdgcn_s_barrier();                                                                                  \
     __builtin_amdgcn_s_waitcnt(0xC07F);                                                                            \
     JOIN                                                                                                           \
@@ -1172,6 +1216,7 @@
         _Pragma("unroll") for (int i = 0; i < 4; ++i)                                                              \
             _Pragma("unroll") for (int j = 0; j < 2; ++j)                                                          \
                 V4_MFMA_OP(acc[QA][QB][i][j], fa[i][ks], FB[j][ks]);                                               \
+    CS(QA)                                                                                                         \
     __builtin_amdgcn_s_setprio(0);                                                                                 \
     __builtin_amdgcn_sched_barrier(0);                                                                             \
     __builtin_amdgcn_s_barrier();                                                                                  \
@@ -1186,23 +1231,25 @@
             int y = b4 + j - 2; y = y < 0 ? y + V4_NS : y; si[j] = y;
         }
         b4 += 4; b4 = b4 >= V4_NS ? b4 - V4_NS : b4;
+        bool cs_now = false;
+        if constexpr (KM) { cs_now = cs_on && t == cs_next; if (cs_now) cs_next += nbN; }
         if constexpr (KM) { V4_READ_B(3, fb0, kfb) } else { V4_READ_B(3, fb, kfb) }
         __builtin_amdgcn_sched_barrier(0);
         V4_READ_A(0, nmt0)
         if (4 * t + V4_LEAD + 0 < nh) issue(t + (V4_LEAD + 0) / 4, (V4_LEAD + 0) % 4, si[0]);
-        if constexpr (KM) { V4_MMA(0, 0, fb0, V4_JOIN_A V4_JOIN_B(fb0, kfb)) } else { V4_MMA(0, 0, fb, V4_JOIN_NONE) }
+        if constexpr (KM) { V4_MMA(0, 0, fb0, V4_JOIN_A V4_JOIN_B(fb0, kfb), V4_CS_ROWS) } else { V4_MMA(0, 0, fb, V4_JOIN_NONE, V4_CS_NONE) }
         V4_READ_B(1, fb, kfb)
         if (4 * t + V4_LEAD + 1 < nh) issue(t + (V4_LEAD + 1) / 4, (V4_LEAD + 1) % 4, si[1]);
-        V4_MMA(0, 1, fb, V4_JOIN_B(fb, kfb))
+        V4_MMA(0, 1, fb, V4_JOIN_B(fb, kfb), V4_CS_NONE)
         V4_READ_A(2, nmt1)
         if (4 * t + V4_LEAD + 2 < nh) issue(t + (V4_LEAD + 2) / 4, (V4_LEAD + 2) % 4, si[2]);
-        V4_MMA(1, 1, fb, V4_JOIN_A)
+        V4_MMA(1, 1, fb, V4_JOIN_A, V4_CS_ROWS)
         if constexpr (!KM) { V4_READ_B(3, fb, kfb) }
         if (4 * t + V4_LEAD + 3 < nh) {
             issue(t + (V4_LEAD + 3) / 4, (V4_LEAD + 3) % 4, si[3]);
             if constexpr (V4_LEAD == 8) asm volatile("s_waitcnt vmcnt(8)" ::: "memory"); else asm volatile("s_waitcnt vmcnt(4)" ::: "memory");
         } else asm volatile("s_waitcnt vmcnt(0)" ::: "memory");
-        if constexpr (KM) { V4_MMA(1, 0, fb0, V4_JOIN_NONE) } else { V4_MMA(1, 0, fb, V4_JOIN_B(fb, kfb)) }
+        if constexpr (KM) { V4_MMA(1, 0, fb0, V4_JOIN_NONE, V4_CS_NONE) } else { V4_MMA(1, 0, fb, V4_JOIN_B(fb, kfb), V4_CS_NONE) }
     }
 #undef V4_READ_A
 #undef V4_READ_B
@@ -1211,8 +1258,21 @@
 #undef V4_JOIN_B
 #undef V4_JOIN_NONE
 #undef V4_MFMA_OP
+#undef V4_CS_ROWS
+#undef V4_CS_NONE
     if (wr == 0) __builtin_amdgcn_s_barrier();
     AV_STAMP(2);
+    if constexpr (KM) {
+        if (cs_on && cs_next != nb && r == 0) {
+#pragma unroll
+            for (int half = 0; half < 2; ++half)
+#pragma unroll
+                for (int e = 0; e < 4; ++e) {
+                    const int row = half * 128 + wr * 64 + cs_i * 16 + 4 * g + e;
+                    if (row < rows_here) atomicAdd(p.a_colsum + m0 + row, csacc[half][e]);
+                }
+        }
+    }
 
     float* cs = (float*)smem;
     const long long cbase = (long long)zo * p.oC + (long long)zi * p.sC;
@@ -1770,6 +1830,7 @@
     if (p.k_total > 0 && !(p.a_mode == AV_A_TRANS && p.b_mode == AV_B_KN && p.batch_inner == 0 && (long long)(p.batch - 1) * p.K < p.k_total)) return -1;
     const bool conv = p.a_mode == AV_A_CONV2D;
     const bool akm = p.a_mode == AV_A_TRANS, bkm = p.b_mode == AV_B_KN;
+    if (p.a_colsum && !(akm && bkm && p.batch_inner == 0)) return -1;
     if (!conv && !akm && p.a_mode != AV_A_ROWMAJOR) return -1;
     if (!bkm && p.b_mode != AV_B_NK) return -1;
     if (p.K < BK || p.ldb % 8 || p.sA % 8 || p.sB % 8 || p.oA % 8 || p.oB % 8) return -1;
diff --git a/multimodal-av-model_amd/model/decoder.py b/multimodal-av-model_amd/model/decoder.py
--- a/multimodal-av-model_amd/model/decoder.py
+++ b/multimodal-av-model_amd/model/decoder.py
@@ -38,8 +38,11 @@
             dx = ops.matmul_nn(d2, wt, out_dtype=torch.float32).view(xt.shape) if fctx.needs_input_grad[0] else None
         ar, dev = fctx.arena, d2.device
         A = (lambda n, shp, vec=False: ar.out("decoder." + n, shp, dev, vec)) if ar is not None else (lambda n, shp, vec=False: None)
-        dw = ops.matmul_tn(d2, xt.view(-1, D), out=A("weight", (V, D))) if fctx.needs_input_grad[1] else None
-        db = ops.colsum_into(d2, A("bias", (V,), True)) if fctx.needs_input_grad[2] else None
+        if fctx.needs_input_grad[1] and fctx.needs_input_grad[2]:
+            dw, db = ops.matmul_tn_bias(d2, xt.view(-1, D), out=A("weight", (V, D)), bias_view=A("bias", (V,), True))
+        else:
+            dw = ops.matmul_tn(d2, xt.view(-1, D), out=A("weight", (V, D))) if fctx.needs_input_grad[1] else None
+            db = ops.colsum_into(d2, A("bias", (V,), True)) if fctx.needs_input_grad[2] else None
         return dx, dw, db, None, None, None
 
 
diff --git a/multimodal-av-model_amd/model/fusion_module.py b/multimodal-av-model_amd/model/fusion_module.py
--- a/multimodal-av-model_amd/model/fusion_module.py
+++ b/multimodal-av-model_amd/model/fusion_module.py
@@ -86,8 +86,8 @@
         M = T * B
         dg2 = dgates.view(M, 8 * H)
         in_f = inp.shape[-1]
-        dwih = ops.matmul_tn(dg2, inp.view(M, in_f), out=A(f"lstm.dwih{layer}", (8 * H, in_f), dev))
-        db = ops.colsum_into(dg2, A(f"lstm.db{layer}", (8 * H,), dev, True))
+        dwih, db = ops.matmul_tn_bias(dg2, inp.view(M, in_f), out=A(f"lstm.dwih{layer}", (8 * H, in_f), dev),
+                                      bias_view=A(f"lstm.db{layer}", (8 * H,), dev, True))
         n = c["names"]
         grads["temporal_model." + n[0]] = dwih[:4 * H]
         grads["temporal_model." + n[1]] = dwih[4 * H:]
@@ -177,12 +177,12 @@
         df2 = dfused.view(M, E)
         dev = dout.device
         A = mod._grad_out
-        g["fusion_proj.weight"] = ops.matmul_tn(df2, s["a2v"].view(M, E), out=A("fusion_proj.weight", (E, E), dev))
-        g["fusion_proj.bias"] = ops.colsum_into(df2, A("fusion_proj.bias", (E,), dev, True))
+        g["fusion_proj.weight"], g["fusion_proj.bias"] = ops.matmul_tn_bias(df2, s["a2v"].view(M, E), out=A("fusion_proj.weight", (E, E), dev),
+                                                                            bias_view=A("fusion_proj.bias", (E,), dev, True))
         da2v = ops.matmul_nn(df2, c(mod.fusion_proj.weight))
         mha = mod.cross_attn_audio
-        g["cross_attn_audio.out_proj.weight"] = ops.matmul_tn(da2v, s["o"].view(M, E), out=A("xa.out_proj.weight", (E, E), dev))
-        g["cross_attn_audio.out_proj.bias"] = ops.colsum_into(da2v, A("xa.out_proj.bias", (E,), dev, True))
+        g["cross_attn_audio.out_proj.weight"], g["cross_attn_audio.out_proj.bias"] = ops.matmul_tn_bias(
+            da2v, s["o"].view(M, E), out=A("xa.out_proj.weight", (E, E), dev), bias_view=A("xa.out_proj.bias", (E,), dev, True))
         do = ops.matmul_nn(da2v, c(mha.out_proj.weight)).view(B, Tv, nh, hd)
         q, kv = s["q"], s["kv"]
         if FUSED_XATTN and is_lp(dtype) and E == 512 and nh == 4 and Tv <= 112:
@@ -195,21 +195,20 @@
         dWin = A("xa.in_proj_weight", (3 * E, E), dev)
         if dWin is None:
             dWin = torch.empty((3 * E, E), dtype=torch.float32, device=dev)
-        ops.matmul_tn(dq2, s["a"].view(M, E), out=dWin[:E])
-        ops.matmul_tn(dkv2, s["v"].view(M, E), out=dWin[E:])
-        g["cross_attn_audio.in_proj_weight"] = dWin
         dbin = A("xa.in_proj_bias", (3 * E,), dev, True)
         zeroed = dbin is not None
         if dbin is None:
             dbin = torch.empty(3 * E, dtype=torch.float32, device=dev)
-        ops.colsum(dq2, out=dbin[:E], accumulate=zeroed); ops.colsum(dkv2, out=dbin[E:], accumulate=zeroed)
+        ops.matmul_tn(dq2, s["a"].view(M, E), out=dWin[:E], colsum_out=dbin[:E], colsum_accumulate=zeroed)
+        ops.matmul_tn(dkv2, s["v"].view(M, E), out=dWin[E:], colsum_out=dbin[E:], colsum_accumulate=zeroed)
+        g["cross_attn_audio.in_proj_weight"] = dWin
         g["cross_attn_audio.in_proj_bias"] = dbin
         da = ops.matmul_nn(dq2, Win[:E])
         dv = ops.matmul_nn(dkv2, Win[E:])
-        g["audio_proj.weight"] = ops.matmul_tn(da, s["a_in_t"].view(M, Da), out=A("audio_proj.weight", (E, Da), dev))
-        g["audio_proj.bias"] = ops.colsum_into(da, A("audio_proj.bias", (E,), dev, True))
-        g["visual_proj.weight"] = ops.matmul_tn(dv, s["vis_t"].view(M, Dv), out=A("visual_proj.weight", (E, Dv), dev))
-        g["visual_proj.bias"] = ops.colsum_into(dv, A("visual_proj.bias", (E,), dev, True))
+        g["audio_proj.weight"], g["audio_proj.bias"] = ops.matmul_tn_bias(da, s["a_in_t"].view(M, Da), out=A("audio_proj.weight", (E, Da), dev),
+                                                                          bias_view=A("audio_proj.bias", (E,), dev, True))
+        g["visual_proj.weight"], g["visual_proj.bias"] = ops.matmul_tn_bias(dv, s["vis_t"].view(M, Dv), out=A("visual_proj.weight", (E, Dv), dev),
+                                                                            bias_view=A("visual_proj.bias", (E,), dev, True))
         d_audio = d_visual = None
         if fctx.need_audio:
             da_in = ops.matmul_nn(da, c(mod.audio_proj.weight), out_dtype=torch.float32)
diff --git a/multimodal-av-model_amd/model/w2v2.py b/multimodal-av-model_amd/model/w2v2.py
--- a/multimodal-av-model_amd/model/w2v2.py
+++ b/multimodal-av-model_amd/model/w2v2.py
@@ -605,12 +605,14 @@
             du = ops.matmul_nn(dh3_t.view(M, Hd), w.w_2, out_dtype=dtype, act=L.ACT_MUL_GELU_GRAD, aux=s["u"].view(M, I), b_is_weight=True,
                                drop=(ac_p, seed, li * 8 + 1))
         if tr:
-            wgrad(p + "feed_forward.output_dense.weight", dh3_t.view(M, Hd), s["g"].view(M, I))
-            bgrad(p + "feed_forward.output_dense.bias", (dh3_t if hd_p > 0 else dh3).view(M, Hd))
+            if hd_p > 0:
+                wgrad(p + "feed_forward.output_dense.weight", dh3_t.view(M, Hd), s["g"].view(M, I), bias=p + "feed_forward.output_dense.bias")
+            else:
+                wgrad(p + "feed_forward.output_dense.weight", dh3_t.view(M, Hd), s["g"].view(M, I))
+                bgrad(p + "feed_forward.output_dense.bias", dh3.view(M, Hd))
         dx2 = ops.matmul_nn(du, w.w_1, out_dtype=dtype, b_is_weight=True)
         if tr:
-            wgrad(p + "feed_forward.intermediate_dense.weight", du, s["x2"].view(M, Hd))
-            bgrad(p + "feed_forward.intermediate_dense.bias", du)
+            wgrad(p + "feed_forward.intermediate_dense.weight", du, s["x2"].view(M, Hd), bias=p + "feed_forward.intermediate_dense.bias")
         ln2 = p + "final_layer_norm."
         r = ops.layernorm_bwd(s["h2"], dx2.view(B, T, Hd), w.ln2_g, s["mu2"], s["rs2"], dres=dh3,
                               want_param_grads=tr, lp_copy=fuse_lp, lp_drop=(hd_p, seed, li * 8 + 0),
@@ -627,16 +629,18 @@
         dh2_t = dh2_lp if dh2_lp is not None else ops.cast_dropout(dh2, dtype, (hd_p, seed, li * 8 + 0))
         dao = ops.matmul_nn(dh2_t.view(M, Hd), w.w_o, out_dtype=dtype, b_is_weight=True).view(B, T, nh, hd)
         if tr:
-            wgrad(p + "attention.out_proj.weight", dh2_t.view(M, Hd), s["ao"].view(M, Hd))
-            bgrad(p + "attention.out_proj.bias", (dh2_t if hd_p > 0 else dh2).view(M, Hd))
+            if hd_p > 0:
+                wgrad(p + "attention.out_proj.weight", dh2_t.view(M, Hd), s["ao"].view(M, Hd), bias=p + "attention.out_proj.bias")
+            else:
+                wgrad(p + "attention.out_proj.weight", dh2_t.view(M, Hd), s["ao"].view(M, Hd))
+                bgrad(p + "attention.out_proj.bias", dh2.view(M, Hd))
         qkv = s["qkv"]
         dqkv = torch.empty_like(qkv)
         ops.attention_bwd(qkv[:, :, 0], qkv[:, :, 1], qkv[:, :, 2], dao, dqkv[:, :, 0], dqkv[:, :, 1], dqkv[:, :, 2], ctx["klen"], scale,
                           o=s["ao"], lse=s["lse"], drop=(at_p, seed, li * 8 + 3), drop_mask=s["amask"])
         dx1 = ops.matmul_nn(dqkv.view(M, 3 * Hd), w.w_qkv, out_dtype=dtype, b_is_weight=True)
         if tr:
-            wgrad(p + "attention._qkv_w", dqkv.view(M, 3 * Hd), s["x1"].view(M, Hd))
-            bgrad(p + "attention._qkv_b", dqkv.view(M, 3 * Hd))
+            wgrad(p + "attention._qkv_w", dqkv.view(M, 3 * Hd), s["x1"].view(M, Hd), bias=p + "attention._qkv_b")
         lp_ok = fuse_lp and self._lower_copy_ok(ctx, li, dmid_c)
         ln1 = p + "layer_norm."
         r = ops.layernorm_bwd(s["h"], dx1.view(B, T, Hd), w.ln1_g, s["mu1"], s["rs1"], dres=dh2,
@@ -671,11 +675,20 @@
 
 
 def _grad_writers(grads: Dict[str, Tensor], ar, dev, Hd: int):
-    def wgrad(key, dy, x):
+    def wgrad(key, dy, x, bias=None):
+        cs = cs_acc = None
+        if bias is not None:
+            cs = grads.get(bias)
+            if cs is None:
+                cs = ar.out(bias, (dy.shape[-1],), dev, vec=True)
+                cs_acc = cs is not None
+                grads[bias] = cs = cs if cs_acc else torch.empty(dy.shape[-1], dtype=torch.float32, device=dev)
+            else:
+                cs_acc = True
         if key in grads:
-            ops.matmul_tn(dy, x, out=grads[key], accumulate=True)
+            ops.matmul_tn(dy, x, out=grads[key], accumulate=True, colsum_out=cs, colsum_accumulate=bool(cs_acc))
         else:
-            grads[key] = ops.matmul_tn(dy, x, out=ar.out(key, (dy.shape[1], x.shape[1]), dev))
+            grads[key] = ops.matmul_tn(dy, x, out=ar.out(key, (dy.shape[1], x.shape[1]), dev), colsum_out=cs, colsum_accumulate=bool(cs_acc))
 
     def bgrad(key, dy):
         if key in grads:
diff --git a/multimodal-av-model_amd/ops.py b/multimodal-av-model_amd/ops.py
--- a/multimodal-av-model_amd/ops.py
+++ b/multimodal-av-model_amd/ops.py
@@ -95,7 +95,8 @@
          R: Optional[Tensor] = None, ldr: int = 0, aux: Optional[Tensor] = None, C2: Optional[Tensor] = None,
          stats: Optional[Tensor] = None, alpha: float = 1.0, batch: int = 1, sA: int = 0, sB: int = 0, sC: int = 0,
          sR: int = 0, sBias: int = 0, conv: Optional[dict] = None, a_off: int = 0, b_off: int = 0, c_off: int = 0,
-         batch_inner: int = 0, oA: int = 0, oB: int = 0, oC: int = 0, drop: Optional[tuple] = None, k_total: int = 0) -> Tensor:
+         batch_inner: int = 0, oA: int = 0, oB: int = 0, oC: int = 0, drop: Optional[tuple] = None, k_total: int = 0,
+         a_colsum: Optional[Tensor] = None) -> Tensor:
     _req(A, "gemm A"); _req(B, "gemm B"); _req(C_, "gemm C")
     if A.dtype != B.dtype:
         raise TypeError(f"gemm: A {A.dtype} and B {B.dtype} must match")
@@ -111,6 +112,7 @@
     a.sA, a.sB, a.sC, a.sR, a.sBias = sA, sB, sC, sR, sBias
     a.batch_inner, a.oA, a.oB, a.oC = batch_inner, oA, oB, oC
     a.k_total = k_total
+    a.a_colsum = ptr(a_colsum)
     if drop is not None and drop[0] > 0:
         a.drop_p, a.drop_seed, a.drop_stream = float(drop[0]), int(drop[1]), int(drop[2])
     a.a_mode, a.b_mode = a_mode, b_mode
@@ -243,12 +245,26 @@
     return best[0], best[1]
 
 
-def matmul_tn(a: Tensor, b: Tensor, *, out: Optional[Tensor] = None, alpha: float = 1.0, accumulate: bool = False) -> Tensor:
+WGRAD_BIAS = os.environ.get("AVAMD_WGRAD_BIAS", "1") != "0"
+
+
+def matmul_tn(a: Tensor, b: Tensor, *, out: Optional[Tensor] = None, alpha: float = 1.0, accumulate: bool = False,
+              colsum_out: Optional[Tensor] = None, colsum_accumulate: bool = False) -> Tensor:
     Kk, M = a.shape
     N = b.shape[1]
     assert b.shape[0] == Kk and a.stride(1) == 1 and b.stride(1) == 1
     if out is None:
         out = torch.empty((M, N), dtype=torch.float32, device=a.device)
+    cs = None
+    if colsum_out is not None:
+        assert colsum_out.dtype == torch.float32 and colsum_out.is_contiguous() and colsum_out.numel() == M
+        if (WGRAD_BIAS and KMAJOR and _fast_ok(a, Kk, N) and M > 64 and M % 8 == 0 and N % 8 == 0 and a.stride(0) % 8 == 0 and b.stride(0) % 8 == 0
+                and a.data_ptr() % 16 == 0 and b.data_ptr() % 16 == 0):
+            cs = colsum_out
+            if not colsum_accumulate:
+                cs.zero_()
+        else:
+            colsum(a, out=colsum_out, accumulate=colsum_accumulate)
     if _fast_ok(a, Kk, N) and M > 64 and not (KMAJOR and M % 8 == 0 and N % 8 == 0 and N > 64 and a.stride(0) % 8 == 0 and b.stride(0) % 8 == 0):
         at = transpose(a, pad_to=64)
         bt = transpose(b, pad_to=64)
@@ -268,12 +284,18 @@
     if S > 1:
         parts = torch.empty((S, M, N), dtype=torch.float32, device=a.device)
         gemm(a, b, parts, M=M, N=N, K=chunk, lda=a.stride(0), ldb=b.stride(0), ldc=N, a_mode=L.A_TRANS, b_mode=L.B_KN, batch=S,
-             sA=chunk * a.stride(0), sB=chunk * b.stride(0), sC=M * N, k_total=Kk)
+             sA=chunk * a.stride(0), sB=chunk * b.stride(0), sC=M * N, k_total=Kk, a_colsum=cs)
         L.check(L.lib().av_sum_slices(ptr(parts), S, M * N, M * N, float(alpha), ptr(out), int(accumulate), stream()), "av_sum_slices")
         return out
     gemm(a, b, out, M=M, N=N, K=Kk, lda=a.stride(0), ldb=b.stride(0), ldc=N, a_mode=L.A_TRANS, b_mode=L.B_KN, alpha=alpha,
-         R=out if accumulate else None)
+         R=out if accumulate else None, a_colsum=cs)
     return out
+
+
+def matmul_tn_bias(a: Tensor, b: Tensor, *, out: Optional[Tensor] = None, bias_view: Optional[Tensor] = None):
+    db = bias_view if bias_view is not None else torch.empty(a.shape[1], dtype=torch.float32, device=a.device)
+    dw = matmul_tn(a, b, out=out, colsum_out=db, colsum_accumulate=bias_view is not None)
+    return dw, db
 
 
 def layernorm_fwd(x: Tensor, gamma: Tensor, beta: Tensor, *, out_dtype: torch.dtype, eps: float = 1e-5, act: int = L.ACT_NONE,
```
